# pynbody/topsy

Measured on AMD Instinct MI355X. Metric: particles/sec splatted to 1024^2 buffer, higher is better.
Workload: dtype f32

## Files before the change

### include/topsy_splat.h

```cpp
#ifndef TOPSY_SPLAT_H
#define TOPSY_SPLAT_H

#include <stdint.h>

#ifdef __cplusplus
extern "C" {
#endif

typedef struct tsp_context tsp_context;

enum {
    TSP_OK = 0,
    TSP_EINVAL = -1,
    TSP_EHIP = -2,
    TSP_ENODEV = -3,
    TSP_ESTATE = -4,
    TSP_ECOMM = -5,
    TSP_ENOMEM = -6
};

enum {
    TSP_MODE_WEIGHTED = 0,
    TSP_MODE_DEPTH = 1,
    TSP_MODE_RGB = 2,
    TSP_MODE_KINEMATIC = 3
};

enum {
    TSP_PIPE_DEFAULT = 0,
    TSP_PIPE_GENERIC = 1,
    TSP_SAMPLE_BILINEAR_MIP0 = 0x10,
    TSP_SAMPLE_BILINEAR_MIP = 0x20
};

const char *tsp_last_error(void);
int tsp_version(void);
int tsp_stats_size(void);

int tsp_device_count(void);

int tsp_create(int device_id, int resolution, int n_channels, tsp_context **out);
void tsp_destroy(tsp_context *ctx);

int tsp_set_kernel_mips(tsp_context *ctx, const float *lut, int n0, int n_levels);

int tsp_upload_particles(tsp_context *ctx, int64_t n, const float *x, const float *y, const float *z,
                         const float *h, const float *mass);
int tsp_upload_quantity(tsp_context *ctx, const float *q);
int tsp_upload_rgb(tsp_context *ctx, const float *r, const float *g, const float *b);
int tsp_upload_band_magnitudes(tsp_context *ctx, int n_bands, const double *mags, const double *weights);

int tsp_generate_synthetic(tsp_context *ctx, int64_t n_total, int64_t first, int64_t count,
                           uint64_t seed, float h_cap, int with_quantity, int with_rgb);

int tsp_reorder_spatial(tsp_context *ctx, int n_strata, uint64_t seed, int64_t *perm_out);
int tsp_get_strata_offsets(tsp_context *ctx, int64_t *offsets_out, int capacity);

int tsp_get_cell_layout(tsp_context *ctx, int *n_strata_out, int *cells_per_axis_out, float *box_lo_out ,
                        float *cell_width_out );
int64_t tsp_get_cell_offsets(tsp_context *ctx, int64_t *offsets_out, int64_t capacity);

int tsp_download_particles(tsp_context *ctx, float *x, float *y, float *z, float *h, float *mass,
                           float *q, float *r, float *g, float *b);
int64_t tsp_num_particles(tsp_context *ctx);

int tsp_render(tsp_context *ctx, const float *M, float scale_factor, const int64_t *starts,
               const int64_t *lens, int n_ranges, int clear, int mode, int flags, double *gpu_ms_out);

int tsp_render_undo(tsp_context *ctx);

int tsp_read_image(tsp_context *ctx, float *out);
int tsp_write_image(tsp_context *ctx, const float *in);

int tsp_colormap_scalar(tsp_context *ctx, const float *lut_rgba, int n_lut, float vmin, float vmax,
                        int log_scale, int weighted, uint8_t *out_rgba);
int tsp_colormap_rgb(tsp_context *ctx, float vmin, float vmax, float gamma, uint8_t *out_rgba8,
                     float *out_rgba_f32);

int tsp_colormap_set_lut2d(tsp_context *ctx, const float *lut_rgba, int n);
int tsp_colormap_bivariate(tsp_context *ctx, float vmin, float vmax, float density_vmin, float density_vmax,
                           int log_scale, int weighted, uint8_t *out_rgba);
int tsp_colormap_bivariate_host(tsp_context *ctx, const float *img, int H, int W, int C, float vmin, float vmax,
                                float density_vmin, float density_vmax, int log_scale, int weighted,
                                uint8_t *out_rgba);

int tsp_colormap_scalar_host(tsp_context *ctx, const float *img, int H, int W, int C,
                             const float *lut_rgba, int n_lut, float vmin, float vmax, int log_scale,
                             int weighted, uint8_t *out_rgba);
int tsp_colormap_rgb_host(tsp_context *ctx, const float *img, int H, int W, int C, float vmin,
                          float vmax, float gamma, uint8_t *out_rgba8, float *out_rgba_f32);

int tsp_tile_periodic(tsp_context *ctx, int n, const float *offsets_xy, const float *weights);

int tsp_smoothing_lengths(tsp_context *ctx, int64_t n, const float *x, const float *y, const float *z,
                          int n_neighbours, float period, float *h_out);

int tsp_sph_sum(tsp_context *ctx, int64_t n, const float *x, const float *y, const float *z, const float *h,
                const float *a, float period, float *out);

typedef struct {
    int64_t n_valid, n_inside;
    int32_t iterations, reserved;
    double radius, mass_inside;
} tsp_center_info;
int tsp_shrink_sphere_center(tsp_context *ctx, int64_t n, const float *x, const float *y, const float *z, const float *mass,
                             float mass_cut_factor, double r_start, double shrink_factor, int64_t min_particles,
                             int max_iterations, double center_out[3], tsp_center_info *info_out);

typedef struct {
    int64_t n_valid, n_groups, n_grouped, largest;
} tsp_fof_info;
int tsp_fof_groups(tsp_context *ctx, int64_t n, const float *x, const float *y, const float *z, float linking_length,
                   float period, int64_t min_members, int32_t *group_out, tsp_fof_info *info_out);

typedef struct {
    int64_t n_valid, n_inside, n_inside_vel;
    double  mass, mass_vel;
    double  com[3];
    double  v_cen[3];
    double  L[3];
    double  S[6];
    double  A;
} tsp_moments;
int tsp_sphere_moments(tsp_context *ctx, int64_t n, const float *x, const float *y, const float *z, const float *mass,
                       const float *vx, const float *vy, const float *vz,
                       const double center[3], double r, double r_vel, tsp_moments *out);

typedef struct {
    int32_t geometry;
    int32_t n_bins;
    const double *edges;
    double center[3];
    double v_cen[3];
    double frame[9];
    double half_height;
} tsp_profile_spec;
typedef struct {
    int64_t n_valid, n_inner, n_binned;
    double  mass_inner;
} tsp_profile_info;
int tsp_radial_profile(tsp_context *ctx, int64_t n, const float *x, const float *y, const float *z, const float *mass,
                       const float *vx, const float *vy, const float *vz,
                       const tsp_profile_spec *spec, int64_t *count_out , double *sums_out ,
                       tsp_profile_info *info_out);

int tsp_upload_velocities(tsp_context *ctx, const float *vx, const float *vy, const float *vz);
int tsp_set_line_of_sight(tsp_context *ctx, const float axis[3], const float v_ref[3]);
int tsp_velocity_moments(tsp_context *ctx, float *maps_out );
int tsp_colormap_moment(tsp_context *ctx, int which , const float *lut_rgba, int n_lut, float vmin, float vmax,
                        int log_scale, uint8_t *out_rgba8);
int tsp_moment_sort(tsp_context *ctx, int which , int absolute, int64_t *n_finite);

typedef struct tsp_surface_params {
    double smoothing_scale;
    float depth_scale;
    float light_direction[3];
    float light_color[3];
    float ambient_color[3];
    float vmin, vmax;
    int weighted_average;
    int log_scale;
    const float *lut_rgba;
    int n_lut;
} tsp_surface_params;

int tsp_set_sphere_mips(tsp_context *ctx, const float *lut, int n0, int n_levels);
int tsp_density_order_stats(tsp_context *ctx, const int64_t *ranks, int n_ranks, float *values_out);
int tsp_render_surface(tsp_context *ctx, const float *M, float scale_factor, float density_cut, const int64_t *starts,
                       const int64_t *lens, int n_ranges, int clear, double *gpu_ms_out);
int tsp_surface_present(tsp_context *ctx, const tsp_surface_params *params, float *content_out, uint8_t *rgba8_out,
                        double *ms_out);

enum { TSP_PRESENT_SCALAR = 0, TSP_PRESENT_BIVARIATE = 1, TSP_PRESENT_RGB = 2, TSP_PRESENT_RGB_HDR = 3, TSP_PRESENT_MOMENT_MEAN = 4,
       TSP_PRESENT_MOMENT_SIGMA = 5 };
enum { TSP_LAYER_QUAD = 0, TSP_LAYER_LINES = 1 };
typedef struct tsp_present_base {
    int map;
    float vmin, vmax;
    float density_vmin, density_vmax;
    float gamma;
    int log_scale, weighted;
    const float *lut_rgba;
    int n_lut;
} tsp_present_base;
typedef struct tsp_present_layer {
    int kind;
    const float *texture_rgba;
    int tex_width, tex_height;
    float clip_origin[2], clip_extent[2], tex_origin[2], tex_extent[2];
    int n_instances;
    const float *instance_offsets;
    const float *instance_weights;
    int n_segments;
    const float *starts, *ends;
    float transform[16];
    float color[4];
    float width_px;
} tsp_present_layer;
int tsp_present(tsp_context *ctx, int width, int height, const tsp_present_base *base, const tsp_present_layer *layers,
                int n_layers, void *out, double *gpu_ms_out);

int tsp_present_yuv420(tsp_context *ctx, int width, int height, const tsp_present_base *base, const tsp_present_layer *layers,
                       int n_layers, uint8_t *out, double *gpu_ms_out);

int tsp_present_surface(tsp_context *ctx, int width, int height, const tsp_surface_params *params, const tsp_present_layer *layers,
                        int n_layers, uint8_t *out_rgba8, double *ms_out);
int tsp_present_surface_yuv420(tsp_context *ctx, int width, int height, const tsp_surface_params *params,
                               const tsp_present_layer *layers, int n_layers, uint8_t *out, double *ms_out);

int tsp_content_sort(tsp_context *ctx, int kind, float scale, int64_t *n_finite, int64_t *n_nonpositive);
int tsp_content_values(tsp_context *ctx, const int64_t *ranks, int n_ranks, float *out);
int tsp_content_neg_inf(tsp_context *ctx, int64_t *n_neg_inf);

typedef struct {
    int64_t n_particles;
    int64_t n_small;
    int64_t n_mid;
    int64_t n_huge;
    int64_t n_culled;
    int64_t n_fragments;
    double ms_stream, ms_mid, ms_huge, ms_total;
    double ms_mega;
    int64_t n_mega;
    int64_t n_fragments_stream, n_fragments_mid, n_fragments_huge, n_fragments_mega;
    int64_t n_chunk_culled;
} tsp_stats;
int tsp_get_stats(tsp_context *ctx, tsp_stats *out);
int tsp_set_option(tsp_context *ctx, const char *name, int64_t value);

int tsp_measure_read_bandwidth(tsp_context *ctx, int64_t bytes, int iters, double *gbps_out);

#define TSP_UNIQUE_ID_BYTES 128
int tsp_comm_unique_id(char *id_out);
int tsp_comm_init(tsp_context *ctx, int n_ranks, int rank, const char *id);
int tsp_comm_reduce_image(tsp_context *ctx, int root, double *gpu_ms_out);
int tsp_comm_destroy(tsp_context *ctx);
int tsp_set_reduced_image(tsp_context *ctx, const float *sum);

typedef struct tsp_group tsp_group;
int tsp_group_create(int n_devices, const int *device_ids, int resolution, int n_channels, tsp_group **out);
void tsp_group_destroy(tsp_group *group);
int tsp_group_size(tsp_group *group);
tsp_context *tsp_group_context(tsp_group *group, int index);
int tsp_group_uses_rccl(tsp_group *group);
int tsp_group_set_kernel_mips(tsp_group *group, const float *lut, int n0, int n_levels);
int tsp_group_upload_particles(tsp_group *group, int64_t n, const float *x, const float *y, const float *z, const float *h,
                               const float *mass);
int tsp_group_upload_quantity(tsp_group *group, const float *q);
int tsp_group_upload_rgb(tsp_group *group, const float *r, const float *g, const float *b);
int tsp_group_generate_synthetic(tsp_group *group, int64_t n_total, int64_t first, int64_t count, uint64_t seed, float h_cap,
                                 int with_quantity, int with_rgb);
int tsp_group_reorder_spatial(tsp_group *group, int n_strata, uint64_t seed);
int64_t tsp_group_num_particles(tsp_group *group);
int tsp_group_set_option(tsp_group *group, const char *name, int64_t value);
int tsp_group_render(tsp_group *group, const float *M, float scale_factor, const int64_t *starts, const int64_t *lens,
                     int n_ranges, int clear, int mode, int flags, double *gpu_ms_out);
int tsp_group_end_frame(tsp_group *group, double *ms_out);
int tsp_group_get_stats(tsp_group *group, tsp_stats *out);
int tsp_group_shard_range(tsp_group *group, int index, int64_t *first_out, int64_t *count_out);
int tsp_group_upload_band_magnitudes(tsp_group *group, int n_bands, const double *mags, const double *weights);

#ifdef __cplusplus
}
#endif
#endif
```

### topsy_amd/_native.py

```python
import ctypes
import os

import numpy as np

_HERE = os.path.dirname(os.path.abspath(__file__))
LIB_PATH = os.environ.get("TOPSY_SPLAT_LIB") or os.path.join(_HERE, "libtopsy_splat.so")

MODE_WEIGHTED, MODE_DEPTH, MODE_RGB, MODE_KINEMATIC = 0, 1, 2, 3
PIPE_DEFAULT, PIPE_GENERIC = 0, 1
SAMPLE_BILINEAR_MIP0, SAMPLE_BILINEAR_MIP = 0x10, 0x20
UNIQUE_ID_BYTES = 128
ABI_VERSION = 112
PRESENT_SCALAR, PRESENT_BIVARIATE, PRESENT_RGB, PRESENT_RGB_HDR, PRESENT_MOMENT_MEAN, PRESENT_MOMENT_SIGMA = 0, 1, 2, 3, 4, 5
LAYER_QUAD, LAYER_LINES = 0, 1


class SurfaceParams(ctypes.Structure):
    _fields_ = [("smoothing_scale", ctypes.c_double), ("depth_scale", ctypes.c_float),
                ("light_direction", ctypes.c_float * 3), ("light_color", ctypes.c_float * 3), ("ambient_color", ctypes.c_float * 3),
                ("vmin", ctypes.c_float), ("vmax", ctypes.c_float), ("weighted_average", ctypes.c_int), ("log_scale", ctypes.c_int),
                ("lut_rgba", ctypes.POINTER(ctypes.c_float)), ("n_lut", ctypes.c_int)]


class PresentBase(ctypes.Structure):
    _fields_ = [("map", ctypes.c_int), ("vmin", ctypes.c_float), ("vmax", ctypes.c_float), ("density_vmin", ctypes.c_float),
                ("density_vmax", ctypes.c_float), ("gamma", ctypes.c_float), ("log_scale", ctypes.c_int), ("weighted", ctypes.c_int),
                ("lut_rgba", ctypes.POINTER(ctypes.c_float)), ("n_lut", ctypes.c_int)]


class PresentLayer(ctypes.Structure):
    _fields_ = [("kind", ctypes.c_int), ("texture_rgba", ctypes.POINTER(ctypes.c_float)), ("tex_width", ctypes.c_int),
                ("tex_height", ctypes.c_int), ("clip_origin", ctypes.c_float * 2), ("clip_extent", ctypes.c_float * 2),
                ("tex_origin", ctypes.c_float * 2), ("tex_extent", ctypes.c_float * 2), ("n_instances", ctypes.c_int),
                ("instance_offsets", ctypes.POINTER(ctypes.c_float)), ("instance_weights", ctypes.POINTER(ctypes.c_float)),
                ("n_segments", ctypes.c_int), ("starts", ctypes.POINTER(ctypes.c_float)), ("ends", ctypes.POINTER(ctypes.c_float)),
                ("transform", ctypes.c_float * 16), ("color", ctypes.c_float * 4), ("width_px", ctypes.c_float)]


class CenterInfo(ctypes.Structure):
    _fields_ = [("n_valid", ctypes.c_int64), ("n_inside", ctypes.c_int64), ("iterations", ctypes.c_int32),
                ("reserved", ctypes.c_int32), ("radius", ctypes.c_double), ("mass_inside", ctypes.c_double)]


class FofInfo(ctypes.Structure):
    _fields_ = [("n_valid", ctypes.c_int64), ("n_groups", ctypes.c_int64), ("n_grouped", ctypes.c_int64),
                ("largest", ctypes.c_int64)]


class Moments(ctypes.Structure):
    _fields_ = [("n_valid", ctypes.c_int64), ("n_inside", ctypes.c_int64), ("n_inside_vel", ctypes.c_int64),
                ("mass", ctypes.c_double), ("mass_vel", ctypes.c_double), ("com", ctypes.c_double * 3),
                ("v_cen", ctypes.c_double * 3), ("L", ctypes.c_double * 3), ("S", ctypes.c_double * 6), ("A", ctypes.c_double)]

    def as_dict(self):
        out = {}
        for name, kind in self._fields_:
            v = getattr(self, name)
            out[name] = int(v) if kind is ctypes.c_int64 else float(v) if kind is ctypes.c_double else np.array(v, dtype=np.float64)
        return out


class ProfileSpec(ctypes.Structure):
    _fields_ = [("geometry", ctypes.c_int32), ("n_bins", ctypes.c_int32), ("edges", ctypes.POINTER(ctypes.c_double)),
                ("center", ctypes.c_double * 3), ("v_cen", ctypes.c_double * 3), ("frame", ctypes.c_double * 9),
                ("half_height", ctypes.c_double)]


class ProfileInfo(ctypes.Structure):
    _fields_ = [("n_valid", ctypes.c_int64), ("n_inner", ctypes.c_int64), ("n_binned", ctypes.c_int64),
                ("mass_inner", ctypes.c_double)]


PROFILE_SUMS = 11


class BackendUnavailable(RuntimeError):
    """libtopsy_splat.so could not be loaded, or no MI355X-class GPU is visible."""


class BackendError(RuntimeError):
    """A C-ABI call returned a negative status."""


class Stats(ctypes.Structure):
    _fields_ = [("n_particles", ctypes.c_int64), ("n_small", ctypes.c_int64), ("n_mid", ctypes.c_int64),
                ("n_huge", ctypes.c_int64), ("n_culled", ctypes.c_int64), ("n_fragments", ctypes.c_int64),
                ("ms_stream", ctypes.c_double), ("ms_mid", ctypes.c_double), ("ms_huge", ctypes.c_double),
                ("ms_total", ctypes.c_double), ("ms_mega", ctypes.c_double), ("n_mega", ctypes.c_int64),
                ("n_fragments_stream", ctypes.c_int64), ("n_fragments_mid", ctypes.c_int64),
                ("n_fragments_huge", ctypes.c_int64), ("n_fragments_mega", ctypes.c_int64), ("n_chunk_culled", ctypes.c_int64)]

    def as_dict(self):
        return {k: getattr(self, k) for k, _ in self._fields_}


_fp = ctypes.POINTER(ctypes.c_float)
_i64p = ctypes.POINTER(ctypes.c_int64)
_u8p = ctypes.POINTER(ctypes.c_uint8)
_ctx = ctypes.c_void_p

SIGNATURES = {
    "tsp_last_error": (ctypes.c_char_p, []),
    "tsp_version": (ctypes.c_int, []),
    "tsp_stats_size": (ctypes.c_int, []),
    "tsp_device_count": (ctypes.c_int, []),
    "tsp_create": (ctypes.c_int, [ctypes.c_int, ctypes.c_int, ctypes.c_int, ctypes.POINTER(_ctx)]),
    "tsp_destroy": (None, [_ctx]),
    "tsp_set_kernel_mips": (ctypes.c_int, [_ctx, _fp, ctypes.c_int, ctypes.c_int]),
    "tsp_upload_particles": (ctypes.c_int, [_ctx, ctypes.c_int64, _fp, _fp, _fp, _fp, _fp]),
    "tsp_upload_quantity": (ctypes.c_int, [_ctx, _fp]),
    "tsp_upload_rgb": (ctypes.c_int, [_ctx, _fp, _fp, _fp]),
    "tsp_upload_velocities": (ctypes.c_int, [_ctx, _fp, _fp, _fp]),
    "tsp_set_line_of_sight": (ctypes.c_int, [_ctx, _fp, _fp]),
    "tsp_velocity_moments": (ctypes.c_int, [_ctx, _fp]),
    "tsp_colormap_moment": (ctypes.c_int, [_ctx, ctypes.c_int, _fp, ctypes.c_int, ctypes.c_float, ctypes.c_float, ctypes.c_int, _u8p]),
    "tsp_upload_band_magnitudes": (ctypes.c_int, [_ctx, ctypes.c_int, ctypes.POINTER(ctypes.c_double), ctypes.POINTER(ctypes.c_double)]),
    "tsp_generate_synthetic": (ctypes.c_int, [_ctx, ctypes.c_int64, ctypes.c_int64, ctypes.c_int64, ctypes.c_uint64,
                                              ctypes.c_float, ctypes.c_int, ctypes.c_int]),
    "tsp_reorder_spatial": (ctypes.c_int, [_ctx, ctypes.c_int, ctypes.c_uint64, _i64p]),
    "tsp_get_strata_offsets": (ctypes.c_int, [_ctx, _i64p, ctypes.c_int]),
    "tsp_get_cell_layout": (ctypes.c_int, [_ctx, ctypes.POINTER(ctypes.c_int), ctypes.POINTER(ctypes.c_int), _fp, _fp]),
    "tsp_get_cell_offsets": (ctypes.c_int64, [_ctx, _i64p, ctypes.c_int64]),
    "tsp_download_particles": (ctypes.c_int, [_ctx] + [_fp] * 9),
    "tsp_num_particles": (ctypes.c_int64, [_ctx]),
    "tsp_render": (ctypes.c_int, [_ctx, _fp, ctypes.c_float, _i64p, _i64p, ctypes.c_int, ctypes.c_int, ctypes.c_int,
                                  ctypes.c_int, ctypes.POINTER(ctypes.c_double)]),
    "tsp_render_undo": (ctypes.c_int, [_ctx]),
    "tsp_read_image": (ctypes.c_int, [_ctx, _fp]),
    "tsp_write_image": (ctypes.c_int, [_ctx, _fp]),
    "tsp_colormap_scalar": (ctypes.c_int, [_ctx, _fp, ctypes.c_int, ctypes.c_float, ctypes.c_float, ctypes.c_int,
                                           ctypes.c_int, _u8p]),
    "tsp_colormap_rgb": (ctypes.c_int, [_ctx, ctypes.c_float, ctypes.c_float, ctypes.c_float, _u8p, _fp]),
    "tsp_colormap_set_lut2d": (ctypes.c_int, [_ctx, _fp, ctypes.c_int]),
    "tsp_colormap_bivariate": (ctypes.c_int, [_ctx, ctypes.c_float, ctypes.c_float, ctypes.c_float, ctypes.c_float, ctypes.c_int,
                                              ctypes.c_int, _u8p]),
    "tsp_colormap_bivariate_host": (ctypes.c_int, [_ctx, _fp, ctypes.c_int, ctypes.c_int, ctypes.c_int, ctypes.c_float, ctypes.c_float,
                                                   ctypes.c_float, ctypes.c_float, ctypes.c_int, ctypes.c_int, _u8p]),
    "tsp_colormap_scalar_host": (ctypes.c_int, [_ctx, _fp, ctypes.c_int, ctypes.c_int, ctypes.c_int, _fp, ctypes.c_int,
                                                ctypes.c_float, ctypes.c_float, ctypes.c_int, ctypes.c_int, _u8p]),
    "tsp_colormap_rgb_host": (ctypes.c_int, [_ctx, _fp, ctypes.c_int, ctypes.c_int, ctypes.c_int, ctypes.c_float,
                                             ctypes.c_float, ctypes.c_float, _u8p, _fp]),
    "tsp_tile_periodic": (ctypes.c_int, [_ctx, ctypes.c_int, _fp, _fp]),
    "tsp_smoothing_lengths": (ctypes.c_int, [_ctx, ctypes.c_int64, _fp, _fp, _fp, ctypes.c_int, ctypes.c_float, _fp]),
    "tsp_sph_sum": (ctypes.c_int, [_ctx, ctypes.c_int64, _fp, _fp, _fp, _fp, _fp, ctypes.c_float, _fp]),
    "tsp_shrink_sphere_center": (ctypes.c_int, [_ctx, ctypes.c_int64, _fp, _fp, _fp, _fp, ctypes.c_float, ctypes.c_double,
                                                ctypes.c_double, ctypes.c_int64, ctypes.c_int, ctypes.POINTER(ctypes.c_double),
                                                ctypes.POINTER(CenterInfo)]),
    "tsp_fof_groups": (ctypes.c_int, [_ctx, ctypes.c_int64, _fp, _fp, _fp, ctypes.c_float, ctypes.c_float, ctypes.c_int64,
                                      ctypes.POINTER(ctypes.c_int32), ctypes.POINTER(FofInfo)]),
    "tsp_sphere_moments": (ctypes.c_int, [_ctx, ctypes.c_int64, _fp, _fp, _fp, _fp, _fp, _fp, _fp, ctypes.POINTER(ctypes.c_double),
                                          ctypes.c_double, ctypes.c_double, ctypes.POINTER(Moments)]),
    "tsp_radial_profile": (ctypes.c_int, [_ctx, ctypes.c_int64, _fp, _fp, _fp, _fp, _fp, _fp, _fp, ctypes.POINTER(ProfileSpec), _i64p,
                                          ctypes.POINTER(ctypes.c_double), ctypes.POINTER(ProfileInfo)]),
    "tsp_set_sphere_mips": (ctypes.c_int, [_ctx, _fp, ctypes.c_int, ctypes.c_int]),
    "tsp_density_order_stats": (ctypes.c_int, [_ctx, _i64p, ctypes.c_int, _fp]),
    "tsp_render_surface": (ctypes.c_int, [_ctx, _fp, ctypes.c_float, ctypes.c_float, _i64p, _i64p, ctypes.c_int, ctypes.c_int,
                                          ctypes.POINTER(ctypes.c_double)]),
    "tsp_surface_present": (ctypes.c_int, [_ctx, ctypes.c_void_p, _fp, _u8p, ctypes.POINTER(ctypes.c_double)]),
    "tsp_present": (ctypes.c_int, [_ctx, ctypes.c_int, ctypes.c_int, ctypes.c_void_p, ctypes.c_void_p, ctypes.c_int, ctypes.c_void_p,
                                   ctypes.POINTER(ctypes.c_double)]),
    "tsp_present_yuv420": (ctypes.c_int, [_ctx, ctypes.c_int, ctypes.c_int, ctypes.c_void_p, ctypes.c_void_p, ctypes.c_int, _u8p,
                                          ctypes.POINTER(ctypes.c_double)]),
    "tsp_present_surface": (ctypes.c_int, [_ctx, ctypes.c_int, ctypes.c_int, ctypes.c_void_p, ctypes.c_void_p, ctypes.c_int, _u8p,
                                           ctypes.POINTER(ctypes.c_double)]),
    "tsp_present_surface_yuv420": (ctypes.c_int, [_ctx, ctypes.c_int, ctypes.c_int, ctypes.c_void_p, ctypes.c_void_p, ctypes.c_int,
                                                  _u8p, ctypes.POINTER(ctypes.c_double)]),
    "tsp_content_sort": (ctypes.c_int, [_ctx, ctypes.c_int, ctypes.c_float, _i64p, _i64p]),
    "tsp_moment_sort": (ctypes.c_int, [_ctx, ctypes.c_int, ctypes.c_int, _i64p]),
    "tsp_content_values": (ctypes.c_int, [_ctx, _i64p, ctypes.c_int, _fp]),
    "tsp_content_neg_inf": (ctypes.c_int, [_ctx, _i64p]),
    "tsp_get_stats": (ctypes.c_int, [_ctx, ctypes.POINTER(Stats)]),
    "tsp_set_option": (ctypes.c_int, [_ctx, ctypes.c_char_p, ctypes.c_int64]),
    "tsp_measure_read_bandwidth": (ctypes.c_int, [_ctx, ctypes.c_int64, ctypes.c_int, ctypes.POINTER(ctypes.c_double)]),
    "tsp_comm_unique_id": (ctypes.c_int, [ctypes.c_char_p]),
    "tsp_comm_init": (ctypes.c_int, [_ctx, ctypes.c_int, ctypes.c_int, ctypes.c_char_p]),
    "tsp_comm_reduce_image": (ctypes.c_int, [_ctx, ctypes.c_int, ctypes.POINTER(ctypes.c_double)]),
    "tsp_comm_destroy": (ctypes.c_int, [_ctx]),
    "tsp_set_reduced_image": (ctypes.c_int, [_ctx, _fp]),
    "tsp_group_create": (ctypes.c_int, [ctypes.c_int, ctypes.POINTER(ctypes.c_int), ctypes.c_int, ctypes.c_int, ctypes.POINTER(_ctx)]),
    "tsp_group_destroy": (None, [_ctx]),
    "tsp_group_size": (ctypes.c_int, [_ctx]),
    "tsp_group_context": (_ctx, [_ctx, ctypes.c_int]),
    "tsp_group_uses_rccl": (ctypes.c_int, [_ctx]),
    "tsp_group_set_kernel_mips": (ctypes.c_int, [_ctx, _fp, ctypes.c_int, ctypes.c_int]),
    "tsp_group_upload_particles": (ctypes.c_int, [_ctx, ctypes.c_int64, _fp, _fp, _fp, _fp, _fp]),
    "tsp_group_upload_quantity": (ctypes.c_int, [_ctx, _fp]),
    "tsp_group_upload_rgb": (ctypes.c_int, [_ctx, _fp, _fp, _fp]),
    "tsp_group_generate_synthetic": (ctypes.c_int, [_ctx, ctypes.c_int64, ctypes.c_int64, ctypes.c_int64, ctypes.c_uint64,
                                                    ctypes.c_float, ctypes.c_int, ctypes.c_int]),
    "tsp_group_reorder_spatial": (ctypes.c_int, [_ctx, ctypes.c_int, ctypes.c_uint64]),
    "tsp_group_num_particles": (ctypes.c_int64, [_ctx]),
    "tsp_group_set_option": (ctypes.c_int, [_ctx, ctypes.c_char_p, ctypes.c_int64]),
    "tsp_group_render": (ctypes.c_int, [_ctx, _fp, ctypes.c_float, _i64p, _i64p, ctypes.c_int, ctypes.c_int, ctypes.c_int,
                                        ctypes.c_int, ctypes.POINTER(ctypes.c_double)]),
    "tsp_group_end_frame": (ctypes.c_int, [_ctx, ctypes.POINTER(ctypes.c_double)]),
    "tsp_group_get_stats": (ctypes.c_int, [_ctx, ctypes.POINTER(Stats)]),
    "tsp_group_shard_range": (ctypes.c_int, [_ctx, ctypes.c_int, _i64p, _i64p]),
    "tsp_group_upload_band_magnitudes": (ctypes.c_int, [_ctx, ctypes.c_int, ctypes.POINTER(ctypes.c_double), ctypes.POINTER(ctypes.c_double)]),
}

_lib = None


def load_library():
    global _lib
    if _lib is not None:
        return _lib
    if not os.path.exists(LIB_PATH):
        raise BackendUnavailable(
            f"{LIB_PATH} not found: build it with `python -c 'import __graft_entry__ as g; g.build()'` "
            f"or `make -C topsy_amd/csrc` (needs hipcc, --offload-arch=gfx950)")
    try:
        lib = ctypes.CDLL(LIB_PATH)
    except OSError as e:
        raise BackendUnavailable(f"cannot load {LIB_PATH}: {e}") from e
    for name, (restype, argtypes) in SIGNATURES.items():
        try:
            fn = getattr(lib, name)
        except AttributeError as e:
            raise BackendUnavailable(f"{LIB_PATH} does not export {name}") from e
        fn.restype = restype
        fn.argtypes = argtypes
    if lib.tsp_version() < ABI_VERSION or lib.tsp_stats_size() != ctypes.sizeof(Stats):
        raise BackendUnavailable(f"{LIB_PATH} has ABI version {lib.tsp_version()} / tsp_stats of {lib.tsp_stats_size()} bytes; "
                                 f"this binding needs version >= {ABI_VERSION} and {ctypes.sizeof(Stats)} bytes: rebuild the library")
    _lib = lib
    return lib


def _check(rc):
    if rc < 0:
        raise BackendError(f"libtopsy_splat error {rc}: {load_library().tsp_last_error().decode(errors='replace')}")
    return rc


def _f32(a, n=None, name="array"):
    a = np.ascontiguousarray(a, dtype=np.float32)
    if n is not None and a.size != n:
        raise ValueError(f"{name} has {a.size} elements, expected {n}")
    return a


def _ptr(a):
    return None if a is None else a.ctypes.data_as(_fp)


def device_count():
    return load_library().tsp_device_count()


def _ranges(starts, lens):
    if starts is None:
        return None, None, 0, None
    s = np.ascontiguousarray(starts, dtype=np.int64)
    l = np.ascontiguousarray(lens, dtype=np.int64)
    if s.shape != l.shape or s.ndim != 1:
        raise ValueError("starts and lens must be 1-D arrays of equal length")
    if len(s) == 0:
        s = np.zeros(1, dtype=np.int64)
        l = np.zeros(1, dtype=np.int64)
    return s.ctypes.data_as(_i64p), l.ctypes.data_as(_i64p), len(s), (s, l)


class Context:

    def __init__(self, resolution, n_channels, device_id=0):
        lib = load_library()
        ndev = lib.tsp_device_count()
        if ndev <= 0:
            raise BackendUnavailable("no HIP device visible: the topsy_amd render path needs an AMD GPU "
                                     "(there is no CPU fallback)")
        h = _ctx()
        _check(lib.tsp_create(int(device_id), int(resolution), int(n_channels), ctypes.byref(h)))
        self._h = h
        self._lib = lib
        self.resolution = int(resolution)
        self.n_channels = int(n_channels)
        self.active_channels = int(n_channels)
        self.device_id = int(device_id)

    def close(self):
        if getattr(self, "_h", None):
            self._lib.tsp_destroy(self._h)
            self._h = None

    def __del__(self):
        try:
            self.close()
        except Exception:
            pass

    def set_kernel_mips(self, mips, n0=64, n_levels=4):
        mips = _f32(mips, name="kernel mips")
        _check(self._lib.tsp_set_kernel_mips(self._h, _ptr(mips), n0, n_levels))

    def upload_particles(self, x, y, z, h, mass=None):
        n = len(x)
        arrs = [_f32(a, n, nm) for a, nm in ((x, "x"), (y, "y"), (z, "z"), (h, "h"))]
        m = None if mass is None else _f32(mass, n, "mass")
        _check(self._lib.tsp_upload_particles(self._h, n, *[_ptr(a) for a in arrs], _ptr(m)))

    def upload_quantity(self, q):
        q = None if q is None else _f32(q, self.num_particles, "quantity")
        _check(self._lib.tsp_upload_quantity(self._h, _ptr(q)))

    def upload_rgb(self, r, g, b):
        n = self.num_particles
        r, g, b = _f32(r, n, "r"), _f32(g, n, "g"), _f32(b, n, "b")
        _check(self._lib.tsp_upload_rgb(self._h, _ptr(r), _ptr(g), _ptr(b)))

    def upload_velocities(self, vx, vy=None, vz=None):
        if vx is None and vy is None and vz is None:
            _check(self._lib.tsp_upload_velocities(self._h, None, None, None))
            return
        n = self.num_particles
        v = [None if a is None else _f32(a, n, name) for a, name in ((vx, "vx"), (vy, "vy"), (vz, "vz"))]
        _check(self._lib.tsp_upload_velocities(self._h, *[_ptr(a) for a in v]))

    def set_line_of_sight(self, axis, v_ref=(0.0, 0.0, 0.0)):
        axis, v_ref = _f32(axis, 3, "axis"), _f32(v_ref, 3, "v_ref")
        _check(self._lib.tsp_set_line_of_sight(self._h, _ptr(axis), _ptr(v_ref)))

    def velocity_moments(self):
        out = np.empty((self.resolution, self.resolution, 4), dtype=np.float32)
        _check(self._lib.tsp_velocity_moments(self._h, _ptr(out)))
        return out

    def colormap_moment(self, which, lut_rgba, vmin, vmax, log=False):
        lut = _f32(lut_rgba, name="lut")
        out = np.empty((self.resolution, self.resolution, 4), dtype=np.uint8)
        _check(self._lib.tsp_colormap_moment(self._h, int(which), _ptr(lut), lut.size // 4, float(vmin), float(vmax), int(bool(log)),
                                             out.ctypes.data_as(_u8p)))
        return out

    def upload_band_magnitudes(self, mags, weights):
        mags = np.ascontiguousarray(mags, dtype=np.float64)
        weights = np.ascontiguousarray(weights, dtype=np.float64)
        if mags.ndim != 2 or mags.shape[1] != self.num_particles or weights.shape != (3, mags.shape[0]):
            raise ValueError("mags must be (n_bands, n_particles) and weights (3, n_bands)")
        dp = ctypes.POINTER(ctypes.c_double)
        _check(self._lib.tsp_upload_band_magnitudes(self._h, mags.shape[0], mags.ctypes.data_as(dp), weights.ctypes.data_as(dp)))

    def generate_synthetic(self, n_total, first=0, count=None, seed=1337, h_cap=0.0, with_quantity=False,
                           with_rgb=False):
        count = n_total - first if count is None else count
        _check(self._lib.tsp_generate_synthetic(self._h, n_total, first, count, seed, h_cap, int(with_quantity),
                                                int(with_rgb)))

    def reorder_spatial(self, n_strata=1, seed=1337, want_permutation=False):
        perm = np.empty(self.num_particles, dtype=np.int64) if want_permutation else None
        _check(self._lib.tsp_reorder_spatial(self._h, n_strata, seed,
                                             None if perm is None else perm.ctypes.data_as(_i64p)))
        return perm

    def strata_offsets(self):
        buf = np.empty(4098, dtype=np.int64)
        k = int(self._lib.tsp_get_strata_offsets(self._h, buf.ctypes.data_as(_i64p), len(buf)))
        return buf[:k].copy()

    def cell_layout(self):
        ns, ca = ctypes.c_int(0), ctypes.c_int(0)
        lo, width = np.zeros(3, dtype=np.float32), np.zeros(3, dtype=np.float32)
        if self._lib.tsp_get_cell_layout(self._h, ctypes.byref(ns), ctypes.byref(ca), _ptr(lo), _ptr(width)) < 0:
            return None
        buf = np.empty(ns.value * ca.value ** 3 + 1, dtype=np.int64)
        k = int(self._lib.tsp_get_cell_offsets(self._h, buf.ctypes.data_as(_i64p), len(buf)))
        if k != len(buf):
            raise BackendError("tsp_get_cell_offsets returned an unexpected number of values")
        return {"n_strata": ns.value, "cells_per_axis": ca.value, "box_lo": lo.astype(np.float64),
                "cell_width": width.astype(np.float64), "offsets": buf}

    def cell_layouts(self):
        lay = self.cell_layout()
        return [] if lay is None else [lay]

    def download_particles(self, names=("x", "y", "z", "h", "mass")):
        order = ("x", "y", "z", "h", "mass", "q", "r", "g", "b")
        n = self.num_particles
        out = {k: np.empty(n, dtype=np.float32) for k in names}
        _check(self._lib.tsp_download_particles(self._h, *[_ptr(out.get(k)) for k in order]))
        return out

    @property
    def num_particles(self):
        return int(self._lib.tsp_num_particles(self._h))

    def render(self, matrix, scale_factor, starts=None, lens=None, clear=True, mode=MODE_WEIGHTED, flags=PIPE_DEFAULT):
        M = _f32(np.asarray(matrix, dtype=np.float32).reshape(16), 16, "matrix")
        ms = ctypes.c_double(0.0)
        sp, lp, nr, _keep = _ranges(starts, lens)
        _check(self._lib.tsp_render(self._h, _ptr(M), float(scale_factor), sp, lp, nr, int(bool(clear)), int(mode),
                                    int(flags), ctypes.byref(ms)))
        self.active_channels = 4 if mode in (MODE_RGB, MODE_KINEMATIC) else 2
        return ms.value

    def render_undo(self):
        _check(self._lib.tsp_render_undo(self._h))

    def read_image(self):
        out = np.empty((self.resolution, self.resolution, self.active_channels), dtype=np.float32)
        _check(self._lib.tsp_read_image(self._h, _ptr(out)))
        return out

    def write_image(self, img):
        img = np.ascontiguousarray(img, dtype=np.float32)
        if img.shape[:2] != (self.resolution, self.resolution) or img.shape[2] not in (2, 4) or img.shape[2] > self.n_channels:
            raise ValueError(f"image shape {img.shape} does not fit the render target")
        self.set_option("active_channels", img.shape[2])
        self.active_channels = img.shape[2]
        _check(self._lib.tsp_write_image(self._h, _ptr(img)))

    def tile_periodic(self, offsets_xy, weights):
        off = _f32(offsets_xy, name="offsets")
        w = _f32(weights, name="weights")
        if off.size != 2 * w.size:
            raise ValueError("offsets must have shape (n, 2) for n weights")
        _check(self._lib.tsp_tile_periodic(self._h, w.size, _ptr(off), _ptr(w)))

    def smoothing_lengths(self, x, y, z, n_neighbours=32, period=None):
        n = len(x)
        x, y, z = _f32(x, n, "x"), _f32(y, n, "y"), _f32(z, n, "z")
        out = np.empty(n, dtype=np.float32)
        _check(self._lib.tsp_smoothing_lengths(self._h, n, _ptr(x), _ptr(y), _ptr(z), int(n_neighbours),
                                               float(np.float32(period or 0.0)), _ptr(out)))
        return out

    def sph_sum(self, x, y, z, h, a, period=None):
        n = len(x)
        x, y, z, h, a = _f32(x, n, "x"), _f32(y, n, "y"), _f32(z, n, "z"), _f32(h, n, "h"), _f32(a, n, "a")
        out = np.empty(n, dtype=np.float32)
        _check(self._lib.tsp_sph_sum(self._h, n, _ptr(x), _ptr(y), _ptr(z), _ptr(h), _ptr(a), float(np.float32(period or 0.0)),
                                     _ptr(out)))
        return out

    def shrink_sphere_center(self, x, y, z, mass, mass_cut_factor=0.0, r_start=0.0, shrink_factor=0.7, min_particles=100,
                             max_iterations=256):
        n = len(x)
        x, y, z, mass = _f32(x, n, "x"), _f32(y, n, "y"), _f32(z, n, "z"), _f32(mass, n, "mass")
        center = np.empty(3, dtype=np.float64)
        info = CenterInfo()
        _check(self._lib.tsp_shrink_sphere_center(self._h, n, _ptr(x), _ptr(y), _ptr(z), _ptr(mass), float(np.float32(mass_cut_factor)),
                                                  float(r_start), float(shrink_factor), int(min_particles), int(max_iterations),
                                                  center.ctypes.data_as(ctypes.POINTER(ctypes.c_double)), ctypes.byref(info)))
        return center, {"n_valid": int(info.n_valid), "n_inside": int(info.n_inside), "iterations": int(info.iterations),
                        "radius": float(info.radius), "mass_inside": float(info.mass_inside)}

    def fof_groups(self, x, y, z, linking_length, period=0.0, min_members=20):
        n = len(x)
        x, y, z = _f32(x, n, "x"), _f32(y, n, "y"), _f32(z, n, "z")
        out = np.empty(n, dtype=np.int32)
        info = FofInfo()
        _check(self._lib.tsp_fof_groups(self._h, n, _ptr(x), _ptr(y), _ptr(z), float(np.float32(linking_length)),
                                        float(np.float32(period or 0.0)), int(min_members),
                                        out.ctypes.data_as(ctypes.POINTER(ctypes.c_int32)), ctypes.byref(info)))
        return out, {"n_valid": int(info.n_valid), "n_groups": int(info.n_groups), "n_grouped": int(info.n_grouped),
                     "largest": int(info.largest)}

    def sphere_moments(self, x, y, z, mass, vel=None, center=(0.0, 0.0, 0.0), r=1.0, r_vel=0.0):
        n = len(x)
        x, y, z, mass = _f32(x, n, "x"), _f32(y, n, "y"), _f32(z, n, "z"), _f32(mass, n, "mass")
        if vel is not None:
            if len(vel) != 3:
                raise ValueError("vel must be the three arrays (vx, vy, vz)")
            vel = [_f32(v, n, name) for v, name in zip(vel, ("vx", "vy", "vz"))]
        vx, vy, vz = vel if vel is not None else (None, None, None)
        center = np.ascontiguousarray(center, dtype=np.float64)
        if center.shape != (3,):
            raise ValueError(f"center must be three coordinates, not shape {center.shape}")
        out = Moments()
        _check(self._lib.tsp_sphere_moments(self._h, n, _ptr(x), _ptr(y), _ptr(z), _ptr(mass), _ptr(vx), _ptr(vy), _ptr(vz),
                                            center.ctypes.data_as(ctypes.POINTER(ctypes.c_double)), float(r), float(r_vel),
                                            ctypes.byref(out)))
        return out.as_dict()

    def radial_profile(self, x, y, z, mass, vel=None, edges=(0.0, 1.0), geometry=0, center=(0.0, 0.0, 0.0), v_cen=(0.0, 0.0, 0.0),
                       frame=None, half_height=np.inf):
        n = len(x)
        x, y, z, mass = _f32(x, n, "x"), _f32(y, n, "y"), _f32(z, n, "z"), _f32(mass, n, "mass")
        if vel is not None:
            if len(vel) != 3:
                raise ValueError("vel must be the three arrays (vx, vy, vz)")
            vel = [_f32(v, n, name) for v, name in zip(vel, ("vx", "vy", "vz"))]
        vx, vy, vz = vel if vel is not None else (None, None, None)
        edges = np.ascontiguousarray(edges, dtype=np.float64)
        if edges.ndim != 1 or len(edges) < 2:
            raise ValueError(f"edges must be at least two radii, not shape {edges.shape}")
        spec = ProfileSpec()
        spec.geometry, spec.n_bins = int(geometry), len(edges) - 1
        spec.edges = edges.ctypes.data_as(ctypes.POINTER(ctypes.c_double))
        for name, value, shape in (("center", center, (3,)), ("v_cen", v_cen, (3,)),
                                   ("frame", np.eye(3) if frame is None else frame, (3, 3))):
            value = np.ascontiguousarray(value, dtype=np.float64)
            if value.shape != shape:
                raise ValueError(f"{name} must have shape {shape}, not {value.shape}")
            getattr(spec, name)[:] = value.ravel().tolist()
        spec.half_height = float(half_height)
        count = np.zeros(spec.n_bins, dtype=np.int64)
        sums = np.zeros((spec.n_bins, PROFILE_SUMS), dtype=np.float64)
        info = ProfileInfo()
        _check(self._lib.tsp_radial_profile(self._h, n, _ptr(x), _ptr(y), _ptr(z), _ptr(mass), _ptr(vx), _ptr(vy), _ptr(vz),
                                            ctypes.byref(spec), count.ctypes.data_as(_i64p),
                                            sums.ctypes.data_as(ctypes.POINTER(ctypes.c_double)), ctypes.byref(info)))
        return {"count": count, "sums": sums, "n_valid": int(info.n_valid), "n_inner": int(info.n_inner),
                "n_binned": int(info.n_binned), "mass_inner": float(info.mass_inner)}

    def set_sphere_mips(self, mips, n0=64, n_levels=4):
        mips = _f32(mips, name="sphere mips")
        _check(self._lib.tsp_set_sphere_mips(self._h, _ptr(mips), n0, n_levels))

    def density_order_stats(self, ranks):
        r = np.ascontiguousarray(ranks, dtype=np.int64)
        out = np.empty(len(r), dtype=np.float32)
        _check(self._lib.tsp_density_order_stats(self._h, r.ctypes.data_as(_i64p), len(r), _ptr(out)))
        return out

    def render_surface(self, matrix, scale_factor, density_cut, starts=None, lens=None, clear=True):
        M = _f32(np.asarray(matrix, dtype=np.float32).reshape(16), 16, "matrix")
        ms = ctypes.c_double(0.0)
        sp, lp, nr, _keep = _ranges(starts, lens)
        _check(self._lib.tsp_render_surface(self._h, _ptr(M), float(scale_factor), float(np.float32(density_cut)), sp, lp, nr,
                                            int(bool(clear)), ctypes.byref(ms)))
        self.active_channels = 2
        return ms.value

    @staticmethod
    def _surface_params(smoothing_scale=0.01, depth_scale=1.0, light_direction=(0.0, 0.0, 1.0), light_color=(1.0, 1.0, 1.0),
                        ambient_color=(0.2, 0.2, 0.2), vmin=0.0, vmax=1.0, weighted_average=False, log=False, lut_rgba=None):
        p = SurfaceParams()
        p.smoothing_scale = float(smoothing_scale)
        p.depth_scale = float(depth_scale)
        p.light_direction[:] = [float(np.float32(v)) for v in light_direction]
        p.light_color[:] = [float(np.float32(v)) for v in light_color]
        p.ambient_color[:] = [float(np.float32(v)) for v in ambient_color]
        p.vmin, p.vmax = float(np.float32(vmin)), float(np.float32(vmax))
        p.weighted_average, p.log_scale = int(bool(weighted_average)), int(bool(log))
        lut = None
        if weighted_average:
            lut = _f32(lut_rgba, name="lut")
            p.lut_rgba, p.n_lut = _ptr(lut), lut.size // 4
        return p, lut

    def surface_present(self, smoothing_scale=0.01, depth_scale=1.0, light_direction=(0.0, 0.0, 1.0), light_color=(1.0, 1.0, 1.0),
                        ambient_color=(0.2, 0.2, 0.2), vmin=0.0, vmax=1.0, weighted_average=False, log=False, lut_rgba=None,
                        content=True, rgba=True, timings=None):
        p, _lut = self._surface_params(smoothing_scale, depth_scale, light_direction, light_color, ambient_color, vmin, vmax,
                                       weighted_average, log, lut_rgba)
        R = self.resolution
        c = np.empty((R, R, 2), dtype=np.float32) if content else None
        o = np.empty((R, R, 4), dtype=np.uint8) if rgba else None
        ms = (ctypes.c_double * 2)()
        _check(self._lib.tsp_surface_present(self._h, ctypes.byref(p), _ptr(c), None if o is None else o.ctypes.data_as(_u8p), ms))
        if timings is not None:
            timings[:] = [ms[0], ms[1]]
        return c, o

    def present_surface(self, width, height, params=None, layers=(), timings=None):
# ... 322 lines not shown
```

### topsy_amd/csrc/tsp_api.hip

```cpp
#include <stdarg.h>
#include <string.h>

#include <algorithm>
#include <cmath>
#include <vector>

#include "tsp_internal.h"

namespace tsp {

static thread_local char g_err[1024] = "";

void set_error(const char *fmt, ...) {
    va_list ap;
    va_start(ap, fmt);
    vsnprintf(g_err, sizeof(g_err), fmt, ap);
    va_end(ap);
}

int ensure_array(float **p, int64_t n) {
    if (*p) {
        TSP_HIP(hipFree(*p));
        *p = nullptr;
    }
// ... 36 lines not shown
            }
            return rc;
        }
    }
    for (const Capacity &c : caps) c.set(c.value);
    return TSP_OK;
}

int scratch_alloc(tsp_context *ctx, const char *site, DeviceScratch &buf, size_t bytes) {
    TSP_REQUIRE(!buf.p, TSP_ESTATE, "scratch buffer of site %s is allocated twice", site);
    if (ctx->debug_fail_alloc > 0 && --ctx->debug_fail_alloc == 0) {
        set_error("injected allocation failure at %s (debug_fail_alloc)", site);
        return TSP_ENOMEM;
    }
    const hipError_t e = hipMalloc(&buf.p, bytes ? bytes : 16);
    if (e != hipSuccess) {
        (void)hipGetLastError();
        buf.p = nullptr;
        set_error("hipMalloc of %zu bytes failed at %s: %s", bytes, site, hipGetErrorString(e));
        return e == hipErrorOutOfMemory ? TSP_ENOMEM : TSP_EHIP;
    }
    return TSP_OK;
}

int check_workspace(const tsp_context *ctx) {
    const Workspace &ws = ctx->ws;
    struct Pair { int64_t cap; const void *p; const char *name; } pairs[] = {
        {ws.mid_capacity, ws.mid_geom, "mid_geom"}, {ws.mid_capacity, ws.mid_w, "mid_w"},
        {ws.huge_capacity, ws.huge_geom, "huge_geom"}, {ws.huge_capacity, ws.huge_w, "huge_w"},
        {ws.hband_stride, ws.hband_geom, "hband_geom"}, {ws.hband_stride, ws.hband_w, "hband_w"}, {ws.hband_stride, ws.hband_count, "hband_count"},
        {ws.hband_bands, ws.hband_geom, "hband_geom"},
        {ws.mband_capacity, ws.mband_geom, "mband_geom"}, {ws.mband_capacity, ws.mband_w, "mband_w"},
        {ws.mitem_capacity, ws.mitem_tile, "mitem_tile"},
        {ws.mtile_capacity, ws.mband_count, "mband_count"}, {ws.mtile_capacity, ws.mband_base, "mband_base"},
        {ws.mtile_capacity, ws.mitem_base, "mitem_base"},
        {ws.chunk_capacity, ws.alive_list, "alive_list"},
        {ws.bounds_capacity, ws.block_bounds, "block_bounds"},
        {ws.range_capacity, ws.range_prefix, "range_prefix"},
        {ws.count_R, ws.count_diff, "count_diff"}, {ws.count_R, ws.count_band, "count_band"},
    };
    for (const Pair &q : pairs)
        TSP_REQUIRE(q.cap <= 0 || q.p, TSP_ESTATE, "workspace invariant broken: %s is null with capacity %lld", q.name, (long long)q.cap);
    return TSP_OK;
}

static int upload_array(tsp_context *ctx, float **dst, const float *src, int64_t n) {
    if (!*dst) TSP_HIP(hipMalloc((void **)dst, (size_t)n * sizeof(float)));
    TSP_HIP(hipMemcpyAsync(*dst, src, (size_t)n * sizeof(float), hipMemcpyHostToDevice, ctx->stream));
    return TSP_OK;
}

__global__ void image_to_float_kernel(const double *__restrict__ src, float *__restrict__ dst, int64_t n) {
    for (int64_t i = (int64_t)blockIdx.x * blockDim.x + threadIdx.x; i < n; i += (int64_t)gridDim.x * blockDim.x)
        dst[i] = (float)src[i];
}
__global__ void image_to_double_kernel(const float *__restrict__ src, double *__restrict__ dst, int64_t n) {
    for (int64_t i = (int64_t)blockIdx.x * blockDim.x + threadIdx.x; i < n; i += (int64_t)gridDim.x * blockDim.x)
        dst[i] = (double)src[i];
}

int launch_image_convert(tsp_context *ctx, bool to_float) {
    const int64_t n = (int64_t)ctx->R * ctx->R * ctx->C;
    const unsigned grid = (unsigned)std::min<int64_t>((n + 255) / 256, (int64_t)ctx->cu_count * 8);
    if (to_float) hipLaunchKernelGGL(image_to_float_kernel, dim3(grid), dim3(256), 0, ctx->stream, ctx->image64, ctx->image, n);
    else hipLaunchKernelGGL(image_to_double_kernel, dim3(grid), dim3(256), 0, ctx->stream, ctx->image, ctx->image64, n);
    TSP_HIP(hipGetLastError());
    return TSP_OK;
}

__global__ void gather_kernel(const float *__restrict__ src, const uint32_t *__restrict__ perm, float *__restrict__ dst,
                              int64_t n) {
    for (int64_t i = (int64_t)blockIdx.x * blockDim.x + threadIdx.x; i < n; i += (int64_t)gridDim.x * blockDim.x)
        dst[i] = src[perm[i]];
}

static int upload_permuted(tsp_context *ctx, float **dst, const float *src, int64_t n) {
    if (!ctx->p.perm) return upload_array(ctx, dst, src, n);
    float *tmp = nullptr;
    TSP_HIP(hipMalloc((void **)&tmp, (size_t)n * sizeof(float)));
    TSP_HIP(hipMemcpyAsync(tmp, src, (size_t)n * sizeof(float), hipMemcpyHostToDevice, ctx->stream));
    if (!*dst) TSP_HIP(hipMalloc((void **)dst, (size_t)n * sizeof(float)));
    hipLaunchKernelGGL(gather_kernel, dim3(2048), dim3(256), 0, ctx->stream, tmp, ctx->p.perm, *dst, n);
    TSP_HIP(hipGetLastError());
    TSP_HIP(hipStreamSynchronize(ctx->stream));
    TSP_HIP(hipFree(tmp));
    return TSP_OK;
}

static void free_particles(tsp_context *ctx) {
    Particles &p = ctx->p;
    float **arrs[] = {&p.x, &p.y, &p.z, &p.h, &p.m, &p.q, &p.r, &p.g, &p.b, &p.vx, &p.vy, &p.vz};
    for (float **a : arrs) {
        if (*a) (void)hipFree(*a);
        *a = nullptr;
    }
    float **derived[] = {&p.wm, &p.wr, &p.wg, &p.wb};
    for (float **a : derived) {
        if (*a) (void)hipFree(*a);
        *a = nullptr;
    }
    p.wm_valid = false;
    p.wrgb_source = W_NONE;
    if (p.perm) (void)hipFree(p.perm);
    p.perm = nullptr;
    p.n = 0;
    ctx->ws.bounds_valid = false;
    ctx->surface_keys = false;
    ctx->forget_render_undo();
    ctx->strata_offsets.clear();
    ctx->cell_offsets.clear();
    ctx->cell_bits = 0;
}

static int clip_ranges(const tsp_context *ctx, const int64_t *starts, const int64_t *lens, int n_ranges, std::vector<int64_t> &s,
                       std::vector<int64_t> &l, int64_t *total) {
    if (!starts) {
        if (ctx->p.n > 0) { s.push_back(0); l.push_back(ctx->p.n); }
    } else {
        for (int i = 0; i < n_ranges; ++i) {
            TSP_REQUIRE(lens[i] >= 0, TSP_EINVAL, "range %d has negative length %lld", i, (long long)lens[i]);
            int64_t b = starts[i], len = lens[i];
            if (b < 0) {
                len = (len > -b) ? len + b : 0;
                b = 0;
            }
            if (b >= ctx->p.n || len == 0) continue;
            if (len > ctx->p.n - b) len = ctx->p.n - b;
            s.push_back(b);
            l.push_back(len);
        }
    }
    *total = 0;
    for (int64_t v : l) *total += v;
    return TSP_OK;
}

static Camera make_camera(const tsp_context *ctx, const float *M, float scale_factor) {
    Camera cam;
    for (int i = 0; i < 12; ++i) cam.m[i] = M[i];
    cam.sf = scale_factor;
    cam.R = ctx->R;
    cam.Rf = (float)ctx->R;
    cam.halfR = 0.5f * cam.Rf;
    return cam;
}

}

using namespace tsp;

extern "C" {

const char *tsp_last_error(void) { return g_err; }
int tsp_version(void) { return 119; }
int tsp_stats_size(void) { return (int)sizeof(tsp_stats); }

int tsp_device_count(void) {
    int n = 0;
    if (hipGetDeviceCount(&n) != hipSuccess) {
        set_error("hipGetDeviceCount failed");
        return TSP_ENODEV;
    }
    return n;
}

static int create_resources(tsp_context *ctx, int device_id, int resolution, int n_channels) {
    hipDeviceProp_t prop;
    TSP_HIP(hipGetDeviceProperties(&prop, device_id));
    ctx->cu_count = prop.multiProcessorCount > 0 ? prop.multiProcessorCount : 256;
    TSP_HIP(hipStreamCreateWithFlags(&ctx->stream, hipStreamNonBlocking));
    TSP_HIP(hipStreamCreateWithFlags(&ctx->stream2, hipStreamNonBlocking));
    for (auto &e : ctx->ev) TSP_HIP(hipEventCreate(&e));
    const size_t npx = (size_t)resolution * resolution;
    TSP_HIP(hipMalloc((void **)&ctx->image, npx * n_channels * sizeof(float)));
    TSP_HIP(hipMemsetAsync(ctx->image, 0, npx * n_channels * sizeof(float), ctx->stream));
    TSP_HIP(hipMalloc((void **)&ctx->image64, npx * n_channels * sizeof(double)));
    TSP_HIP(hipMemsetAsync(ctx->image64, 0, npx * n_channels * sizeof(double), ctx->stream));
    TSP_HIP(hipMalloc((void **)&ctx->mips, 2 * MIP_TOTAL * sizeof(float)));
    TSP_HIP(hipMalloc((void **)&ctx->counters, sizeof(Counters)));
    TSP_HIP(hipMemsetAsync(ctx->counters, 0, sizeof(Counters), ctx->stream));
    TSP_HIP(hipMalloc((void **)&ctx->out8, npx * 4));
    TSP_HIP(hipStreamSynchronize(ctx->stream));
    return TSP_OK;
}

int tsp_create(int device_id, int resolution, int n_channels, tsp_context **out) {
    TSP_REQUIRE(out != nullptr, TSP_EINVAL, "out is NULL");
    *out = nullptr;
    TSP_REQUIRE(resolution > 0 && resolution <= 16384, TSP_EINVAL, "resolution %d out of range", resolution);
    TSP_REQUIRE(n_channels == 2 || n_channels == 4, TSP_EINVAL, "n_channels must be 2 (SPH) or 4 (RGBSPH), got %d",
                n_channels);
    int ndev = 0;
    if (hipGetDeviceCount(&ndev) != hipSuccess || ndev <= 0) {
        set_error("no HIP device available");
        return TSP_ENODEV;
    }
    TSP_REQUIRE(device_id >= 0 && device_id < ndev, TSP_ENODEV, "device %d not present (%d devices)", device_id, ndev);
    TSP_HIP(hipSetDevice(device_id));
    tsp_context *ctx = new tsp_context();
    ctx->device = device_id;
    ctx->R = resolution;
    ctx->C = n_channels;
    ctx->Ccap = n_channels;
    const int rc = create_resources(ctx, device_id, resolution, n_channels);
    if (rc != TSP_OK) {
        tsp_destroy(ctx);
        return rc;
    }
    *out = ctx;
    return TSP_OK;
}

void tsp_destroy(tsp_context *ctx) {
    if (!ctx) return;
    (void)hipSetDevice(ctx->device);
    tsp_comm_destroy(ctx);
    free_particles(ctx);
    void *ptrs[] = {ctx->image, ctx->image64, ctx->image64_entry, ctx->mips, ctx->counters, ctx->out8, ctx->outf, ctx->lut, ctx->lut2d, ctx->scratch,
                    ctx->ws.mid_geom, ctx->ws.mid_w, ctx->ws.huge_geom, ctx->ws.huge_w, ctx->ws.hband_geom, ctx->ws.hband_w, ctx->ws.hband_count, ctx->ws.mband_geom, ctx->ws.mband_w, ctx->ws.mband_count, ctx->ws.mband_base, ctx->ws.mitem_tile, ctx->ws.mitem_base, 
                    ctx->ws.block_bounds, ctx->ws.alive_list, ctx->ws.cull_info, ctx->ws.range_prefix, ctx->ws.count_diff, ctx->ws.count_band, ctx->sort_keys, ctx->sort_keys_alt, ctx->sort_tmp};
    for (void *p : ptrs)
        if (p) (void)hipFree(p);
    for (auto &e : ctx->ev)
        if (e) (void)hipEventDestroy(e);
    if (ctx->stream2) (void)hipStreamDestroy(ctx->stream2);
    if (ctx->stream) (void)hipStreamDestroy(ctx->stream);
    delete ctx;
}

int tsp_set_kernel_mips(tsp_context *ctx, const float *lut, int n0, int n_levels) {
    TSP_REQUIRE(ctx && lut, TSP_EINVAL, "NULL argument");
    TSP_REQUIRE(n0 == 64 && n_levels == 4, TSP_EINVAL,
                "kernel texture must be 64^2 with 4 mip levels (reference sph.py:396), got n0=%d levels=%d", n0, n_levels);
    TSP_HIP(hipSetDevice(ctx->device));
    TSP_HIP(hipMemcpy(ctx->mips, lut, MIP_TOTAL * sizeof(float), hipMemcpyHostToDevice));
    ctx->have_mips = true;
    bool zero = true;
    for (int l = 0, off = 0; l < 4 && zero; off += (64 >> l) * (64 >> l), ++l) {
        const int n = 64 >> l;
        for (int j = 0; j < n && zero; ++j)
            for (int i = 0; i < n; ++i) {
                const double x = -2.0 + (i + 0.5) * 4.0 / n, y = -2.0 + (j + 0.5) * 4.0 / n;
                if (x * x + y * y >= 4.0 && lut[off + j * n + i] != 0.0f) { zero = false; break; }
            }
    }
    ctx->lut_zero_outside_disc = zero;
    bool sym = true;
    for (int l = 0, off = 0; l < 4 && sym; off += (64 >> l) * (64 >> l), ++l) {
        const int n = 64 >> l;
        for (int j = 0; j < n && sym; ++j)
            for (int i = 0; i < n; ++i)
                if (memcmp(&lut[off + j * n + i], &lut[off + j * n + (n - 1 - i)], 4) || memcmp(&lut[off + j * n + i], &lut[off + (n - 1 - j) * n + i], 4)) { sym = false; break; }
    }
    ctx->lut_mirror_symmetric = sym;
    return TSP_OK;
}

int tsp_upload_particles(tsp_context *ctx, int64_t n, const float *x, const float *y, const float *z, const float *h,
                         const float *mass) {
    TSP_REQUIRE(ctx, TSP_EINVAL, "NULL context");
    TSP_REQUIRE(n >= 0 && n < ((int64_t)1 << 32), TSP_EINVAL, "particle count %lld out of range", (long long)n);
    TSP_REQUIRE(n == 0 || (x && y && z && h), TSP_EINVAL, "NULL position/smoothing array");
    TSP_HIP(hipSetDevice(ctx->device));
    free_particles(ctx);
    ctx->p.n = n;
    if (n == 0) return TSP_OK;
    int rc;
    if ((rc = upload_array(ctx, &ctx->p.x, x, n))) return rc;
    if ((rc = upload_array(ctx, &ctx->p.y, y, n))) return rc;
    if ((rc = upload_array(ctx, &ctx->p.z, z, n))) return rc;
    if ((rc = upload_array(ctx, &ctx->p.h, h, n))) return rc;
    if (mass && (rc = upload_array(ctx, &ctx->p.m, mass, n))) return rc;
    TSP_HIP(hipStreamSynchronize(ctx->stream));
    return TSP_OK;
}

int tsp_upload_quantity(tsp_context *ctx, const float *q) {
    TSP_REQUIRE(ctx, TSP_EINVAL, "NULL context");
    TSP_REQUIRE(!q || ctx->p.n > 0, TSP_ESTATE, "upload particles before the quantity");
    TSP_HIP(hipSetDevice(ctx->device));
    ctx->forget_render_undo();
    if (!q) {
        if (ctx->p.q) TSP_HIP(hipFree(ctx->p.q));
        ctx->p.q = nullptr;
        return TSP_OK;
    }
    int rc = upload_permuted(ctx, &ctx->p.q, q, ctx->p.n);
    if (rc) return rc;
    TSP_HIP(hipStreamSynchronize(ctx->stream));
    return TSP_OK;
}

int tsp_upload_rgb(tsp_context *ctx, const float *r, const float *g, const float *b) {
    TSP_REQUIRE(ctx && r && g && b, TSP_EINVAL, "NULL argument");
    TSP_REQUIRE(ctx->p.n > 0, TSP_ESTATE, "upload particles before rgb");
    TSP_HIP(hipSetDevice(ctx->device));
    ctx->forget_render_undo();
    int rc;
    if ((rc = upload_permuted(ctx, &ctx->p.r, r, ctx->p.n))) return rc;
    if ((rc = upload_permuted(ctx, &ctx->p.g, g, ctx->p.n))) return rc;
    if ((rc = upload_permuted(ctx, &ctx->p.b, b, ctx->p.n))) return rc;
    ctx->p.wrgb_source = W_NONE;
    TSP_HIP(hipStreamSynchronize(ctx->stream));
    return TSP_OK;
}

int tsp_upload_velocities(tsp_context *ctx, const float *vx, const float *vy, const float *vz) {
    TSP_REQUIRE(ctx, TSP_EINVAL, "NULL context");
    TSP_REQUIRE((vx && vy && vz) || (!vx && !vy && !vz), TSP_EINVAL, "vx, vy and vz must be given together or not at all");
    Particles &p = ctx->p;
    TSP_REQUIRE(!vx || p.n > 0, TSP_ESTATE, "upload particles before the velocities");
    TSP_HIP(hipSetDevice(ctx->device));
    ctx->forget_render_undo();
    if (p.wrgb_source == W_KINEMATIC) p.wrgb_source = W_NONE;
    if (!vx) {
        float **arrs[] = {&p.vx, &p.vy, &p.vz};
        for (float **a : arrs) {
            if (*a) TSP_HIP(hipFree(*a));
            *a = nullptr;
        }
        return TSP_OK;
    }
    int rc;
    if ((rc = upload_permuted(ctx, &p.vx, vx, p.n))) return rc;
    if ((rc = upload_permuted(ctx, &p.vy, vy, p.n))) return rc;
    if ((rc = upload_permuted(ctx, &p.vz, vz, p.n))) return rc;
    TSP_HIP(hipStreamSynchronize(ctx->stream));
    return TSP_OK;
}

int tsp_set_line_of_sight(tsp_context *ctx, const float axis[3], const float v_ref[3]) {
    TSP_REQUIRE(ctx && axis && v_ref, TSP_EINVAL, "NULL argument");
    double norm2 = 0.0;
    for (int k = 0; k < 3; ++k) {
        TSP_REQUIRE(std::isfinite(axis[k]) && std::isfinite(v_ref[k]), TSP_EINVAL, "axis and v_ref must be finite");
        norm2 += (double)axis[k] * (double)axis[k];
    }
    TSP_REQUIRE(std::fabs(std::sqrt(norm2) - 1.0) <= 1e-5, TSP_EINVAL, "axis must have unit length to 1e-5, not %.9g", std::sqrt(norm2));
    for (int k = 0; k < 3; ++k) {
        ctx->los[k] = axis[k] == 0.0f ? 0.0f : axis[k];
        ctx->los[3 + k] = v_ref[k] == 0.0f ? 0.0f : v_ref[k];
    }
    ctx->have_los = true;
    return TSP_OK;
}

__global__ __launch_bounds__(256) void band_contraction_kernel(const double *__restrict__ mags, const double *__restrict__ weights,
                                                               int n_bands, int64_t n, const uint32_t *__restrict__ perm,
                                                               float *__restrict__ r, float *__restrict__ g, float *__restrict__ b) {
    for (int64_t i = (int64_t)blockIdx.x * blockDim.x + threadIdx.x; i < n; i += (int64_t)gridDim.x * blockDim.x) {
        const int64_t src = perm ? (int64_t)perm[i] : i;
        double acc[3] = {0.0, 0.0, 0.0};
        for (int k = 0; k < n_bands; ++k) {
            const double lum = pow(10.0, -0.4 * mags[(int64_t)k * n + src]);
            for (int c = 0; c < 3; ++c) {
                const double w = weights[c * n_bands + k];
                if (w != 0.0) acc[c] += w * lum;
            }
        }
        const float fr = (float)acc[0], fg = (float)acc[1], fb = (float)acc[2];
        r[i] = (fr != fr) ? 0.0f : fr;
        g[i] = (fg != fg) ? 0.0f : fg;
        b[i] = (fb != fb) ? 0.0f : fb;
    }
}

int tsp_upload_band_magnitudes(tsp_context *ctx, int n_bands, const double *mags, const double *weights) {
    TSP_REQUIRE(ctx && mags && weights, TSP_EINVAL, "NULL argument");
    TSP_REQUIRE(n_bands >= 1 && n_bands <= 64, TSP_EINVAL, "n_bands %d out of range", n_bands);
    TSP_REQUIRE(ctx->p.n > 0, TSP_ESTATE, "upload particles before the band magnitudes");
    TSP_HIP(hipSetDevice(ctx->device));
    ctx->forget_render_undo();
    const int64_t n = ctx->p.n;
    DeviceScratch d_mags, d_w;
    TSP_SCRATCH_ALLOC(ctx, SITE("band_magnitudes"), d_mags, (size_t)n_bands * n * sizeof(double));
    TSP_SCRATCH_ALLOC(ctx, SITE("band_weights"), d_w, (size_t)3 * n_bands * sizeof(double));
    TSP_HIP(hipMemcpyAsync(d_mags.p, mags, (size_t)n_bands * n * sizeof(double), hipMemcpyHostToDevice, ctx->stream));
// ... 99 lines not shown
    const int rc = render_block(ctx, M, scale_factor, starts, lens, n_ranges, clear, mode, flags, gpu_ms_out);
    if (rc != TSP_OK) {
        const std::string why = tsp_last_error();
        ctx->C = C_entry; ctx->stats = stats_entry; ctx->chunk_culled_particles = culled_entry;
        const hipError_t e0 = ctx->stream2 ? hipStreamSynchronize(ctx->stream2) : hipSuccess;
        const hipError_t e1 = hipMemcpyAsync(ctx->image64, ctx->image64_entry, bytes, hipMemcpyDeviceToDevice, ctx->stream);
        const hipError_t e2 = hipStreamSynchronize(ctx->stream);
        const hipError_t e = e0 != hipSuccess ? e0 : (e1 != hipSuccess ? e1 : e2);
        if (e != hipSuccess) set_error("%s; and the accumulator could not be restored (%s)", why.c_str(), hipGetErrorString(e));
        else set_error("%s", why.c_str());
        if (e == hipSuccess && !ctx->surface_keys) ctx->undo.kind = 2;
    } else {
        if (!ctx->surface_keys) {
            ctx->undo.kind = 1;
            ctx->undo.C = C_entry; ctx->undo.stats = stats_entry; ctx->undo.chunk_culled_particles = culled_entry;
            ctx->undo.image_source = source_entry;
            memcpy(ctx->undo.image_los, los_entry, sizeof(los_entry));
        }
        ctx->surface_keys = false;
    }
    return rc;
}

int tsp_render_undo(tsp_context *ctx) {
    TSP_REQUIRE(ctx, TSP_EINVAL, "NULL context");
    TSP_REQUIRE(ctx->undo.kind != 0, TSP_ESTATE, "nothing to undo: the last call that changed the image was not tsp_render");
    TSP_HIP(hipSetDevice(ctx->device));
    if (ctx->undo.kind == 1) {
        const size_t bytes = (size_t)ctx->R * ctx->R * ctx->Ccap * sizeof(double);
        if (ctx->stream2) TSP_HIP(hipStreamSynchronize(ctx->stream2));
        TSP_HIP(hipMemcpyAsync(ctx->image64, ctx->image64_entry, bytes, hipMemcpyDeviceToDevice, ctx->stream));
        ctx->C = ctx->undo.C; ctx->stats = ctx->undo.stats; ctx->chunk_culled_particles = ctx->undo.chunk_culled_particles;
        ctx->image_source = ctx->undo.image_source;
        memcpy(ctx->image_los, ctx->undo.image_los, sizeof(ctx->image_los));
    }
    ctx->forget_render_undo();
    const int rc = launch_image_convert(ctx, true);
    if (rc) return rc;
    ctx->image_is_reduced = false;
    TSP_HIP(hipStreamSynchronize(ctx->stream));
    return TSP_OK;
}

static int render_block(tsp_context *ctx, const float *M, float scale_factor, const int64_t *starts, const int64_t *lens,
                        int n_ranges, int clear, int mode, int flags, double *gpu_ms_out) {
    TSP_REQUIRE(ctx && M, TSP_EINVAL, "NULL argument");
    TSP_REQUIRE(ctx->have_mips, TSP_ESTATE, "tsp_set_kernel_mips must be called before tsp_render");
    TSP_REQUIRE(mode == TSP_MODE_WEIGHTED || mode == TSP_MODE_DEPTH || mode == TSP_MODE_RGB || mode == TSP_MODE_KINEMATIC, TSP_EINVAL,
                "bad mode %d", mode);
    const bool kinematic = mode == TSP_MODE_KINEMATIC;
    if (kinematic) {
        TSP_REQUIRE(ctx->Ccap == 4, TSP_EINVAL, "TSP_MODE_KINEMATIC needs a 4-channel context");
        TSP_REQUIRE(!(flags & (TSP_PIPE_GENERIC | TSP_SAMPLE_BILINEAR_MIP0 | TSP_SAMPLE_BILINEAR_MIP)), TSP_EINVAL,
                    "TSP_MODE_KINEMATIC draws with the three-class pipeline only (flags must be TSP_PIPE_DEFAULT)");
        TSP_REQUIRE(ctx->p.n == 0 || ctx->p.m, TSP_ESTATE, "mass array not uploaded");
        TSP_REQUIRE(ctx->p.n == 0 || (ctx->p.vx && ctx->p.vy && ctx->p.vz), TSP_ESTATE, "velocities not uploaded (tsp_upload_velocities)");
        TSP_REQUIRE(ctx->have_los, TSP_ESTATE, "no line of sight set (tsp_set_line_of_sight)");
    } else if (mode == TSP_MODE_RGB) {
        TSP_REQUIRE(ctx->Ccap == 4, TSP_EINVAL, "TSP_MODE_RGB needs a 4-channel context");
        TSP_REQUIRE(ctx->p.n == 0 || (ctx->p.r && ctx->p.g && ctx->p.b), TSP_ESTATE, "rgb arrays not uploaded");
    } else {
        TSP_REQUIRE(ctx->p.n == 0 || ctx->p.m, TSP_ESTATE, "mass array not uploaded");
    }
    const int newC = (mode == TSP_MODE_RGB || kinematic) ? 4 : 2;
    TSP_REQUIRE(clear || newC == ctx->C, TSP_ESTATE, "cannot accumulate a %d-channel block onto a %d-channel image",
                newC, ctx->C);
    const int source = newC == 4 ? (kinematic ? W_KINEMATIC : W_RGB) : W_NONE;
    if (!clear && newC == 4 && ctx->image_source != W_NONE) {
        TSP_REQUIRE(ctx->image_source == source, TSP_ESTATE, "cannot accumulate %s block onto %s image: start with clear = 1",
                    kinematic ? "a kinematic" : "an rgb", kinematic ? "an rgb" : "a kinematic");
        TSP_REQUIRE(!kinematic || !memcmp(ctx->image_los, ctx->los, sizeof(ctx->los)), TSP_ESTATE,
                    "the kinematic image was started along another line of sight (axis or v_ref): start with clear = 1");
    }
    ctx->C = newC;
    TSP_REQUIRE(n_ranges >= 0 && (n_ranges == 0 || (starts && lens) || (!starts && !lens)), TSP_EINVAL, "bad ranges");
    TSP_HIP(hipSetDevice(ctx->device));

    std::vector<int64_t> s, l;
    int64_t total = 0;
    if (int rc = clip_ranges(ctx, starts, lens, n_ranges, s, l, &total)) return rc;
    const int nr = (int)s.size();
    const Camera cam = make_camera(ctx, M, scale_factor);

    TSP_HIP(hipEventRecord(ctx->ev[EV_RENDER_BEGIN], ctx->stream));
    if (clear)
        TSP_HIP(hipMemsetAsync(ctx->image64, 0, (size_t)ctx->R * ctx->R * ctx->C * sizeof(double), ctx->stream));
    TSP_HIP(hipMemsetAsync(ctx->counters, 0, sizeof(Counters), ctx->stream));
    ctx->stats = tsp_stats{};
    ctx->stats.n_particles = total;
    ctx->chunk_culled_particles = 0;
    int rc = TSP_OK;
    if (total > 0) {
        const int rule = (flags & TSP_SAMPLE_BILINEAR_MIP0) ? 1 : ((flags & TSP_SAMPLE_BILINEAR_MIP) ? 2 : 0);
        if ((flags & TSP_PIPE_GENERIC) || rule != 0) {
            std::vector<int64_t> pack(3 * (size_t)nr + 1);
            int64_t acc = 0;
            for (int i = 0; i < nr; ++i) {
                pack[i] = s[i];
                pack[nr + i] = l[i];
                pack[2 * nr + i] = acc;
                acc += l[i];
            }
            pack[3 * nr] = acc;
            if (ctx->ws.range_capacity < (int64_t)pack.size()) {
                const int64_t cap = (int64_t)pack.size() * 2 + 64;
                if ((rc = alloc_group(ctx, {{"range_prefix_generic", (void **)&ctx->ws.range_prefix, (size_t)cap * sizeof(int64_t)}},
                                      {{&ctx->ws.range_capacity, cap}})))
                    return rc;
            }
            TSP_HIP(hipMemcpyAsync(ctx->ws.range_prefix, pack.data(), pack.size() * sizeof(int64_t),
                                   hipMemcpyHostToDevice, ctx->stream));
            rc = launch_generic(ctx, cam, ctx->ws.range_prefix, nr, total, mode, rule);
            TSP_HIP(hipStreamSynchronize(ctx->stream));
        } else {
            ctx->kinematic_block = kinematic;
            rc = launch_pipeline(ctx, cam, s.data(), l.data(), nr, total, kinematic ? (int)TSP_MODE_RGB : mode);
            ctx->kinematic_block = false;
        }
    }
    if (rc) return rc;
    if ((rc = launch_image_convert(ctx, true))) return rc;
    ctx->image_is_reduced = false;
    ctx->image_source = source;
    if (kinematic) memcpy(ctx->image_los, ctx->los, sizeof(ctx->los));
    TSP_HIP(hipEventRecord(ctx->ev[EV_RENDER_END], ctx->stream));
    TSP_HIP(hipStreamSynchronize(ctx->stream));
    float ms = 0.f;
    TSP_HIP(hipEventElapsedTime(&ms, ctx->ev[EV_RENDER_BEGIN], ctx->ev[EV_RENDER_END]));
    ctx->stats.ms_total = ms;
    Counters hc;
    TSP_HIP(hipMemcpy(&hc, ctx->counters, sizeof(hc), hipMemcpyDeviceToHost));
    ctx->stats.n_small = (int64_t)hc.n_small;
    ctx->stats.n_mid = (int64_t)hc.n_mid;
    ctx->stats.n_huge = (int64_t)hc.n_huge;
    ctx->stats.n_mega = 0;
    ctx->stats.n_culled = (int64_t)hc.n_culled + ctx->chunk_culled_particles;
    ctx->stats.n_chunk_culled = ctx->chunk_culled_particles;
    ctx->stats.n_fragments = (int64_t)hc.n_fragments;
    ctx->stats.n_fragments_stream = (int64_t)hc.n_frag_class[0];
    ctx->stats.n_fragments_mid = (int64_t)hc.n_frag_class[1];
    ctx->stats.n_fragments_huge = (int64_t)hc.n_frag_class[2];
    ctx->stats.n_fragments_mega = (int64_t)hc.n_frag_class[3];
    if (gpu_ms_out) *gpu_ms_out = ms;
    return TSP_OK;
}

int tsp_read_image(tsp_context *ctx, float *out) {
    TSP_REQUIRE(ctx && out, TSP_EINVAL, "NULL argument");
    TSP_HIP(hipSetDevice(ctx->device));
    TSP_HIP(hipMemcpy(out, ctx->image, (size_t)ctx->R * ctx->R * ctx->C * sizeof(float), hipMemcpyDeviceToHost));
    return TSP_OK;
}

int tsp_write_image(tsp_context *ctx, const float *in) {
    TSP_REQUIRE(ctx && in, TSP_EINVAL, "NULL argument");
    TSP_HIP(hipSetDevice(ctx->device));
    TSP_HIP(hipMemcpy(ctx->image, in, (size_t)ctx->R * ctx->R * ctx->C * sizeof(float), hipMemcpyHostToDevice));
    int rc = launch_image_convert(ctx, false);
    if (rc) return rc;
    ctx->forget_render_undo();
    ctx->image_is_reduced = false;
    ctx->surface_keys = false;
    TSP_HIP(hipStreamSynchronize(ctx->stream));
    return TSP_OK;
}

int tsp_set_reduced_image(tsp_context *ctx, const float *sum) {
    TSP_REQUIRE(ctx && sum, TSP_EINVAL, "NULL argument");
    TSP_REQUIRE(!ctx->image_is_reduced, TSP_ESTATE, "the render target was already reduced for this frame (call tsp_render before reducing again)");
    TSP_HIP(hipSetDevice(ctx->device));
    TSP_HIP(hipMemcpy(ctx->image, sum, (size_t)ctx->R * ctx->R * ctx->C * sizeof(float), hipMemcpyHostToDevice));
    ctx->forget_render_undo();
    ctx->image_is_reduced = true;
    return TSP_OK;
}

static int ensure_lut(tsp_context *ctx, const float *lut_rgba, int n_lut) {
    TSP_REQUIRE(lut_rgba && n_lut >= 2 && n_lut <= 65536, TSP_EINVAL, "bad colormap LUT (n=%d)", n_lut);
    if (ctx->lut_capacity < n_lut) {
        const int rc = alloc_group(ctx, {{"lut", (void **)&ctx->lut, (size_t)n_lut * 4 * sizeof(float)}}, {{&ctx->lut_capacity, n_lut}});
        if (rc) return rc;
    }
    TSP_HIP(hipMemcpyAsync(ctx->lut, lut_rgba, (size_t)n_lut * 4 * sizeof(float), hipMemcpyHostToDevice, ctx->stream));
    return TSP_OK;
}

int tsp_colormap_scalar(tsp_context *ctx, const float *lut_rgba, int n_lut, float vmin, float vmax, int log_scale,
                        int weighted, uint8_t *out_rgba) {
    TSP_REQUIRE(ctx && out_rgba, TSP_EINVAL, "NULL argument");
    TSP_HIP(hipSetDevice(ctx->device));
    int rc = ensure_lut(ctx, lut_rgba, n_lut);
    if (rc) return rc;
    const int64_t npix = (int64_t)ctx->R * ctx->R;
    rc = launch_colormap_scalar(ctx, ctx->image, npix, ctx->C, ctx->lut, n_lut, vmin, vmax, log_scale, weighted, ctx->out8);
    if (rc) return rc;
    TSP_HIP(hipMemcpyAsync(out_rgba, ctx->out8, (size_t)npix * 4, hipMemcpyDeviceToHost, ctx->stream));
    TSP_HIP(hipStreamSynchronize(ctx->stream));
    return TSP_OK;
}

static int ensure_outf(tsp_context *ctx) {
    if (ctx->outf) return TSP_OK;
    return alloc_group(ctx, {{"outf", (void **)&ctx->outf, (size_t)ctx->R * ctx->R * 4 * sizeof(float)}}, {});
}

static int moment_maps(tsp_context *ctx) {
    TSP_REQUIRE(ctx->image_source == W_KINEMATIC && ctx->C == 4, TSP_ESTATE,
                "the image is not a kinematic one (render with TSP_MODE_KINEMATIC first)");
    TSP_HIP(hipSetDevice(ctx->device));
    if (int rc = ensure_outf(ctx)) return rc;
    return launch_velocity_moments(ctx, ctx->image, (int64_t)ctx->R * ctx->R, ctx->outf);
}

int tsp_velocity_moments(tsp_context *ctx, float *maps_out) {
    TSP_REQUIRE(ctx && maps_out, TSP_EINVAL, "NULL argument");
    if (int rc = moment_maps(ctx)) return rc;
    TSP_HIP(hipMemcpyAsync(maps_out, ctx->outf, (size_t)ctx->R * ctx->R * 4 * sizeof(float), hipMemcpyDeviceToHost, ctx->stream));
    TSP_HIP(hipStreamSynchronize(ctx->stream));
    return TSP_OK;
}

int tsp_colormap_moment(tsp_context *ctx, int which, const float *lut_rgba, int n_lut, float vmin, float vmax, int log_scale,
                        uint8_t *out_rgba8) {
    TSP_REQUIRE(ctx && out_rgba8, TSP_EINVAL, "NULL argument");
    TSP_REQUIRE(which == 1 || which == 2, TSP_EINVAL, "which must be 1 (mean) or 2 (sigma), not %d", which);
    TSP_REQUIRE(lut_rgba && n_lut >= 2 && n_lut <= 65536, TSP_EINVAL, "bad colormap LUT (n=%d)", n_lut);
    int rc = moment_maps(ctx);
    if (rc) return rc;
    if ((rc = ensure_lut(ctx, lut_rgba, n_lut))) return rc;
    const int64_t npix = (int64_t)ctx->R * ctx->R;
    if ((rc = launch_colormap_scalar(ctx, ctx->outf + which, npix, 4, ctx->lut, n_lut, vmin, vmax, log_scale, 0, ctx->out8))) return rc;
    TSP_HIP(hipMemcpyAsync(out_rgba8, ctx->out8, (size_t)npix * 4, hipMemcpyDeviceToHost, ctx->stream));
    TSP_HIP(hipStreamSynchronize(ctx->stream));
    return TSP_OK;
}

int tsp_colormap_rgb(tsp_context *ctx, float vmin, float vmax, float gamma, uint8_t *out_rgba8, float *out_rgba_f32) {
    TSP_REQUIRE(ctx && (out_rgba8 || out_rgba_f32), TSP_EINVAL, "NULL argument");
    TSP_REQUIRE(ctx->C == 4, TSP_EINVAL, "rgb colormap needs a 4-channel image");
    TSP_HIP(hipSetDevice(ctx->device));
    const int64_t npix = (int64_t)ctx->R * ctx->R;
    int rc;
    if (out_rgba_f32 && (rc = ensure_outf(ctx))) return rc;
    rc = launch_colormap_rgb(ctx, ctx->image, npix, ctx->C, vmin, vmax, gamma, out_rgba8 ? ctx->out8 : nullptr,
                                 out_rgba_f32 ? ctx->outf : nullptr);
    if (rc) return rc;
    if (out_rgba8) TSP_HIP(hipMemcpyAsync(out_rgba8, ctx->out8, (size_t)npix * 4, hipMemcpyDeviceToHost, ctx->stream));
    if (out_rgba_f32)
        TSP_HIP(hipMemcpyAsync(out_rgba_f32, ctx->outf, (size_t)npix * 16, hipMemcpyDeviceToHost, ctx->stream));
    TSP_HIP(hipStreamSynchronize(ctx->stream));
    return TSP_OK;
}

int tsp_colormap_set_lut2d(tsp_context *ctx, const float *lut_rgba, int n) {
    TSP_REQUIRE(ctx && lut_rgba && n >= 2 && n <= 4096, TSP_EINVAL, "bad 2-D colormap LUT (n=%d)", n);
    TSP_HIP(hipSetDevice(ctx->device));
    if (ctx->lut2d_n != n || !ctx->lut2d) {
        const int rc = alloc_group(ctx, {{"lut2d", (void **)&ctx->lut2d, (size_t)n * n * 4 * sizeof(float)}}, {{&ctx->lut2d_n, n}});
        if (rc) return rc;
    }
    TSP_HIP(hipMemcpy(ctx->lut2d, lut_rgba, (size_t)n * n * 4 * sizeof(float), hipMemcpyHostToDevice));
    return TSP_OK;
}

int tsp_colormap_bivariate(tsp_context *ctx, float vmin, float vmax, float density_vmin, float density_vmax, int log_scale,
                           int weighted, uint8_t *out_rgba) {
    TSP_REQUIRE(ctx && out_rgba, TSP_EINVAL, "NULL argument");
    TSP_REQUIRE(ctx->lut2d, TSP_ESTATE, "tsp_colormap_set_lut2d must be called first");
    TSP_HIP(hipSetDevice(ctx->device));
    const int64_t npix = (int64_t)ctx->R * ctx->R;
    int rc = launch_colormap_bivariate(ctx, ctx->image, npix, ctx->C, vmin, vmax, density_vmin, density_vmax, log_scale, weighted,
                                       ctx->out8);
    if (rc) return rc;
    TSP_HIP(hipMemcpyAsync(out_rgba, ctx->out8, (size_t)npix * 4, hipMemcpyDeviceToHost, ctx->stream));
    TSP_HIP(hipStreamSynchronize(ctx->stream));
    return TSP_OK;
}

struct HostStage { float *in; uint8_t *out8; float *outf; };
static int stage_host_image(tsp_context *ctx, size_t in_bytes, size_t out8_bytes, size_t outf_bytes, HostStage &hs) {
    const size_t a_in = (in_bytes + 255) & ~(size_t)255, a_o8 = (out8_bytes + 255) & ~(size_t)255, bytes = a_in + a_o8 + outf_bytes;
    if (ctx->scratch_bytes < bytes)
        if (int rc = alloc_group(ctx, {{"colormap_scratch", &ctx->scratch, bytes}}, {{&ctx->scratch_bytes, (int64_t)bytes}})) return rc;
    hs.in = (float *)ctx->scratch;
    hs.out8 = (uint8_t *)ctx->scratch + a_in;
    hs.outf = (float *)(hs.out8 + a_o8);
    return TSP_OK;
}
static int unstage_host_image(tsp_context *ctx, const HostStage &hs, uint8_t *out8, size_t out8_bytes, float *outf, size_t outf_bytes) {
    if (out8) TSP_HIP(hipMemcpyAsync(out8, hs.out8, out8_bytes, hipMemcpyDeviceToHost, ctx->stream));
    if (outf) TSP_HIP(hipMemcpyAsync(outf, hs.outf, outf_bytes, hipMemcpyDeviceToHost, ctx->stream));
    TSP_HIP(hipStreamSynchronize(ctx->stream));
    return TSP_OK;
}

int tsp_colormap_scalar_host(tsp_context *ctx, const float *img, int H, int W, int C, const float *lut_rgba, int n_lut,
                             float vmin, float vmax, int log_scale, int weighted, uint8_t *out_rgba) {
    TSP_REQUIRE(ctx && img && out_rgba, TSP_EINVAL, "NULL argument");
    TSP_REQUIRE(H > 0 && W > 0 && C >= 2, TSP_EINVAL, "bad image shape %dx%dx%d", H, W, C);
    TSP_HIP(hipSetDevice(ctx->device));
    const int64_t npix = (int64_t)H * W;
    const size_t in_bytes = (size_t)npix * C * sizeof(float), out_bytes = (size_t)npix * 4;
    HostStage hs;
    int rc = stage_host_image(ctx, in_bytes, out_bytes, 0, hs);
    if (rc) return rc;
    if ((rc = ensure_lut(ctx, lut_rgba, n_lut))) return rc;
// ... 172 lines not shown
    TSP_REQUIRE(ctx && n_finite, TSP_EINVAL, "NULL argument");
    TSP_REQUIRE(which == 1 || which == 2, TSP_EINVAL, "which must be 1 (mean) or 2 (sigma), not %d", which);
    TSP_REQUIRE(ctx->image_source == W_KINEMATIC && ctx->C == 4, TSP_ESTATE,
                "the image is not a kinematic one (render with TSP_MODE_KINEMATIC first)");
    TSP_HIP(hipSetDevice(ctx->device));
    return moment_sort(ctx, which, absolute, n_finite);
}

int tsp_content_values(tsp_context *ctx, const int64_t *ranks, int n_ranks, float *out) {
    TSP_REQUIRE(ctx && ranks && out && n_ranks >= 0, TSP_EINVAL, "bad argument");
    TSP_REQUIRE(ctx->sort_keys_alt, TSP_ESTATE, "tsp_content_sort / tsp_moment_sort has not been called");
    TSP_HIP(hipSetDevice(ctx->device));
    for (int i = 0; i < n_ranks; ++i) {
        TSP_REQUIRE(ranks[i] >= 0 && ranks[i] < ctx->sorted_count, TSP_EINVAL, "rank %lld outside [0, %lld)",
                    (long long)ranks[i], (long long)ctx->sorted_count);
        uint32_t key;
        TSP_HIP(hipMemcpy(&key, ctx->sort_keys_alt + ranks[i], 4, hipMemcpyDeviceToHost));
        const uint32_t bits = (key & 0x80000000u) ? (key & 0x7fffffffu) : ~key;
        memcpy(&out[i], &bits, 4);
    }
    return TSP_OK;
}

int tsp_content_neg_inf(tsp_context *ctx, int64_t *n_neg_inf) {
    TSP_REQUIRE(ctx && n_neg_inf, TSP_EINVAL, "NULL argument");
    TSP_REQUIRE(ctx->sort_keys_alt, TSP_ESTATE, "tsp_content_sort / tsp_moment_sort has not been called");
    *n_neg_inf = ctx->sorted_neg_inf;
    return TSP_OK;
}

int tsp_set_sphere_mips(tsp_context *ctx, const float *lut, int n0, int n_levels) {
    TSP_REQUIRE(ctx && lut, TSP_EINVAL, "NULL argument");
    TSP_REQUIRE(n0 == 64 && n_levels == 4, TSP_EINVAL, "sphere texture must be 64^2 with 4 mip levels, got n0=%d levels=%d", n0,
                n_levels);
    TSP_HIP(hipSetDevice(ctx->device));
    TSP_HIP(hipMemcpy(ctx->mips + MIP_TOTAL, lut, MIP_TOTAL * sizeof(float), hipMemcpyHostToDevice));
    ctx->have_sphere_mips = true;
    return TSP_OK;
}

int tsp_density_order_stats(tsp_context *ctx, const int64_t *ranks, int n_ranks, float *values_out) {
    TSP_REQUIRE(ctx && n_ranks >= 0 && (n_ranks == 0 || (ranks && values_out)), TSP_EINVAL, "bad argument");
    TSP_REQUIRE(ctx->p.n > 0 && ctx->p.m, TSP_EINVAL, "the density cut needs resident particles with mass");
    for (int i = 0; i < n_ranks; ++i)
        TSP_REQUIRE(ranks[i] >= 0 && ranks[i] < ctx->p.n, TSP_EINVAL, "rank %lld outside [0, %lld)", (long long)ranks[i],
                    (long long)ctx->p.n);
    TSP_HIP(hipSetDevice(ctx->device));
    return density_order_stats(ctx, ranks, n_ranks, values_out);
}

int tsp_render_surface(tsp_context *ctx, const float *M, float scale_factor, float density_cut, const int64_t *starts,
                       const int64_t *lens, int n_ranges, int clear, double *gpu_ms_out) {
    TSP_REQUIRE(ctx && M, TSP_EINVAL, "NULL argument");
    TSP_REQUIRE(ctx->p.n == 0 || ctx->p.m, TSP_EINVAL, "the surface pass needs the mass array (density cut)");
    TSP_REQUIRE(ctx->p.n < ((int64_t)1 << 32), TSP_EINVAL, "the surface keys hold indices below 2^32");
    TSP_REQUIRE(n_ranges >= 0 && (n_ranges == 0 || (starts && lens) || (!starts && !lens)), TSP_EINVAL, "bad ranges");
    TSP_REQUIRE(ctx->have_sphere_mips, TSP_ESTATE, "tsp_set_sphere_mips must be called before tsp_render_surface");
    TSP_REQUIRE(clear || ctx->surface_keys, TSP_ESTATE, "clear = 0 continues a surface image; the accumulator holds none");
    ctx->forget_render_undo();
    TSP_HIP(hipSetDevice(ctx->device));
    std::vector<int64_t> s, l;
    int64_t total = 0;
    if (int rc = clip_ranges(ctx, starts, lens, n_ranges, s, l, &total)) return rc;
    const Camera cam = make_camera(ctx, M, scale_factor);
    double ms_draw = 0.0, ms_resolve = 0.0;
    const int rc = render_surface(ctx, cam, density_cut, s.data(), l.data(), (int)s.size(), total, clear, &ms_draw, &ms_resolve);
    if (rc) return rc;
    ctx->C = 2;
    ctx->image_source = W_NONE;
    ctx->surface_keys = true;
    ctx->image_is_reduced = false;
    ctx->stats.ms_stream = ms_draw;
    ctx->stats.ms_mid = ms_resolve;
    ctx->stats.ms_total = ms_draw + ms_resolve;
    if (gpu_ms_out) *gpu_ms_out = ms_draw + ms_resolve;
    return TSP_OK;
}

static int check_surface_params(const tsp_context *ctx, const tsp_surface_params *params, bool shading) {
    TSP_REQUIRE(ctx->C == 2, TSP_EINVAL, "surface presentation needs a 2-channel (q, depth) image, the active one has %d", ctx->C);
    TSP_REQUIRE(std::isfinite(params->smoothing_scale), TSP_EINVAL, "smoothing_scale must be finite");
    TSP_REQUIRE(!shading || !params->weighted_average || (params->lut_rgba && params->n_lut >= 2 && params->n_lut <= 65536),
                TSP_EINVAL, "weighted_average needs a colormap LUT of 2 to 65536 entries");
    return TSP_OK;
}

int tsp_surface_present(tsp_context *ctx, const tsp_surface_params *params, float *content_out, uint8_t *rgba8_out,
                        double *ms_out) {
    TSP_REQUIRE(ctx && params, TSP_EINVAL, "NULL argument");
    if (int rc = check_surface_params(ctx, params, rgba8_out != nullptr)) return rc;
    TSP_HIP(hipSetDevice(ctx->device));
    return surface_present(ctx, *params, content_out, rgba8_out, ms_out);
}

static int check_surface_frame(const tsp_context *ctx, const tsp_surface_params *params) {
    if (int rc = check_surface_params(ctx, params, true)) return rc;
    bool ok = std::isfinite(params->depth_scale);
    for (int k = 0; k < 3; ++k)
        ok = ok && std::isfinite(params->light_direction[k]) && std::isfinite(params->light_color[k]) &&
             std::isfinite(params->ambient_color[k]);
    TSP_REQUIRE(ok, TSP_EINVAL, "depth_scale, light_direction, light_color and ambient_color must be finite");
    TSP_REQUIRE(!params->weighted_average || (std::isfinite(params->vmin) && std::isfinite(params->vmax)), TSP_EINVAL,
                "the material range [vmin, vmax] must be finite");
    return TSP_OK;
}

int tsp_present_surface(tsp_context *ctx, int width, int height, const tsp_surface_params *params, const tsp_present_layer *layers,
                        int n_layers, uint8_t *out_rgba8, double *ms_out) {
    TSP_REQUIRE(ctx && params && out_rgba8, TSP_EINVAL, "NULL argument");
    if (int rc = check_surface_frame(ctx, params)) return rc;
    return present_surface(ctx, width, height, *params, layers, n_layers, out_rgba8, ms_out, false);
}

int tsp_present_surface_yuv420(tsp_context *ctx, int width, int height, const tsp_surface_params *params,
                               const tsp_present_layer *layers, int n_layers, uint8_t *out, double *ms_out) {
    TSP_REQUIRE(ctx && params && out, TSP_EINVAL, "NULL argument");
    if (int rc = check_surface_frame(ctx, params)) return rc;
    return present_surface(ctx, width, height, *params, layers, n_layers, out, ms_out, true);
}

int tsp_get_stats(tsp_context *ctx, tsp_stats *out) {
    TSP_REQUIRE(ctx && out, TSP_EINVAL, "NULL argument");
    *out = ctx->stats;
    return TSP_OK;
}

int tsp_set_option(tsp_context *ctx, const char *name, int64_t value) {
    TSP_REQUIRE(ctx && name, TSP_EINVAL, "NULL argument");
    if (!strcmp(name, "count_fragments")) {
        ctx->count_fragments = value != 0;
        return TSP_OK;
    }
    if (!strcmp(name, "p_small_milli")) {
        TSP_REQUIRE(value >= 0 && value <= 16000, TSP_EINVAL, "p_small out of range (kernel S packs <= 16 texel columns per footprint)");
        ctx->p_small = (float)value * 1e-3f;
        return TSP_OK;
    }
    if (!strcmp(name, "debug_no_raster")) {
        ctx->debug_no_raster = value != 0;
        return TSP_OK;
    }
    if (!strcmp(name, "huge_split") || !strcmp(name, "stream_blocks_per_cu")) {
        TSP_REQUIRE(value >= 0 && value <= 4096, TSP_EINVAL, "%s out of range", name);
        if (name[0] == 'h') ctx->huge_split = (int)value;
        else ctx->stream_blocks_per_cu = (int)value;
        return TSP_OK;
    }
    if (!strcmp(name, "slice_records")) {
        TSP_REQUIRE(value == 0 || (value >= 64 && value <= (1ll << 27)), TSP_EINVAL, "%s: 0 or 64 .. 2^27", name);
        ctx->slice_records = value;
        return TSP_OK;
    }
    if (!strcmp(name, "debug_fail_stage")) {
        TSP_REQUIRE(value >= 0 && value <= 2, TSP_EINVAL, "%s out of range", name);
        ctx->debug_fail_stage = (int)value;
        return TSP_OK;
    }
    if (!strcmp(name, "debug_fail_alloc")) {
        TSP_REQUIRE(value >= 0, TSP_EINVAL, "%s out of range", name);
        ctx->debug_fail_alloc = value;
        return TSP_OK;
    }
    if (!strcmp(name, "debug_gather_full_lut")) { ctx->debug_gather_full_lut = value ? 1 : 0; return TSP_OK; }
    if (!strcmp(name, "mid_item_scale_milli")) {
        TSP_REQUIRE(value >= 1 && value <= 100000, TSP_EINVAL, "%s out of range", name);
        ctx->mid_item_scale = (double)value * 1e-3;
        return TSP_OK;
    }
    if (!strcmp(name, "mid_narrow_px_milli")) {
        TSP_REQUIRE(value >= 0 && value <= 64000, TSP_EINVAL, "%s out of range", name);
        ctx->mid_narrow_px = (float)value * 1e-3f;
        return TSP_OK;
    }
    if (!strcmp(name, "mid_item_records")) {
        TSP_REQUIRE(value == 0 || (value >= 64 && value <= 8192 && (value & (value - 1)) == 0), TSP_EINVAL, "%s: 0 or a power of two from 64 to 8192", name);
        ctx->mid_item_records = (int)value;
        return TSP_OK;
    }
    if (!strcmp(name, "stream_batch_chunks")) {
        TSP_REQUIRE(value >= 4 && value <= 4096, TSP_EINVAL, "%s out of range", name);
        ctx->stream_batch_chunks = (int)value;
        return TSP_OK;
    }
    if (!strcmp(name, "huge_band_mib")) {
        TSP_REQUIRE(value >= 0 && value <= (1 << 20), TSP_EINVAL, "%s out of range", name);
        ctx->huge_band_budget = value << 20;
        return TSP_OK;
    }
    if (!strcmp(name, "huge_variant")) {
        TSP_REQUIRE(value >= 1 && value <= 7 && value != 3, TSP_EINVAL, "huge_variant out of range");
        ctx->huge_variant = (int)value;
        return TSP_OK;
    }
    if (!strcmp(name, "h2_walk")) {
        TSP_REQUIRE(value == 0 || value == 1, TSP_EINVAL, "%s out of range", name);
        ctx->h2_walk = (int)value;
        return TSP_OK;
    }
    if (!strcmp(name, "reorder_interleave")) {
        TSP_REQUIRE(value >= 0 && value <= 2, TSP_EINVAL, "%s out of range", name);
        ctx->reorder_interleave = (int)value;
        return TSP_OK;
    }
    if (!strcmp(name, "chunk_cull")) {
        ctx->chunk_cull = value != 0;
        return TSP_OK;
    }
    if (!strcmp(name, "overlap_mid_huge")) {
        ctx->overlap_mid_huge = value != 0;
        return TSP_OK;
    }
    if (!strcmp(name, "use_quantity")) {
        ctx->use_quantity = value != 0;
        return TSP_OK;
    }
    if (!strcmp(name, "active_channels")) {
        TSP_REQUIRE((value == 2 || value == 4) && value <= ctx->Ccap, TSP_EINVAL, "bad channel count %lld", (long long)value);
        ctx->C = (int)value;
        ctx->forget_render_undo();
        return TSP_OK;
    }
    set_error("unknown option '%s'", name);
    return TSP_EINVAL;
}

int tsp_measure_read_bandwidth(tsp_context *ctx, int64_t bytes, int iters, double *gbps_out) {
    TSP_REQUIRE(ctx && gbps_out && bytes > 0 && iters > 0, TSP_EINVAL, "bad argument");
    TSP_HIP(hipSetDevice(ctx->device));
    return measure_read_bandwidth(ctx, bytes, iters, gbps_out);
}

}
```

### topsy_amd/csrc/tsp_group.hip

```cpp
#include <algorithm>
#include <string>
#include <thread>
#include <vector>

#include "tsp_internal.h"

struct tsp_group {
    std::vector<tsp_context *> ctx;
    std::vector<int64_t> bounds;
    bool rccl = false;
    bool needs_reduce = false;
    int R = 0, Ccap = 0;
};

namespace {

using tsp::set_error;

template <typename F> int for_each_context(tsp_group *grp, F fn) {
    const int G = (int)grp->ctx.size();
    std::vector<int> rc(G, TSP_OK);
    std::vector<std::string> msg(G);
    std::vector<std::thread> th;
    th.reserve(G);
// ... 92 lines not shown
    return for_each_context(grp, [&](int g) {
        const int64_t a = grp->bounds[g], len = grp->bounds[g + 1] - a;
        return tsp_upload_particles(grp->ctx[g], len, x + a, y + a, z + a, h + a, mass ? mass + a : nullptr);
    });
}

int tsp_group_upload_quantity(tsp_group *grp, const float *q) {
    TSP_REQUIRE(grp, TSP_EINVAL, "NULL group");
    return for_each_context(grp, [&](int g) {
        if (q && grp->bounds[g + 1] == grp->bounds[g]) return (int)TSP_OK;
        return tsp_upload_quantity(grp->ctx[g], q ? q + grp->bounds[g] : nullptr);
    });
}

int tsp_group_upload_rgb(tsp_group *grp, const float *r, const float *g_, const float *b) {
    TSP_REQUIRE(grp && r && g_ && b, TSP_EINVAL, "NULL argument");
    return for_each_context(grp, [&](int g) {
        const int64_t a = grp->bounds[g];
        if (grp->bounds[g + 1] == a) return (int)TSP_OK;
        return tsp_upload_rgb(grp->ctx[g], r + a, g_ + a, b + a);
    });
}

int tsp_group_generate_synthetic(tsp_group *grp, int64_t n_total, int64_t first, int64_t count, uint64_t seed, float h_cap,
                                 int with_quantity, int with_rgb) {
    TSP_REQUIRE(grp, TSP_EINVAL, "NULL group");
    TSP_REQUIRE(count >= 0, TSP_EINVAL, "negative particle count");
    set_bounds(grp, count);
    return for_each_context(grp, [&](int g) {
        const int64_t a = grp->bounds[g], len = grp->bounds[g + 1] - a;
        return tsp_generate_synthetic(grp->ctx[g], n_total, first + a, len, seed, h_cap, with_quantity, with_rgb);
    });
}

int tsp_group_reorder_spatial(tsp_group *grp, int n_strata, uint64_t seed) {
    TSP_REQUIRE(grp, TSP_EINVAL, "NULL group");
    const int G = (int)grp->ctx.size();
    const int per = std::max(1, (n_strata + G - 1) / G);
    return for_each_context(grp, [&](int g) {
        if (grp->bounds[g + 1] == grp->bounds[g]) return (int)TSP_OK;
        return tsp_reorder_spatial(grp->ctx[g], per, seed, nullptr);
    });
}

int64_t tsp_group_num_particles(tsp_group *grp) { return grp ? grp->bounds.back() : 0; }

int tsp_group_set_option(tsp_group *grp, const char *name, int64_t value) {
    TSP_REQUIRE(grp && name, TSP_EINVAL, "NULL argument");
    return for_each_context(grp, [&](int g) { return tsp_set_option(grp->ctx[g], name, value); });
}

int tsp_group_render(tsp_group *grp, const float *M, float scale_factor, const int64_t *starts, const int64_t *lens, int n_ranges,
                     int clear, int mode, int flags, double *gpu_ms_out) {
    TSP_REQUIRE(grp && M, TSP_EINVAL, "NULL argument");
    TSP_REQUIRE(n_ranges >= 0 && (n_ranges == 0 || (starts && lens) || (!starts && !lens)), TSP_EINVAL, "bad ranges");
    const int G = (int)grp->ctx.size();
    const int64_t all_start = 0, all_len = grp->bounds.back();
    if (!starts) { starts = &all_start; lens = &all_len; n_ranges = 1; }
    for (int i = 0; i < n_ranges; ++i) TSP_REQUIRE(lens[i] >= 0, TSP_EINVAL, "range %d has negative length %lld", i, (long long)lens[i]);
    std::vector<double> ms(G, 0.0);
    const int rc = for_each_context(grp, [&](int g) {
        const int64_t a = grp->bounds[g], b = grp->bounds[g + 1];
        std::vector<int64_t> s, l;
        const int64_t n = grp->bounds.back();
        for (int i = 0; i < n_ranges; ++i) {
            int64_t r0 = starts[i], len = lens[i];
            if (r0 < 0) { len = (len > -r0) ? len + r0 : 0; r0 = 0; }
            if (r0 >= n || len == 0) continue;
            if (len > n - r0) len = n - r0;
            const int64_t lo = std::max(r0, a), hi = std::min(r0 + len, b);
            if (hi > lo) { s.push_back(lo - a); l.push_back(hi - lo); }
        }
        if (s.empty()) { s.push_back(0); l.push_back(0); }
        return tsp_render(grp->ctx[g], M, scale_factor, s.data(), l.data(), (int)s.size(), clear, mode, flags, &ms[g]);
    });
    if (rc) {
        const std::string why = tsp_last_error();
        std::string undo_error;
        for (int g = 0; g < G; ++g)
            if (grp->ctx[g]->undo.kind != 0 && tsp_render_undo(grp->ctx[g]) != TSP_OK)
                undo_error += std::string("; and context ") + std::to_string(g) + " could not be put back (" + tsp_last_error() + ")";
        if (!grp->ctx[0]->image_is_reduced) grp->needs_reduce = true;
        set_error("%s%s", why.c_str(), undo_error.c_str());
        return rc;
    }
    grp->needs_reduce = true;
    if (gpu_ms_out) *gpu_ms_out = *std::max_element(ms.begin(), ms.end());
    return TSP_OK;
}

int tsp_group_end_frame(tsp_group *grp, double *ms_out) {
    TSP_REQUIRE(grp, TSP_EINVAL, "NULL group");
    if (ms_out) *ms_out = 0.0;
    if (!grp->needs_reduce || grp->ctx.size() == 1) { grp->needs_reduce = false; return TSP_OK; }
    const int G = (int)grp->ctx.size();
    for (int g = 0; g < G; ++g) {
        const tsp_context *c = grp->ctx[g];
        TSP_REQUIRE(c->C == grp->ctx[0]->C, TSP_ESTATE, "context %d holds a %d-channel image, context 0 a %d-channel one", g, c->C, grp->ctx[0]->C);
        TSP_REQUIRE(!c->image_is_reduced, TSP_ESTATE, "context %d was already reduced for this frame", g);
        TSP_REQUIRE(!grp->rccl || c->comm, TSP_ESTATE, "context %d has lost its communicator", g);
    }
    grp->needs_reduce = false;
    if (grp->rccl) {
        std::vector<double> ms(G, 0.0);
        const int rc = for_each_context(grp, [&](int g) { return tsp_comm_reduce_image(grp->ctx[g], 0, &ms[g]); });
        if (rc) return rc;
        if (ms_out) *ms_out = *std::max_element(ms.begin(), ms.end());
        return TSP_OK;
    }
    const size_t count = (size_t)grp->R * grp->R * grp->ctx[0]->C;
    std::vector<std::vector<float>> part(G, std::vector<float>(count));
    int rc = for_each_context(grp, [&](int g) { return tsp_read_image(grp->ctx[g], part[g].data()); });
    if (rc) return rc;
    std::vector<float> sum(part[0]);
    for (int g = 1; g < G; ++g)
        for (size_t i = 0; i < count; ++i) sum[i] += part[g][i];
    return tsp_set_reduced_image(grp->ctx[0], sum.data());
}

int tsp_group_shard_range(tsp_group *grp, int index, int64_t *first_out, int64_t *count_out) {
    TSP_REQUIRE(grp && first_out && count_out, TSP_EINVAL, "NULL argument");
    TSP_REQUIRE(index >= 0 && index < (int)grp->ctx.size(), TSP_EINVAL, "shard %d of %d", index, (int)grp->ctx.size());
    *first_out = grp->bounds[index];
    *count_out = grp->bounds[index + 1] - grp->bounds[index];
    return TSP_OK;
}

int tsp_group_upload_band_magnitudes(tsp_group *grp, int n_bands, const double *mags, const double *weights) {
    TSP_REQUIRE(grp && mags && weights, TSP_EINVAL, "NULL argument");
    TSP_REQUIRE(n_bands >= 1 && n_bands <= 64, TSP_EINVAL, "n_bands %d out of range", n_bands);
    const int64_t n = grp->bounds.back();
    return for_each_context(grp, [&](int g) {
        const int64_t a = grp->bounds[g], len = grp->bounds[g + 1] - a;
        if (len == 0) return (int)TSP_OK;
        std::vector<double> cut((size_t)n_bands * len);
        for (int k = 0; k < n_bands; ++k) std::copy(mags + (size_t)k * n + a, mags + (size_t)k * n + a + len, cut.begin() + (size_t)k * len);
        return tsp_upload_band_magnitudes(grp->ctx[g], n_bands, cut.data(), weights);
    });
}

int tsp_group_get_stats(tsp_group *grp, tsp_stats *out) {
    TSP_REQUIRE(grp && out, TSP_EINVAL, "NULL argument");
    tsp_stats t = {};
    for (tsp_context *c : grp->ctx) {
        tsp_stats s;
        const int rc = tsp_get_stats(c, &s);
        if (rc) return rc;
        t.n_particles += s.n_particles; t.n_small += s.n_small; t.n_mid += s.n_mid; t.n_huge += s.n_huge; t.n_culled += s.n_culled;
        t.n_fragments += s.n_fragments; t.n_mega += s.n_mega;
        t.n_fragments_stream += s.n_fragments_stream; t.n_fragments_mid += s.n_fragments_mid;
        t.n_fragments_huge += s.n_fragments_huge; t.n_fragments_mega += s.n_fragments_mega; t.n_chunk_culled += s.n_chunk_culled;
        t.ms_stream = std::max(t.ms_stream, s.ms_stream); t.ms_mid = std::max(t.ms_mid, s.ms_mid);
        t.ms_huge = std::max(t.ms_huge, s.ms_huge); t.ms_mega = std::max(t.ms_mega, s.ms_mega);
        t.ms_total = std::max(t.ms_total, s.ms_total);
    }
    *out = t;
    return TSP_OK;
}

}
```

### topsy_amd/csrc/tsp_internal.h

```cpp
#pragma once
#include <hip/hip_runtime.h>
#include <stdint.h>

#include <initializer_list>
#include <vector>
#include <stdio.h>
#include <string>

#include "../../include/topsy_splat.h"
#include "tsp_math.h"

namespace tsp {

void set_error(const char *fmt, ...);

#define TSP_HIP(call)                                                                          \
    do {                                                                                       \
        hipError_t e_ = (call);                                                                \
        if (e_ != hipSuccess) {                                                                \
            tsp::set_error("%s failed: %s (%s:%d)", #call, hipGetErrorString(e_), __FILE__, __LINE__); \
            return TSP_EHIP;                                                                   \
        }                                                                                      \
    } while (0)

#define TSP_REQUIRE(cond, code, ...)       \
    do {                                   \
        if (!(cond)) {                     \
            tsp::set_error(__VA_ARGS__);   \
            return (code);                 \
        }                                  \
    } while (0)

struct Particles {
    int64_t n = 0;
    float *x = nullptr, *y = nullptr, *z = nullptr, *h = nullptr, *m = nullptr;
    float *q = nullptr;
    float *r = nullptr, *g = nullptr, *b = nullptr;
    float *vx = nullptr, *vy = nullptr, *vz = nullptr;
    uint32_t *perm = nullptr;
    float *wm = nullptr;
    float *wr = nullptr, *wg = nullptr, *wb = nullptr;
    bool wm_valid = false;
    int wrgb_source = 0;
};
enum { W_NONE = 0, W_RGB = 1, W_KINEMATIC = 2 };

constexpr int BOUNDS_BLOCK = 512;

struct Record {
    float pcx, pcy, P, w0, w1;
};
struct Record4 {
    float pcx, pcy, P, w0, w1, w2;
};

struct Counters {
    unsigned long long n_small, n_mid, n_huge, n_culled, n_fragments, huge_count, next_chunk, mid_odd_weights;
    unsigned long long n_frag_class[4];
};

struct Workspace {
    void *mid_geom = nullptr, *mid_w = nullptr;
    int64_t mid_capacity = 0;
    void *huge_geom = nullptr, *huge_w = nullptr;
    int64_t huge_capacity = 0;
    void *hband_geom = nullptr, *hband_w = nullptr;
    int *hband_count = nullptr;
    int64_t hband_stride = 0; int hband_bands = 0;
    void *mband_geom = nullptr, *mband_w = nullptr;
    int *mband_count = nullptr;
    long long *mband_base = nullptr;
    int64_t mband_capacity = 0;
    int mtile_capacity = 0;
    int64_t mitem_capacity = 0;
    int *mitem_tile = nullptr, *mitem_base = nullptr;
    int64_t chunk_capacity = 0;
    float4 *block_bounds = nullptr;
    int64_t bounds_capacity = 0;
    bool bounds_valid = false;
    int *alive_list = nullptr;
    unsigned long long *cull_info = nullptr;
    int64_t *range_prefix = nullptr;
    int64_t range_capacity = 0;
    int *count_diff = nullptr;
    int *count_band = nullptr;
    int count_R = 0;
};

enum {
    EV_RENDER_BEGIN, EV_RENDER_END,
    EV_S_BEGIN, EV_S_END,
    EV_MID_BEGIN, EV_MID_END,
    EV_BLOCK_END,
    EV_CULL_BEGIN,
    EV_S_DONE,
    EV_HUGE_BEGIN, EV_HUGE_END,
    EV_COUNT,
    EV_T0 = 0, EV_T1, EV_T2, EV_T3, EV_T4, EV_T5
};
constexpr uint32_t attr_bit_stream(int mode) { return 1u << mode; }
constexpr uint32_t attr_bit_bins(int nw) { return 1u << (8 + nw); }

}

struct tsp_context {
    int device = 0;
    int R = 0, C = 0, Ccap = 0;
    bool use_quantity = true;
    hipStream_t stream = nullptr;
    hipStream_t stream2 = nullptr;
    hipEvent_t ev[tsp::EV_COUNT] = {};
    float *image = nullptr;
    double *image64 = nullptr;
    double *image64_entry = nullptr;
    float *mips = nullptr;
    bool have_mips = false;
    bool have_sphere_mips = false;
    bool surface_keys = false;
    bool lut_mirror_symmetric = false;
    bool lut_zero_outside_disc = false;
    tsp::Particles p;
    tsp::Counters *counters = nullptr;
    tsp::Workspace ws;
    uint8_t *out8 = nullptr;
    float *outf = nullptr;
    float *lut = nullptr;
    int lut_capacity = 0;
    float *lut2d = nullptr;
    int lut2d_n = 0;
    void *scratch = nullptr;
    size_t scratch_bytes = 0;
    uint32_t *sort_keys = nullptr, *sort_keys_alt = nullptr;
    void *sort_tmp = nullptr;
    size_t sort_tmp_bytes = 0;
    int64_t sort_capacity = 0, sorted_count = 0;
    int64_t sorted_neg_inf = 0;
    tsp_stats stats = {};
    std::vector<int64_t> cell_offsets;
    int cell_bits = 0;
    float cell_lo[3] = {0, 0, 0}, cell_width[3] = {0, 0, 0};
    std::vector<int64_t> strata_offsets;
    uint32_t kernel_attr_done = 0;
    bool count_fragments = false;
    float p_small = 16.0f;
    int64_t huge_band_budget = 6ll << 30;
    int huge_variant = 1;
    int h2_walk = 1;
    int huge_split = 0;
    int reorder_interleave = 2;
    int stream_blocks_per_cu = 0;
    int debug_gather_full_lut = 0;
    double mid_item_scale = 0.35;
    float mid_narrow_px = 64.0f;
    int mid_item_records = 0;
    int stream_batch_chunks = 8;
    bool chunk_cull = true;
    int64_t chunk_culled_particles = 0;
    bool overlap_mid_huge = false;
    int64_t slice_records = 0;
    int debug_fail_stage = 0;
    int64_t debug_fail_alloc = 0;
    int stream_occ[3][2] = {};
    bool debug_no_raster = false;
    int cu_count = 256;
    void *comm = nullptr;
    int n_ranks = 1, rank = 0;
    bool image_is_reduced = false;
    bool have_los = false;
    float los[6] = {};
    float w_los[6] = {};
    int image_source = tsp::W_NONE;
    float image_los[6] = {};
    bool kinematic_block = false;
    struct RenderUndo {
        int kind = 0;
        int C = 0;
        tsp_stats stats = {};
        int64_t chunk_culled_particles = 0;
        int image_source = tsp::W_NONE;
        float image_los[6] = {};
    } undo;
    void forget_render_undo() { undo.kind = 0; }
};

namespace tsp {
struct DeviceScratch {
    void *p = nullptr;
    DeviceScratch() = default;
    DeviceScratch(const DeviceScratch &) = delete;
    DeviceScratch &operator=(const DeviceScratch &) = delete;
    ~DeviceScratch() { if (p) (void)hipFree(p); }
    template <typename T> T *as() const { return static_cast<T *>(p); }
    void *release() { void *q = p; p = nullptr; return q; }
    void reset(void *q) { if (p) (void)hipFree(p); p = q; }
};
int scratch_alloc(tsp_context *ctx, const char *site, DeviceScratch &buf, size_t bytes);
#define TSP_SCRATCH_ALLOC(ctx, site, buf, bytes)                                     \
    do {                                                                             \
        const int rc_ = tsp::scratch_alloc((ctx), (site), (buf), (size_t)(bytes));   \
        if (rc_ != TSP_OK) return rc_;                                               \
    } while (0)

#define SITE(name) name
struct DeviceBuffer {
    const char *site;
    void **p;
    size_t bytes;
};
struct Capacity {
    int64_t *c64 = nullptr; int *c32 = nullptr; size_t *csz = nullptr;
    int64_t value = 0;
    Capacity(int64_t *c, int64_t v) : c64(c), value(v) {}
    Capacity(int *c, int64_t v) : c32(c), value(v) {}
    Capacity(size_t *c, int64_t v) : csz(c), value(v) {}
    void set(int64_t v) const {
        if (c64) *c64 = v;
        else if (c32) *c32 = (int)v;
        else *csz = (size_t)v;
    }
};
int alloc_group(tsp_context *ctx, std::initializer_list<DeviceBuffer> bufs, std::initializer_list<Capacity> caps);

int check_workspace(const tsp_context *ctx);

int launch_generic(tsp_context *ctx, const Camera &cam, const int64_t *d_ranges, int n_ranges,
                   int64_t total, int mode, int rule);
int launch_pipeline(tsp_context *ctx, const Camera &cam, const int64_t *h_starts, const int64_t *h_lens,
                    int n_ranges, int64_t total, int mode);
int launch_colormap_scalar(tsp_context *ctx, const float *d_img, int64_t npix, int C, const float *d_lut,
                           int n_lut, float vmin, float vmax, int log_scale, int weighted, uint8_t *d_out);
int launch_colormap_rgb(tsp_context *ctx, const float *d_img, int64_t npix, int C, float vmin, float vmax,
                        float gamma, uint8_t *d_out8, float *d_outf);
int launch_colormap_bivariate(tsp_context *ctx, const float *d_img, int64_t npix, int C, float vmin, float vmax,
                             float dvmin, float dvmax, int log_scale, int weighted, uint8_t *d_out);
int generate_synthetic(tsp_context *ctx, int64_t n_total, int64_t first, int64_t count, uint64_t seed,
                       float h_cap, int with_quantity, int with_rgb);
int reorder_spatial(tsp_context *ctx, int n_strata, uint64_t seed, int64_t *perm_out);
int ensure_weights(tsp_context *ctx, bool rgb);
int launch_kinematic_weights(tsp_context *ctx);
int launch_velocity_moments(tsp_context *ctx, const float *d_img, int64_t npix, float *d_maps);
int ensure_block_bounds(tsp_context *ctx);
int measure_read_bandwidth(tsp_context *ctx, int64_t bytes, int iters, double *gbps_out);
int launch_image_convert(tsp_context *ctx, bool to_float);
int tile_periodic(tsp_context *ctx, int n, const float *h_offsets, const float *h_weights);
int moment_sort(tsp_context *ctx, int which, int absolute, int64_t *n_finite);
int content_sort(tsp_context *ctx, int kind, float scale, int64_t *n_finite, int64_t *n_nonpositive);
int ensure_array(float **p, int64_t n);
int smoothing_lengths(tsp_context *ctx, int64_t n, const float *x, const float *y, const float *z, int k, float period,
                      float *h_out);
int sph_sum(tsp_context *ctx, int64_t n, const float *x, const float *y, const float *z, const float *h, const float *a,
            float period, float *out);
int fof_groups(tsp_context *ctx, int64_t n, const float *x, const float *y, const float *z, float linking_length, float period,
               int64_t min_members, int32_t *group_out, tsp_fof_info *info_out);
int shrink_sphere_center(tsp_context *ctx, int64_t n, const float *x, const float *y, const float *z, const float *mass,
                         float mass_cut_factor, double r_start, double shrink_factor, int64_t min_particles, int max_iterations,
                         double center_out[3], tsp_center_info *info_out);
int sphere_moments(tsp_context *ctx, int64_t n, const float *x, const float *y, const float *z, const float *mass, const float *vx,
                   const float *vy, const float *vz, const double center[3], double r, double r_vel, tsp_moments *out);
int radial_profile(tsp_context *ctx, int64_t n, const float *x, const float *y, const float *z, const float *mass, const float *vx,
                   const float *vy, const float *vz, const tsp_profile_spec *spec, int64_t *count_out, double *sums_out,
                   tsp_profile_info *info_out);
int render_surface(tsp_context *ctx, const Camera &cam, float cut, const int64_t *h_starts, const int64_t *h_lens,
                   int n_ranges, int64_t total, int clear, double *ms_draw, double *ms_resolve);
int density_order_stats(tsp_context *ctx, const int64_t *ranks, int n_ranks, float *values_out);
int surface_present(tsp_context *ctx, const tsp_surface_params &prm, float *content_out, uint8_t *rgba8_out, double *ms_out);
int launch_bilateral(tsp_context *ctx, double smoothing_scale, float2 *filtered);
ShadeParams shade_params(const tsp_surface_params &prm, int width);
int present(tsp_context *ctx, int W, int H, const tsp_present_base &base, const tsp_present_layer *layers, int n_layers, void *out,
            double *gpu_ms_out, bool yuv420);
int present_surface(tsp_context *ctx, int W, int H, const tsp_surface_params &prm, const tsp_present_layer *layers, int n_layers,
                    void *out, double *ms_out, bool yuv420);
}
```

### topsy_amd/csrc/tsp_mid.hip

```cpp
#include <algorithm>
#include <cmath>

#include "tsp_pipeline.h"

namespace tsp {

#ifndef TSP_G_OCC1
#define TSP_G_OCC1 8
#define TSP_G_HR1 32
#define TSP_G_OCC2 8
#define TSP_G_OCC3 5
#endif
constexpr int GCHUNK_MAX = 1024;
#ifndef TSP_BIN_PER
#define TSP_BIN_PER 4
#endif
constexpr int G_WIN_TILES = 4096;
constexpr int G_LDS_TILES = 16384;

template <int MODE, int NACC, int HR, int OCC, bool QUAD, bool CNT>
__global__ __launch_bounds__(H2T, OCC) void splat_mid_gather_kernel(TileArgs a) {
    constexpr int C = (MODE == TSP_MODE_RGB) ? 4 : 2;
    constexpr int NW = (MODE == TSP_MODE_RGB) ? 2 : 1;
    constexpr int NG = HR / 4;
// ... 343 lines not shown
struct TileSpan { int x0, x1, y0, y1; };
struct BinArgs {
    int R, tw, th, tiles_x, tiles_y;
    float pmin, pmax;
    float disc_k2;
    int exact;
    int narrow;
    int win_rows;
};
__device__ __forceinline__ TileSpan tile_span(const float4 g, const BinArgs &b) {
    TileSpan s; s.x0 = s.y0 = 1; s.x1 = s.y1 = 0;
    if (!(g.z >= b.pmin && g.z < b.pmax)) return s;
    const float half = 0.5f * g.z, mx = bin_margin(g.x, half), my = bin_margin(g.y, half);
    const float xl = g.x - half - mx, xh = g.x + half + mx, yl = g.y - half - my, yh = g.y + half + my;
    if (xh >= 0.0f && xl < (float)b.R && yh >= 0.0f && yl < (float)b.R && xl == xl && xh == xh && yl == yl && yh == yh) {
        s.x0 = max(0, (int)__builtin_floorf(fmaxf(xl, 0.0f) / (float)b.tw));
        s.x1 = min(b.tiles_x - 1, (int)__builtin_floorf(fminf(xh, (float)b.R) / (float)b.tw));
        s.y0 = max(0, (int)__builtin_floorf(fmaxf(yl, 0.0f) / (float)b.th));
        s.y1 = min(b.tiles_y - 1, (int)__builtin_floorf(fminf(yh, (float)b.R) / (float)b.th));
    }
    return s;
}
__device__ __forceinline__ bool strip_hit(const float4 g, int tx, int ty, const BinArgs &b) {
    if (!b.exact) return true;
    return reaches_strip(g, (float)(tx * b.tw), (float)(tx * b.tw + b.tw), (float)(ty * b.th), (float)(ty * b.th + b.th), b.disc_k2);
}
__global__ __launch_bounds__(256) void tile_count_kernel(const float4 *__restrict__ geom, long long n, BinArgs b, int *__restrict__ tile_count) {
    constexpr int PER = TSP_BIN_PER;
    extern __shared__ int s_tile[];
    const int tiles_x = b.tiles_x;
    const int row0 = (int)blockIdx.y * b.win_rows, row1 = min(b.tiles_y, row0 + b.win_rows) - 1, t0 = row0 * tiles_x, n_win = (row1 - row0 + 1) * tiles_x;
    const bool lds = n_win <= G_LDS_TILES;
    if (lds) {
        for (int t = threadIdx.x; t < n_win; t += 256) s_tile[t] = 0;
        __syncthreads();
    }
    int *cnt = lds ? s_tile : tile_count + t0;
    const long long first = ((long long)blockIdx.x * 256 + threadIdx.x) * PER;
#pragma unroll
    for (int k = 0; k < PER; ++k) {
        if (first + k >= n) continue;
        const float4 g = geom[first + k];
        const TileSpan sp = tile_span(g, b);
        for (int ty = max(sp.y0, row0); ty <= min(sp.y1, row1); ++ty)
            for (int tx = sp.x0; tx <= sp.x1; ++tx)
                if (strip_hit(g, tx, ty, b)) atomicAdd(&cnt[ty * tiles_x + tx - t0], 1);
    }
    if (lds) {
        __syncthreads();
        for (int t = threadIdx.x; t < n_win; t += 256)
            if (s_tile[t]) atomicAdd(&tile_count[t0 + t], s_tile[t]);
    }
}
__global__ __launch_bounds__(1024) void tile_prefix_kernel(const int *__restrict__ tile_count, int n_tiles, long long *__restrict__ tile_base,
                                                           int *__restrict__ item_base, int *__restrict__ item_tile, int item_capacity, int item_records) {
    __shared__ long long s_rec[1024];
    __shared__ int s_item[1024];
    __shared__ long long s_carry_rec;
    __shared__ int s_carry_item;
    const int tid = threadIdx.x;
    if (tid == 0) { s_carry_rec = 0; s_carry_item = 0; }
    __syncthreads();
    for (int base = 0; base < n_tiles; base += 1024) {
        const int t = base + tid;
        const int c = t < n_tiles ? tile_count[t] : 0;
        const int it = (c + item_records - 1) / item_records;
        s_rec[tid] = c; s_item[tid] = it;
        __syncthreads();
        for (int o = 1; o < 1024; o <<= 1) {
            const long long vr = tid >= o ? s_rec[tid - o] : 0;
            const int vi = tid >= o ? s_item[tid - o] : 0;
            __syncthreads();
            s_rec[tid] += vr; s_item[tid] += vi;
            __syncthreads();
        }
        const long long rec0 = s_carry_rec + s_rec[tid] - c;
        const int item0 = s_carry_item + s_item[tid] - it;
        if (t < n_tiles) {
            tile_base[t] = rec0; item_base[t] = item0;
            for (int i = 0; item_tile && i < it; ++i)
                if ( item0 + i < item_capacity) item_tile[item0 + i] = t;
        }
        __syncthreads();
        if (tid == 1023) { s_carry_rec += s_rec[1023]; s_carry_item += s_item[1023]; }
        __syncthreads();
    }
    if (tid == 0) { tile_base[n_tiles] = s_carry_rec; item_base[n_tiles] = s_carry_item; }
}
template <int NW>
__global__ __launch_bounds__(256) void tile_fill_kernel(const float4 *__restrict__ geom, const float *__restrict__ w, long long n, BinArgs b,
                                                        float4 *__restrict__ out_geom, float *__restrict__ out_w,
                                                        const long long *__restrict__ tile_base, int *__restrict__ tile_cursor,
                                                        unsigned long long *__restrict__ odd_flag) {
    constexpr int PER = TSP_BIN_PER;
    extern __shared__ int s_tile[];
    const int tiles_x = b.tiles_x;
    const int row0 = (int)blockIdx.y * b.win_rows, row1 = min(b.tiles_y, row0 + b.win_rows) - 1, t0 = row0 * tiles_x, n_win = (row1 - row0 + 1) * tiles_x;
    const bool lds = n_win <= G_LDS_TILES;
    int *s_cnt = s_tile, *s_base = s_tile + n_win;
    if (lds) {
        for (int t = threadIdx.x; t < n_win; t += 256) s_cnt[t] = 0;
        __syncthreads();
    }
    const long long first = ((long long)blockIdx.x * 256 + threadIdx.x) * PER;
    float4 g[PER];
    TileSpan sp[PER];
#pragma unroll
    for (int k = 0; k < PER; ++k) {
        sp[k].x0 = sp[k].y0 = 1; sp[k].x1 = sp[k].y1 = 0;
        if (first + k < n) {
            g[k] = geom[first + k];
            sp[k] = tile_span(g[k], b);
            sp[k].y0 = max(sp[k].y0, row0); sp[k].y1 = min(sp[k].y1, row1);
            if (lds)
                for (int ty = sp[k].y0; ty <= sp[k].y1; ++ty)
                    for (int tx = sp[k].x0; tx <= sp[k].x1; ++tx)
                        if (strip_hit(g[k], tx, ty, b)) atomicAdd(&s_cnt[ty * tiles_x + tx - t0], 1);
        }
    }
    if (lds) {
        __syncthreads();
        for (int t = threadIdx.x; t < n_win; t += 256) {
            const int c = s_cnt[t];
            s_base[t] = c ? atomicAdd(&tile_cursor[t0 + t], c) : 0;
            s_cnt[t] = 0;
        }
        __syncthreads();
    }
#pragma unroll
    for (int k = 0; k < PER; ++k) {
        if (first + k >= n || sp[k].y0 > sp[k].y1 || sp[k].x0 > sp[k].x1) continue;
        const float w0 = w[(first + k) * NW], w1 = (NW == 2) ? w[(first + k) * NW + 1] : 0.0f;
        const float4 gn = make_float4(g[k].x, g[k].y, g[k].z, 1.0f / g[k].z);
        if (b.narrow && odd_flag && !(__builtin_fabsf(g[k].w) < __builtin_inff() && __builtin_fabsf(w0) < __builtin_inff() && __builtin_fabsf(w1) < __builtin_inff()))
            *odd_flag = 1ull;
        for (int ty = sp[k].y0; ty <= sp[k].y1; ++ty)
            for (int tx = sp[k].x0; tx <= sp[k].x1; ++tx) {
                if (!strip_hit(g[k], tx, ty, b)) continue;
                const int t = ty * tiles_x + tx;
                const long long slot = tile_base[t] + (lds ? s_base[t - t0] + atomicAdd(&s_cnt[t - t0], 1) : atomicAdd(&tile_cursor[t], 1));
                if (b.narrow) {
                    out_geom[slot] = gn;
                    if (NW == 2) reinterpret_cast<float4 *>(out_w)[slot] = make_float4(g[k].w, w0, w1, 0.0f);
                    else reinterpret_cast<float2 *>(out_w)[slot] = make_float2(g[k].w, w0);
                } else {
                    out_geom[slot] = g[k];
                    out_w[slot * NW] = w0;
                    if (NW == 2) out_w[slot * NW + 1] = w1;
                }
            }
    }
}

template <int NW>
static int bin_mid_records(tsp_context *ctx, TileArgs &ta, const float4 *mid_geom, const float *mid_w, long long n_mid, int tw, int th, float pmin,
                           float pmax, bool exact, int *n_items_out, hipStream_t st) {
    Workspace &ws = ctx->ws;
    const int tiles_x = (ctx->R + tw - 1) / tw, tiles_y = (ctx->R + th - 1) / th, n_tiles = tiles_x * tiles_y;
    BinArgs ba;
    ba.R = ctx->R; ba.tw = tw; ba.th = th; ba.tiles_x = tiles_x; ba.tiles_y = tiles_y; ba.pmin = pmin; ba.pmax = pmax;
    ba.disc_k2 = ta.disc_k2; ba.exact = exact ? 1 : 0; ba.narrow = exact ? 1 : 0;
    ba.win_rows = std::max(1, G_WIN_TILES / tiles_x);
    const int n_win = (tiles_y + ba.win_rows - 1) / ba.win_rows, win_tiles = std::min(tiles_y, ba.win_rows) * tiles_x;
    int rc;
    if (ws.mtile_capacity < n_tiles) {
        if ((rc = alloc_group(ctx, {{"mband_count", (void **)&ws.mband_count, 2 * (size_t)n_tiles * sizeof(int)},
                                    {"mband_base", (void **)&ws.mband_base, ((size_t)n_tiles + 1) * sizeof(long long)},
                                    {"mitem_base", (void **)&ws.mitem_base, ((size_t)n_tiles + 1) * sizeof(int)}},
                              {{&ws.mtile_capacity, n_tiles}})))
            return rc;
    }
    if ((rc = check_workspace(ctx))) return rc;
    int item_records = ctx->mid_item_records;
    if (item_records <= 0) {
        const double want = ctx->mid_item_scale * std::sqrt((double)n_mid);
        item_records = 64;
        while (item_records < GCHUNK_MAX && (double)item_records * 1.41 < want) item_records *= 2;
    }
    TSP_HIP(hipMemsetAsync(ws.mband_count, 0, 2 * (size_t)ws.mtile_capacity * sizeof(int), st));
    const bool lds = win_tiles <= G_LDS_TILES;
    if (!(ctx->kernel_attr_done & attr_bit_bins(NW))) {
        TSP_HIP(hipFuncSetAttribute((const void *)tile_count_kernel, hipFuncAttributeMaxDynamicSharedMemorySize, G_LDS_TILES * (int)sizeof(int)));
        TSP_HIP(hipFuncSetAttribute((const void *)tile_fill_kernel<NW>, hipFuncAttributeMaxDynamicSharedMemorySize, 2 * G_LDS_TILES * (int)sizeof(int)));
        ctx->kernel_attr_done |= attr_bit_bins(NW);
    }
    const unsigned grid = (unsigned)((n_mid + 256 * TSP_BIN_PER - 1) / (256 * TSP_BIN_PER));
    hipLaunchKernelGGL(tile_count_kernel, dim3(grid, n_win), dim3(256), lds ? win_tiles * sizeof(int) : 0, st, mid_geom, n_mid, ba, ws.mband_count);
    hipLaunchKernelGGL(tile_prefix_kernel, dim3(1), dim3(1024), 0, st, (const int *)ws.mband_count, n_tiles, ws.mband_base, ws.mitem_base, (int *)nullptr, 0, item_records);
    long long total_records = 0; int total_items = 0;
    TSP_HIP(hipMemcpyAsync(&total_records, ws.mband_base + n_tiles, sizeof(long long), hipMemcpyDeviceToHost, st));
    TSP_HIP(hipMemcpyAsync(&total_items, ws.mitem_base + n_tiles, sizeof(int), hipMemcpyDeviceToHost, st));
    TSP_HIP(hipStreamSynchronize(st));
    if (ws.mband_capacity < total_records || ws.mitem_capacity < total_items) {
        const int64_t rec_cap = std::max<int64_t>(ws.mband_capacity, total_records + total_records / 4 + 1024);
        const int64_t item_cap = std::max<int64_t>(ws.mitem_capacity, (int64_t)total_items + total_items / 4 + 1024);
        if ((rc = alloc_group(ctx, {{"mband_geom", &ws.mband_geom, (size_t)rec_cap * sizeof(float4)},
                                    {"mband_w", &ws.mband_w, (size_t)rec_cap * 4 * sizeof(float)},
                                    {"mitem_tile", (void **)&ws.mitem_tile, (size_t)item_cap * sizeof(int)}},
                              {{&ws.mband_capacity, rec_cap}, {&ws.mitem_capacity, item_cap}})))
            return rc;
    }
    if ((rc = check_workspace(ctx))) return rc;
    hipLaunchKernelGGL(tile_prefix_kernel, dim3(1), dim3(1024), 0, st, (const int *)ws.mband_count, n_tiles, ws.mband_base, ws.mitem_base, ws.mitem_tile, total_items, item_records);
    hipLaunchKernelGGL((tile_fill_kernel<NW>), dim3(grid, n_win), dim3(256), lds ? 2 * win_tiles * sizeof(int) : 0, st, mid_geom, mid_w, n_mid, ba,
                       (float4 *)ws.mband_geom, (float *)ws.mband_w, (const long long *)ws.mband_base, ws.mband_count + ws.mtile_capacity,
                       &ctx->counters->mid_odd_weights);
    TSP_HIP(hipGetLastError());
    ta.geom = (const float4 *)ws.mband_geom; ta.w = (const float *)ws.mband_w;
    ta.bin_count = ws.mband_count; ta.band_stride = 0; ta.bin_base = ws.mband_base;
    ta.item_tile = ws.mitem_tile; ta.item_base = ws.mitem_base; ta.n_tiles = n_tiles; ta.item_records = item_records;
    ta.tiles_x = tiles_x;
    *n_items_out = total_items;
    return TSP_OK;
}

struct KernelG {
    static constexpr int STRIP_W = 64;
    static constexpr bool EXACT_BINS = false;
    static size_t lds_bytes(bool quad, int ) { return (size_t)(quad ? MIPQ_TOTAL : MIP_TOTAL) * sizeof(float) + (H2T / 64) * 64 * sizeof(int); }
    template <int MODE, int NACC, int HR, int OCC, bool QUAD, bool CNT> static constexpr auto kernel() { return splat_mid_gather_kernel<MODE, NACC, HR, OCC, QUAD, CNT>; }
};
struct KernelN {
    static constexpr int STRIP_W = NSW;
    static constexpr bool EXACT_BINS = true;
    static size_t lds_bytes(bool quad, int HR) { return (size_t)(quad ? NQ_LINES * 32 : MIP_TOTAL + 64) * sizeof(float) + (H2T / 64) * 4 * HR * sizeof(int); }
    template <int MODE, int NACC, int HR, int OCC, bool QUAD, bool CNT> static constexpr auto kernel() { return splat_narrow_gather_kernel<MODE, NACC, HR, OCC, QUAD, CNT>; }
};

template <class K, int MODE, int NACC, int HR, int OCC>
static int launch_strip_kernel(tsp_context *ctx, TileArgs ta, const float4 *mid_geom, const float *mid_w, long long n_mid, float pmin, float pmax, hipStream_t st) {
    const bool quad = ctx->lut_mirror_symmetric && !ctx->debug_gather_full_lut;
    int rc, n_items = 0;
    ta.n_records = n_mid;
    if ((rc = bin_mid_records<(MODE == TSP_MODE_RGB) ? 2 : 1>(ctx, ta, mid_geom, mid_w, n_mid, K::STRIP_W, HR, pmin, pmax, K::EXACT_BINS, &n_items, st))) return rc;
    if (n_items == 0) return TSP_OK;
    const dim3 grid((n_items + H2T / 64 - 1) / (H2T / 64));
    with_bool(quad, [&](auto Q) { with_bool(ta.count_frag != 0, [&](auto CNT) {
        hipLaunchKernelGGL((K::template kernel<MODE, NACC, HR, OCC, decltype(Q)::value, decltype(CNT)::value>()), grid, dim3(H2T), K::lds_bytes(quad, HR), st, ta);
    }); });
    TSP_HIP(hipGetLastError());
    return TSP_OK;
}
template <class K, int MODE>
static int launch_strip_kernel_mode(tsp_context *ctx, TileArgs ta, bool second_channel, const float4 *mid_geom, const float *mid_w, long long n_mid, float pmin, float pmax, hipStream_t st) {
    if (MODE == TSP_MODE_RGB) return launch_strip_kernel<K, MODE, 3, 16, TSP_G_OCC3>(ctx, ta, mid_geom, mid_w, n_mid, pmin, pmax, st);
    if (second_channel) return launch_strip_kernel<K, MODE, 2, 16, TSP_G_OCC2>(ctx, ta, mid_geom, mid_w, n_mid, pmin, pmax, st);
    return launch_strip_kernel<K, MODE, 1, TSP_G_HR1, TSP_G_OCC1>(ctx, ta, mid_geom, mid_w, n_mid, pmin, pmax, st);
}

template <int MODE>
static int launch_mid_gather_mode(tsp_context *ctx, TileArgs ta, bool second_channel, const float4 *mid_geom, const float *mid_w, long long n_mid, hipStream_t st) {
    TSP_REQUIRE(n_mid < (1ll << 28), TSP_EINVAL, "%lld mid footprints in one launch (kernel G indexes its work items with 32 bits; run_pipeline slices the list)", n_mid);
    const float split = ctx->mid_narrow_px;
    if (split > 0.0f) {
        if (int rc = launch_strip_kernel_mode<KernelN, MODE>(ctx, ta, second_channel, mid_geom, mid_w, n_mid, 0.0f, split, st)) return rc;
        if (split >= P_BILINEAR) return TSP_OK;
    }
    return launch_strip_kernel_mode<KernelG, MODE>(ctx, ta, second_channel, mid_geom, mid_w, n_mid, split, __builtin_inff(), st);
}

int launch_mid_gather(tsp_context *ctx, TileArgs ta, int mode, bool second_channel, const float4 *mid_geom, const float *mid_w,
                      long long n_mid, hipStream_t st) {
    return with_mode(mode, [&](auto M) {
        constexpr int MODE = decltype(M)::value;
        return launch_mid_gather_mode<MODE>(ctx, ta, MODE != TSP_MODE_WEIGHTED || second_channel, mid_geom, mid_w, n_mid, st);
    });
}

}
```

### topsy_amd/csrc/tsp_pipeline.h

```cpp
#pragma once
#include <type_traits>

#include "tsp_internal.h"

namespace tsp {


#ifndef TSP_S_BLOCK
#define TSP_S_BLOCK 256
#endif
#ifndef TSP_S_KPT
#define TSP_S_KPT 2
#endif
constexpr int SBLOCK = TSP_S_BLOCK;
constexpr int SWAVES = SBLOCK / 64;
constexpr int KPT = TSP_S_KPT;
constexpr int CHUNK = SBLOCK * KPT;
#ifndef TSP_WIN1
#define TSP_WIN1 60
#define TSP_WIN2 44
#define TSP_WIN4 40
#endif
#ifndef TSP_S_OCC
#define TSP_S_OCC 5
#endif
template <int WC> struct WinSize { static constexpr int value = (WC == 1) ? TSP_WIN1 : (WC == 2 ? TSP_WIN2 : TSP_WIN4); };

constexpr int HBAND_H = 64;

enum { CLS_NONE = 0, CLS_SMALL = 1, CLS_MID = 2, CLS_HUGE = 3 };

__device__ __forceinline__ void gatomic_add(double *addr, double v) {
#ifdef TSP_DEBUG_NO_FLUSH
    if (v == 123.456) *addr = v;
#else
    __hip_atomic_fetch_add(addr, v, __ATOMIC_RELAXED, __HIP_MEMORY_SCOPE_AGENT);
#endif
}
constexpr int MIPQ_TOTAL = 1024 + 256 + 64 + 16;
__device__ __forceinline__ int mipq_offset(int lvl) { return lvl == 0 ? 0 : (lvl == 1 ? 1024 : (lvl == 2 ? 1280 : 1344)); }

#define TSP_DPP_QUAD(t) "quad_perm:[" #t "," #t "," #t "," #t "] row_mask:0xf bank_mask:0xf"
template <int T> __device__ __forceinline__ void fmac_quad(float &acc, float rowval, float v) {
    static_assert(T >= 0 && T < 4, "quad lane");
    if (T == 0) asm volatile("v_fmac_f32_dpp %0, %1, %2 " TSP_DPP_QUAD(0) : "+v"(acc) : "v"(rowval), "v"(v));
    if (T == 1) asm volatile("v_fmac_f32_dpp %0, %1, %2 " TSP_DPP_QUAD(1) : "+v"(acc) : "v"(rowval), "v"(v));
    if (T == 2) asm volatile("v_fmac_f32_dpp %0, %1, %2 " TSP_DPP_QUAD(2) : "+v"(acc) : "v"(rowval), "v"(v));
    if (T == 3) asm volatile("v_fmac_f32_dpp %0, %1, %2 " TSP_DPP_QUAD(3) : "+v"(acc) : "v"(rowval), "v"(v));
}
template <int T> __device__ __forceinline__ float mul_quad(float rowval, float v) {
    float r;
    if (T == 0) asm volatile("v_mul_f32_dpp %0, %1, %2 " TSP_DPP_QUAD(0) : "=v"(r) : "v"(rowval), "v"(v));
    if (T == 1) asm volatile("v_mul_f32_dpp %0, %1, %2 " TSP_DPP_QUAD(1) : "=v"(r) : "v"(rowval), "v"(v));
    if (T == 2) asm volatile("v_mul_f32_dpp %0, %1, %2 " TSP_DPP_QUAD(2) : "=v"(r) : "v"(rowval), "v"(v));
    if (T == 3) asm volatile("v_mul_f32_dpp %0, %1, %2 " TSP_DPP_QUAD(3) : "=v"(r) : "v"(rowval), "v"(v));
    return r;
}
__device__ __forceinline__ void fmac_plain(float &acc, float x, float y) {
    asm volatile("v_fmac_f32_e32 %0, %1, %2" : "+v"(acc) : "v"(x), "v"(y));
}

__device__ __forceinline__ bool reaches_strip(const float4 g, float sx0, float sx1, float sy0, float sy1, float disc_k2) {
    const float half = 0.5f * g.z;
    const float sdx = fmaxf(fmaxf(sx0 - g.x, g.x - sx1), 0.0f), sdy = fmaxf(fmaxf(sy0 - g.y, g.y - sy1), 0.0f);
    return g.z > 0.0f && sdx < half && sdy < half && !(disc_k2 > 0.0f && sdx * sdx + sdy * sdy >= disc_k2 * g.z * g.z);
}
__device__ __forceinline__ float bin_margin(float c, float half) { return 1.0f + 2.4e-7f * (__builtin_fabsf(c) + half); }

constexpr int H2T = 256;

__device__ __forceinline__ void latomic_add(double *addr, float v) {
    __hip_atomic_fetch_add(addr, (double)v, __ATOMIC_RELAXED, __HIP_MEMORY_SCOPE_WORKGROUP);
}

#ifndef TSP_FOLD_EVERY
#define TSP_FOLD_EVERY 2048
#endif
#ifndef TSP_HDEAL
#define TSP_HDEAL 16
#endif
constexpr int HDEAL = TSP_HDEAL;

struct TileArgs {
    const float4 *geom; const float *w;
    long long n_records;
    Camera cam;
    const float *mips;
    double *img;
    Counters *cnt;
    int tiles_x, split;
    int count_frag;
    float disc_k2;
    const int *bin_count; long long band_stride; const long long *bin_base;
    int n_tiles; const int *item_tile; const int *item_base; int item_records;
};

template <bool BUILT = true, class F> auto with_bool(bool b, F &&f) {
    if constexpr (BUILT) { if (b) return f(std::true_type{}); }
    return f(std::false_type{});
}
template <class F> int with_mode(int mode, F &&f) {
    switch (mode) {
        case TSP_MODE_WEIGHTED: return f(std::integral_constant<int, TSP_MODE_WEIGHTED>{});
        case TSP_MODE_DEPTH: return f(std::integral_constant<int, TSP_MODE_DEPTH>{});
        case TSP_MODE_RGB: return f(std::integral_constant<int, TSP_MODE_RGB>{});
    }
    set_error("bad mode %d", mode);
    return TSP_EINVAL;
}

int launch_gather_kernels(tsp_context *ctx, TileArgs ta, int mode, bool second_channel, const float4 *huge_geom, const float *huge_w,
                          long long n_huge);

int launch_mid_gather(tsp_context *ctx, TileArgs ta, int mode, bool second_channel, const float4 *mid_geom, const float *mid_w,
                      long long n_mid, hipStream_t st);

}
```

### topsy_amd/csrc/tsp_pipeline.hip

```cpp
#include <string.h>

#include <algorithm>
#include <type_traits>
#include <vector>

#include "tsp_pipeline.h"

namespace tsp {

template <int CTRL, int ROW_MASK> __device__ __forceinline__ int dpp_or(int identity, int v) {
    return __builtin_amdgcn_update_dpp(identity, v, CTRL, ROW_MASK, 0xf, false);
}
template <typename Op> __device__ __forceinline__ int wave_scan_bits(int v, int identity, Op op) {
    v = op(v, dpp_or<0x111, 0xf>(identity, v));
    v = op(v, dpp_or<0x112, 0xf>(identity, v));
    v = op(v, dpp_or<0x114, 0xf>(identity, v));
    v = op(v, dpp_or<0x118, 0xf>(identity, v));
    v = op(v, dpp_or<0x142, 0xa>(identity, v));
    v = op(v, dpp_or<0x143, 0xc>(identity, v));
    return v;
}
__device__ __forceinline__ float wave_min(float v) {
    const int r = wave_scan_bits(__float_as_int(v), __float_as_int(__builtin_inff()),
                                 [](int a, int b) { return __float_as_int(fminf(__int_as_float(a), __int_as_float(b))); });
// ... 484 lines not shown
                    if (g == 2 || nc <= 4) {
                        if (nc <= 2) group(g, std::integral_constant<int, 2>());
                        else group(g, std::integral_constant<int, 4>());
                    } else group(g, std::integral_constant<int, 6>());
                }
            }
            if (act) {
                ++n_small;
                if (count_frag) n_frag += (unsigned long long)(nx * ny);
            }
        }

        if (tid == 0) {
            s_base[0] = r_mid; s_base[1] = r_huge;
            if (grab) s_batch = (int)r_batch;
        }
        __syncthreads();
        if (grab) {
            CArgs *ap = KA();
            const int n_todo = list_size(), start = (int)gridDim.x * ap->chunks_per_block + s_batch;
            if (start < n_todo) { n0 = start; n1 = min(start + grab, n_todo); }
        }
        const long long mid_base = s_base[0], huge_base = s_base[1];
        {
            CArgs *ap = KA();
            float4 *const mid_geom = ap->mid_geom, *const huge_geom = ap->huge_geom;
            float *const mid_w = ap->mid_w, *const huge_w = ap->huge_w;
            const long long mid_capacity = ap->mid_capacity, huge_capacity = ap->huge_capacity;
            long long mpos = mid_base + mid_before + (mid_incl - my_mid);
            long long hpos = huge_base + huge_before + (huge_incl - my_huge);
#pragma unroll
            for (int k = 0; k < KPT; ++k) {
                if (cls[k] == CLS_MID) {
                    if (mpos < mid_capacity) {
                        mid_geom[mpos] = make_float4(pcx[k], pcy[k], PP[k], w0[k]);
                        mid_w[mpos * NW] = w1[k];
                        if (NW == 2) mid_w[mpos * NW + 1] = w2[k];
                    }
                    ++mpos;
                } else if (cls[k] == CLS_HUGE) {
                    if (hpos < huge_capacity) {
                        huge_geom[hpos] = make_float4(pcx[k], pcy[k], PP[k], w0[k]);
                        huge_w[hpos * NW] = w1[k];
                        if (NW == 2) huge_w[hpos * NW + 1] = w2[k];
                    }
                    ++hpos;
                }
            }
        }
        if (c_next == NO_CHUNK) break;
        first = first_next; cnt = cnt_next;
        batch_head = false;
        if (c + 1 == b1) { b0 = n0; b1 = n1; n0 = n1 = NO_CHUNK; batch_head = true; }
        c = c_next;
    }
    __syncthreads();
    flush();
    for (int o = 32; o; o >>= 1) {
        n_small += __shfl_xor((long long)n_small, o);
        n_cull += __shfl_xor((long long)n_cull, o);
        n_frag += __shfl_xor((long long)n_frag, o);
    }
    if (lane == 0) {
        Counters *cntp = KA()->cnt;
        if (n_small) atomicAdd(&cntp->n_small, n_small);
        if (n_cull) atomicAdd(&cntp->n_culled, n_cull);
        if (n_frag) { atomicAdd(&cntp->n_fragments, n_frag); atomicAdd(&cntp->n_frag_class[0], n_frag); }
#ifdef TSP_S_DEBUG
        if (dbg_slots) atomicAdd(&cntp->n_frag_class[1], dbg_slots);
#endif
    }
}

__global__ __launch_bounds__(256) void rect_count_corners_kernel(const float4 *__restrict__ geom, long long n, int R, int *__restrict__ D) {
    const long long i = (long long)blockIdx.x * 256 + threadIdx.x;
    if (i >= n) return;
    const float4 g = geom[i];
    const float half = 0.5f * __builtin_fabsf(g.z);
    int ilo, ihi, jlo, jhi;
    cover_range(g.x, half, R, ilo, ihi);
    cover_range(g.y, half, R, jlo, jhi);
    if (ilo > ihi || jlo > jhi) return;
    const int S = R + 1;
    atomicAdd(&D[jlo * S + ilo], 1);
    atomicAdd(&D[jlo * S + ihi + 1], -1);
    atomicAdd(&D[(jhi + 1) * S + ilo], -1);
    atomicAdd(&D[(jhi + 1) * S + ihi + 1], 1);
}

__global__ __launch_bounds__(256) void count_row_scan_kernel(int *__restrict__ D, int R) {
    __shared__ int part[256];
    const int S = R + 1, tid = threadIdx.x;
    int *row = D + (size_t)blockIdx.x * S;
    const int per = (S + 255) / 256, b = tid * per, e = min(b + per, S);
    int sum = 0;
    for (int i = b; i < e; ++i) sum += row[i];
    part[tid] = sum;
    __syncthreads();
    for (int o = 1; o < 256; o <<= 1) {
        const int v = tid >= o ? part[tid - o] : 0;
        __syncthreads();
        part[tid] += v;
        __syncthreads();
    }
    int run = part[tid] - sum;
    for (int i = b; i < e; ++i) { run += row[i]; row[i] = run; }
}

constexpr int CBAND = 64;
__global__ __launch_bounds__(256) void count_band_sum_kernel(const int *__restrict__ D, int R, int *__restrict__ band) {
    const int i = blockIdx.x * 256 + threadIdx.x, bnd = blockIdx.y;
    if (i >= R) return;
    const int S = R + 1, j0 = bnd * CBAND, j1 = min(j0 + CBAND, R);
    int sum = 0;
    for (int j = j0; j < j1; ++j) sum += D[(size_t)j * S + i];
    band[(size_t)bnd * R + i] = sum;
}
__global__ __launch_bounds__(256) void count_apply_kernel(const int *__restrict__ D, const int *__restrict__ band, int R, double *__restrict__ img) {
    const int i = blockIdx.x * 256 + threadIdx.x, bnd = blockIdx.y;
    if (i >= R) return;
    const int S = R + 1, j0 = bnd * CBAND, j1 = min(j0 + CBAND, R);
    long long run = 0;
    for (int b = 0; b < bnd; ++b) run += band[(size_t)b * R + i];
    for (int j = j0; j < j1; ++j) {
        run += D[(size_t)j * S + i];
        if (run != 0) img[((size_t)j * R + i) * 4 + 3] += (double)run;
    }
}

static int add_rect_counts(tsp_context *ctx, const float4 *mid_geom, long long n_mid, const float4 *huge_geom, long long n_huge) {
    Workspace &ws = ctx->ws;
    const int R = ctx->R, S = R + 1, nb = (R + CBAND - 1) / CBAND;
    if (ws.count_R != R) {
        const int rc = alloc_group(ctx, {{"count_diff", (void **)&ws.count_diff, (size_t)S * S * sizeof(int)},
                                         {"count_band", (void **)&ws.count_band, (size_t)nb * R * sizeof(int)}}, {{&ws.count_R, R}});
        if (rc) return rc;
    }
    hipStream_t st = ctx->stream;
    TSP_HIP(hipMemsetAsync(ws.count_diff, 0, (size_t)S * S * sizeof(int), st));
    if (n_mid > 0) hipLaunchKernelGGL(rect_count_corners_kernel, dim3((unsigned)((n_mid + 255) / 256)), dim3(256), 0, st, mid_geom, n_mid, R, ws.count_diff);
    if (n_huge > 0) hipLaunchKernelGGL(rect_count_corners_kernel, dim3((unsigned)((n_huge + 255) / 256)), dim3(256), 0, st, huge_geom, n_huge, R, ws.count_diff);
    hipLaunchKernelGGL(count_row_scan_kernel, dim3(R), dim3(256), 0, st, ws.count_diff, R);
    hipLaunchKernelGGL(count_band_sum_kernel, dim3((R + 255) / 256, nb), dim3(256), 0, st, ws.count_diff, R, ws.count_band);
    hipLaunchKernelGGL(count_apply_kernel, dim3((R + 255) / 256, nb), dim3(256), 0, st, ws.count_diff, ws.count_band, R, ctx->image64);
    TSP_HIP(hipGetLastError());
    return TSP_OK;
}

static int alloc_list(tsp_context *ctx, void **geom, void **w, int64_t *cap, int64_t need, const char *geom_site, const char *w_site) {
    return alloc_group(ctx, {{geom_site, geom, (size_t)need * sizeof(float4)}, {w_site, w, (size_t)need * 2 * sizeof(float)}}, {{cap, need}});
}

template <int MODE>
static int run_pipeline(tsp_context *ctx, const Camera &cam, const int64_t *h_starts, const int64_t *h_lens, int n_ranges,
                        int64_t total) {
    constexpr int C = (MODE == TSP_MODE_RGB) ? 4 : 2;
    Workspace &ws = ctx->ws;
    hipStream_t st = ctx->stream;

    std::vector<int64_t> pack(3 * (size_t)n_ranges + 1);
    int64_t n_chunks64 = 0;
    for (int i = 0; i < n_ranges; ++i) {
        pack[i] = h_starts[i];
        pack[n_ranges + i] = h_lens[i];
        pack[2 * n_ranges + i] = n_chunks64;
        n_chunks64 += (h_lens[i] + CHUNK - 1) / CHUNK;
    }
    pack[3 * n_ranges] = n_chunks64;
    TSP_REQUIRE(n_chunks64 < (1ll << 30), TSP_EINVAL, "too many chunks");
    const int n_chunks = (int)n_chunks64;
    int rc;
    if ((rc = check_workspace(ctx))) return rc;
    if (ws.range_capacity < (int64_t)pack.size()) {
        const int64_t cap = (int64_t)pack.size() * 2 + 64;
        if ((rc = alloc_group(ctx, {{"range_prefix", (void **)&ws.range_prefix, (size_t)cap * sizeof(int64_t)}}, {{&ws.range_capacity, cap}}))) return rc;
    }
    TSP_HIP(hipMemcpyAsync(ws.range_prefix, pack.data(), pack.size() * sizeof(int64_t), hipMemcpyHostToDevice, st));
    if (ws.chunk_capacity < n_chunks) {
        const int64_t cap = (int64_t)n_chunks + n_chunks / 4 + 64;
        if ((rc = alloc_group(ctx, {{"alive_list", (void **)&ws.alive_list, (size_t)(cap + cap / 256 + 2) * sizeof(int)}}, {{&ws.chunk_capacity, cap}})))
            return rc;
    }
    if ((rc = ensure_weights(ctx, MODE == TSP_MODE_RGB))) return rc;
    if (ws.mid_capacity == 0 && (rc = alloc_list(ctx, &ws.mid_geom, &ws.mid_w, &ws.mid_capacity, std::max<int64_t>(total / 4, 1 << 16),
                                                 SITE("mid_geom"), SITE("mid_w"))))
        return rc;
    if (ws.huge_capacity == 0 && (rc = alloc_list(ctx, &ws.huge_geom, &ws.huge_w, &ws.huge_capacity, std::max<int64_t>(total / 16, 1 << 16),
                                                  SITE("huge_geom"), SITE("huge_w"))))
        return rc;

    Particles parts = ctx->p;
    if (!ctx->use_quantity) parts.q = nullptr;
    const bool second_channel = (MODE == TSP_MODE_DEPTH) || (MODE == TSP_MODE_RGB) || (ctx->p.q != nullptr && ctx->use_quantity);
    const int WCr = (MODE == TSP_MODE_RGB) ? 4 : (second_channel ? 2 : 1);
    const int WIN = (WCr == 1) ? WinSize<1>::value : WinSize<C>::value;
    const size_t smem_s = (size_t)WCr * WIN * WIN * sizeof(double) + T23_FLOATS * sizeof(float);
    if (!(ctx->kernel_attr_done & attr_bit_stream(MODE))) {
        TSP_HIP(hipFuncSetAttribute((const void *)splat_stream_kernel<MODE, C>, hipFuncAttributeMaxDynamicSharedMemorySize, (int)((size_t)C * WinSize<C>::value * WinSize<C>::value * sizeof(double) + T23_FLOATS * sizeof(float))));
        TSP_HIP(hipFuncSetAttribute((const void *)splat_stream_kernel<MODE, 1>, hipFuncAttributeMaxDynamicSharedMemorySize, (int)((size_t)WinSize<1>::value * WinSize<1>::value * sizeof(double) + T23_FLOATS * sizeof(float))));
        ctx->kernel_attr_done |= attr_bit_stream(MODE);
    }

    const bool cull = ctx->chunk_cull && n_chunks >= 4096;
    unsigned long long cull_info_h[2] = {0, 0};
    ctx->chunk_culled_particles = 0;
    TSP_HIP(hipEventRecord(ctx->ev[EV_CULL_BEGIN], st));
    if (cull) {
        if ((rc = ensure_block_bounds(ctx))) return rc;
        if (!ws.cull_info && (rc = alloc_group(ctx, {{"cull_info", (void **)&ws.cull_info, 2 * sizeof(unsigned long long)}}, {}))) return rc;
        TSP_HIP(hipMemsetAsync(ws.cull_info, 0, 2 * sizeof(unsigned long long), st));
        CullArgs ca;
        ca.ranges = ws.range_prefix; ca.n_ranges = n_ranges; ca.n_chunks = n_chunks; ca.cam = cam;
        ca.bounds = ws.block_bounds; ca.n_particles = ctx->p.n; ca.alive = ws.alive_list; ca.info = ws.cull_info;
        ca.wg_count = ws.alive_list + ws.chunk_capacity;
        const int n_wg = (n_chunks + 255) / 256;
        hipLaunchKernelGGL(chunk_cull_kernel<0>, dim3(n_wg), dim3(256), 0, st, ca);
        hipLaunchKernelGGL(chunk_cull_scan_kernel, dim3(1), dim3(1024), 0, st, ca.wg_count, n_wg, ws.cull_info);
        hipLaunchKernelGGL(chunk_cull_kernel<1>, dim3(n_wg), dim3(256), 0, st, ca);
        TSP_HIP(hipGetLastError());
    }

    Counters hc, carry;
    memset(&carry, 0, sizeof(carry));
    for (int attempt = 0; attempt < 2; ++attempt) {
        StreamArgs sa;
        sa.p = parts;
        sa.alive = cull ? ws.alive_list : nullptr; sa.cull_info = ws.cull_info;
        sa.ranges = ws.range_prefix; sa.n_ranges = n_ranges; sa.n_chunks = n_chunks;
        const int min_cpb = std::max(1, std::min(8, n_chunks / (ctx->cu_count * 2)));
        int per_cu = ctx->stream_blocks_per_cu;
        if (per_cu <= 0) {
            int &occ = ctx->stream_occ[MODE][WCr == 1 ? 0 : 1];
            if (occ <= 0) {
                const void *fn = (WCr == 1) ? (const void *)splat_stream_kernel<MODE, 1> : (const void *)splat_stream_kernel<MODE, C>;
                if (hipOccupancyMaxActiveBlocksPerMultiprocessor(&occ, fn, SBLOCK, smem_s) != hipSuccess || occ <= 0) { (void)hipGetLastError(); occ = 4; }
            }
            per_cu = occ;
        }
        const int resident = ctx->cu_count * per_cu;
        sa.dynamic = (min_cpb >= 8 && n_chunks > resident * 8) ? 1 : 0;
        sa.chunks_per_block = sa.dynamic ? std::max(4, ctx->stream_batch_chunks) : min_cpb;
        const int grid_s = sa.dynamic ? resident : (n_chunks + sa.chunks_per_block - 1) / sa.chunks_per_block;
        sa.cam = cam; sa.mips = ctx->mips; sa.img = ctx->image64;
        sa.mid_geom = (float4 *)ws.mid_geom; sa.mid_w = (float *)ws.mid_w; sa.mid_capacity = ws.mid_capacity;
        sa.huge_geom = (float4 *)ws.huge_geom; sa.huge_w = (float *)ws.huge_w; sa.huge_capacity = ws.huge_capacity;
        sa.cnt = ctx->counters; sa.p_small = ctx->p_small;
        sa.count_frag = ctx->count_fragments ? 1 : 0;
        sa.emit_small = (attempt == 0 && !ctx->debug_no_raster) ? 1 : 0;
        TSP_HIP(hipEventRecord(ctx->ev[EV_S_BEGIN], st));
        if (WCr == 1) hipLaunchKernelGGL((splat_stream_kernel<MODE, 1>), dim3(grid_s), dim3(SBLOCK), smem_s, st, sa);
        else hipLaunchKernelGGL((splat_stream_kernel<MODE, C>), dim3(grid_s), dim3(SBLOCK), smem_s, st, sa);
        TSP_HIP(hipGetLastError());
        TSP_HIP(hipEventRecord(ctx->ev[EV_S_END], st));
        TSP_HIP(hipMemcpyAsync(&hc, ctx->counters, sizeof(hc), hipMemcpyDeviceToHost, st));
        if (cull && attempt == 0) TSP_HIP(hipMemcpyAsync(cull_info_h, ws.cull_info, sizeof(cull_info_h), hipMemcpyDeviceToHost, st));
        TSP_HIP(hipStreamSynchronize(st));
        ctx->chunk_culled_particles = (int64_t)cull_info_h[1];
        const bool mid_over = (int64_t)hc.n_mid > ws.mid_capacity, huge_over = (int64_t)hc.n_huge > ws.huge_capacity;
        if (!mid_over && !huge_over) break;
        TSP_REQUIRE(attempt == 0, TSP_ENOMEM, "record lists overflowed twice");
        if (mid_over && (rc = alloc_list(ctx, &ws.mid_geom, &ws.mid_w, &ws.mid_capacity, (int64_t)hc.n_mid + (int64_t)hc.n_mid / 8 + 1024,
                                         SITE("mid_geom_replay"), SITE("mid_w_replay"))))
            return rc;
        if (huge_over && (rc = alloc_list(ctx, &ws.huge_geom, &ws.huge_w, &ws.huge_capacity, (int64_t)hc.n_huge + (int64_t)hc.n_huge / 8 + 1024,
                                          SITE("huge_geom_replay"), SITE("huge_w_replay"))))
            return rc;
        TSP_HIP(hipMemsetAsync(ctx->counters, 0, sizeof(Counters), st));
        carry = hc;
    }

    if (carry.n_small || carry.n_fragments) {
        hc.n_small += carry.n_small;
        hc.n_fragments += carry.n_fragments;
        hc.n_frag_class[0] += carry.n_frag_class[0];
        TSP_HIP(hipMemcpyAsync(ctx->counters, &hc, sizeof(hc), hipMemcpyHostToDevice, st));
        TSP_HIP(hipStreamSynchronize(st));
    }
    TileArgs ta;
    ta.cam = cam; ta.mips = ctx->mips; ta.img = ctx->image64; ta.cnt = ctx->counters; ta.tiles_x = 0; ta.split = 1;
    ta.count_frag = ctx->count_fragments ? 1 : 0;
    ta.bin_count = nullptr; ta.band_stride = 0; ta.bin_base = nullptr; ta.n_tiles = 0; ta.item_tile = nullptr; ta.item_base = nullptr;
    ta.disc_k2 = (ctx->lut_zero_outside_disc && !ctx->count_fragments) ? 0.5235f * 0.5235f : 0.0f;
    hipStream_t st_mid = ctx->overlap_mid_huge ? ctx->stream2 : st;
    if (ctx->overlap_mid_huge) {
        TSP_HIP(hipEventRecord(ctx->ev[EV_S_DONE], st));
        TSP_HIP(hipStreamWaitEvent(st_mid, ctx->ev[EV_S_DONE], 0));
    }
    if ((rc = check_workspace(ctx))) return rc;
    if (ctx->debug_fail_stage == 1) { ctx->debug_fail_stage = 0; TSP_REQUIRE(false, TSP_ENOMEM, "injected failure after kernel S (debug_fail_stage)"); }
    constexpr int NWr = (MODE == TSP_MODE_RGB) ? 2 : 1;
    const long long n_mid = (long long)hc.n_mid, n_huge = (long long)hc.n_huge;
    const long long mid_slice = ctx->slice_records > 0 ? ctx->slice_records : (1ll << 27);
    const long long huge_slice = ctx->slice_records > 0 ? ctx->slice_records : (1ll << 30);
    const float4 *mid_geom = (const float4 *)ws.mid_geom, *huge_geom = (const float4 *)ws.huge_geom;
    const float *mid_w = (const float *)ws.mid_w, *huge_w = (const float *)ws.huge_w;
    TSP_HIP(hipEventRecord(ctx->ev[EV_MID_BEGIN], st_mid));
    for (long long o = 0; o < n_mid; o += mid_slice)
        if ((rc = launch_mid_gather(ctx, ta, MODE, second_channel, mid_geom + o, mid_w + o * NWr, std::min(mid_slice, n_mid - o), st_mid))) return rc;
    TSP_HIP(hipEventRecord(ctx->ev[EV_MID_END], st_mid));
    if (ctx->debug_fail_stage == 2) { ctx->debug_fail_stage = 0; TSP_REQUIRE(false, TSP_ENOMEM, "injected failure after kernel G (debug_fail_stage)"); }
    TSP_HIP(hipEventRecord(ctx->ev[EV_HUGE_BEGIN], st));
    TSP_HIP(hipEventRecord(ctx->ev[EV_HUGE_END], st));
    for (long long o = 0; o < n_huge; o += huge_slice)
        if ((rc = launch_gather_kernels(ctx, ta, MODE, second_channel, huge_geom + o, huge_w + o * NWr, std::min(huge_slice, n_huge - o)))) return rc;
    if (MODE == TSP_MODE_RGB && (n_mid > 0 || n_huge > 0)) {
        if (ctx->overlap_mid_huge) TSP_HIP(hipStreamWaitEvent(st, ctx->ev[EV_MID_END], 0));
        if (n_mid <= mid_slice && n_huge <= huge_slice) {
            if ((rc = add_rect_counts(ctx, mid_geom, n_mid, huge_geom, n_huge))) return rc;
        } else {
            for (long long o = 0; o < n_mid; o += mid_slice)
                if ((rc = add_rect_counts(ctx, mid_geom + o, std::min(mid_slice, n_mid - o), nullptr, 0))) return rc;
            for (long long o = 0; o < n_huge; o += huge_slice)
                if ((rc = add_rect_counts(ctx, nullptr, 0, huge_geom + o, std::min(huge_slice, n_huge - o)))) return rc;
        }
    }
    TSP_HIP(hipEventRecord(ctx->ev[EV_BLOCK_END], st));
    if (ctx->overlap_mid_huge) TSP_HIP(hipStreamWaitEvent(st, ctx->ev[EV_MID_END], 0));
    TSP_HIP(hipStreamSynchronize(st));
    float ms = 0.f;
    TSP_HIP(hipEventElapsedTime(&ms, ctx->ev[cull ? EV_CULL_BEGIN : EV_S_BEGIN], ctx->ev[EV_S_END])); ctx->stats.ms_stream = ms;
    TSP_HIP(hipEventElapsedTime(&ms, ctx->ev[EV_MID_BEGIN], ctx->ev[EV_MID_END])); ctx->stats.ms_mid = ms;
    TSP_HIP(hipEventElapsedTime(&ms, ctx->ev[EV_HUGE_BEGIN], ctx->ev[EV_HUGE_END])); ctx->stats.ms_huge = ms;
    ctx->stats.ms_mega = 0.0;
    return TSP_OK;
}

int launch_pipeline(tsp_context *ctx, const Camera &cam, const int64_t *h_starts, const int64_t *h_lens, int n_ranges,
                    int64_t total, int mode) {
    return with_mode(mode, [&](auto M) { return run_pipeline<decltype(M)::value>(ctx, cam, h_starts, h_lens, n_ranges, total); });
}

}
```

Baseline: 20.76 billion.

## Overlap mid-footprint binning with huge gather kernels on a second stream

Splits mid-footprint processing into count, prefix, fill and draw stages, then runs the first pass's binning on a high-priority second stream while the huge-footprint gather kernels run on the main stream. Events join the streams before the mid draw. This is on by default, unless the older mid/huge overlap option is set. The aim is to hide binning latency, including its host sync for the totals, behind the huge kernels. The cost is extra events, stream-priority setup and a changed order of accumulation, which could change rounding or cause contention.

After: 20.94 billion, median of 6. About the same (+0.9%).

```diff
diff --git a/include/topsy_splat.h b/include/topsy_splat.h
--- a/include/topsy_splat.h
+++ b/include/topsy_splat.h
@@ -70,6 +70,7 @@
 int tsp_render_undo(tsp_context *ctx);
 
 int tsp_read_image(tsp_context *ctx, float *out);
+int tsp_read_accumulator(tsp_context *ctx, double *out);
 int tsp_write_image(tsp_context *ctx, const float *in);
 
 int tsp_colormap_scalar(tsp_context *ctx, const float *lut_rgba, int n_lut, float vmin, float vmax,
@@ -224,6 +225,7 @@
     int64_t n_mega;
     int64_t n_fragments_stream, n_fragments_mid, n_fragments_huge, n_fragments_mega;
     int64_t n_chunk_culled;
+    double ms_mid_bin;
 } tsp_stats;
 int tsp_get_stats(tsp_context *ctx, tsp_stats *out);
 int tsp_set_option(tsp_context *ctx, const char *name, int64_t value);
diff --git a/topsy_amd/_native.py b/topsy_amd/_native.py
--- a/topsy_amd/_native.py
+++ b/topsy_amd/_native.py
@@ -88,7 +88,8 @@
                 ("ms_stream", ctypes.c_double), ("ms_mid", ctypes.c_double), ("ms_huge", ctypes.c_double),
                 ("ms_total", ctypes.c_double), ("ms_mega", ctypes.c_double), ("n_mega", ctypes.c_int64),
                 ("n_fragments_stream", ctypes.c_int64), ("n_fragments_mid", ctypes.c_int64),
-                ("n_fragments_huge", ctypes.c_int64), ("n_fragments_mega", ctypes.c_int64), ("n_chunk_culled", ctypes.c_int64)]
+                ("n_fragments_huge", ctypes.c_int64), ("n_fragments_mega", ctypes.c_int64), ("n_chunk_culled", ctypes.c_int64),
+                ("ms_mid_bin", ctypes.c_double)]
 
     def as_dict(self):
         return {k: getattr(self, k) for k, _ in self._fields_}
@@ -127,6 +128,7 @@
                                   ctypes.c_int, ctypes.POINTER(ctypes.c_double)]),
     "tsp_render_undo": (ctypes.c_int, [_ctx]),
     "tsp_read_image": (ctypes.c_int, [_ctx, _fp]),
+    "tsp_read_accumulator": (ctypes.c_int, [_ctx, ctypes.POINTER(ctypes.c_double)]),
     "tsp_write_image": (ctypes.c_int, [_ctx, _fp]),
     "tsp_colormap_scalar": (ctypes.c_int, [_ctx, _fp, ctypes.c_int, ctypes.c_float, ctypes.c_float, ctypes.c_int,
                                            ctypes.c_int, _u8p]),
@@ -402,6 +404,11 @@
         _check(self._lib.tsp_read_image(self._h, _ptr(out)))
         return out
 
+    def read_accumulator(self):
+        out = np.empty((self.resolution, self.resolution, self.active_channels), dtype=np.float64)
+        _check(self._lib.tsp_read_accumulator(self._h, out.ctypes.data_as(ctypes.POINTER(ctypes.c_double))))
+        return out
+
     def write_image(self, img):
         img = np.ascontiguousarray(img, dtype=np.float32)
         if img.shape[:2] != (self.resolution, self.resolution) or img.shape[2] not in (2, 4) or img.shape[2] > self.n_channels:
diff --git a/topsy_amd/csrc/tsp_api.hip b/topsy_amd/csrc/tsp_api.hip
--- a/topsy_amd/csrc/tsp_api.hip
+++ b/topsy_amd/csrc/tsp_api.hip
@@ -212,7 +212,7 @@
 extern "C" {
 
 const char *tsp_last_error(void) { return g_err; }
-int tsp_version(void) { return 119; }
+int tsp_version(void) { return 120; }
 int tsp_stats_size(void) { return (int)sizeof(tsp_stats); }
 
 int tsp_device_count(void) {
@@ -228,8 +228,10 @@
     hipDeviceProp_t prop;
     TSP_HIP(hipGetDeviceProperties(&prop, device_id));
     ctx->cu_count = prop.multiProcessorCount > 0 ? prop.multiProcessorCount : 256;
-    TSP_HIP(hipStreamCreateWithFlags(&ctx->stream, hipStreamNonBlocking));
-    TSP_HIP(hipStreamCreateWithFlags(&ctx->stream2, hipStreamNonBlocking));
+    int prio_low = 0, prio_high = 0;
+    TSP_HIP(hipDeviceGetStreamPriorityRange(&prio_low, &prio_high));
+    TSP_HIP(hipStreamCreateWithPriority(&ctx->stream, hipStreamNonBlocking, prio_low));
+    TSP_HIP(hipStreamCreateWithPriority(&ctx->stream2, hipStreamNonBlocking, prio_high));
     for (auto &e : ctx->ev) TSP_HIP(hipEventCreate(&e));
     const size_t npx = (size_t)resolution * resolution;
     TSP_HIP(hipMalloc((void **)&ctx->image, npx * n_channels * sizeof(float)));
@@ -283,6 +285,7 @@
         if (p) (void)hipFree(p);
     for (auto &e : ctx->ev)
         if (e) (void)hipEventDestroy(e);
+    for (auto &e : ctx->pass_ev) (void)hipEventDestroy(e);
     if (ctx->stream2) (void)hipStreamDestroy(ctx->stream2);
     if (ctx->stream) (void)hipStreamDestroy(ctx->stream);
     delete ctx;
@@ -688,6 +691,14 @@
     return TSP_OK;
 }
 
+int tsp_read_accumulator(tsp_context *ctx, double *out) {
+    TSP_REQUIRE(ctx && out, TSP_EINVAL, "NULL argument");
+    TSP_REQUIRE(!ctx->surface_keys, TSP_ESTATE, "the accumulator holds the keys of tsp_render_surface");
+    TSP_HIP(hipSetDevice(ctx->device));
+    TSP_HIP(hipMemcpy(out, ctx->image64, (size_t)ctx->R * ctx->R * ctx->C * sizeof(double), hipMemcpyDeviceToHost));
+    return TSP_OK;
+}
+
 int tsp_write_image(tsp_context *ctx, const float *in) {
     TSP_REQUIRE(ctx && in, TSP_EINVAL, "NULL argument");
     TSP_HIP(hipSetDevice(ctx->device));
@@ -1166,7 +1177,7 @@
         return TSP_OK;
     }
     if (!strcmp(name, "debug_fail_stage")) {
-        TSP_REQUIRE(value >= 0 && value <= 2, TSP_EINVAL, "%s out of range", name);
+        TSP_REQUIRE(value >= 0 && value <= 3, TSP_EINVAL, "%s out of range", name);
         ctx->debug_fail_stage = (int)value;
         return TSP_OK;
     }
@@ -1224,6 +1235,10 @@
         ctx->overlap_mid_huge = value != 0;
         return TSP_OK;
     }
+    if (!strcmp(name, "overlap_binning")) {
+        ctx->overlap_binning = value != 0;
+        return TSP_OK;
+    }
     if (!strcmp(name, "use_quantity")) {
         ctx->use_quantity = value != 0;
         return TSP_OK;
diff --git a/topsy_amd/csrc/tsp_group.hip b/topsy_amd/csrc/tsp_group.hip
--- a/topsy_amd/csrc/tsp_group.hip
+++ b/topsy_amd/csrc/tsp_group.hip
@@ -268,7 +268,7 @@
         t.n_fragments_huge += s.n_fragments_huge; t.n_fragments_mega += s.n_fragments_mega; t.n_chunk_culled += s.n_chunk_culled;
         t.ms_stream = std::max(t.ms_stream, s.ms_stream); t.ms_mid = std::max(t.ms_mid, s.ms_mid);
         t.ms_huge = std::max(t.ms_huge, s.ms_huge); t.ms_mega = std::max(t.ms_mega, s.ms_mega);
-        t.ms_total = std::max(t.ms_total, s.ms_total);
+        t.ms_total = std::max(t.ms_total, s.ms_total); t.ms_mid_bin = std::max(t.ms_mid_bin, s.ms_mid_bin);
     }
     *out = t;
     return TSP_OK;
diff --git a/topsy_amd/csrc/tsp_internal.h b/topsy_amd/csrc/tsp_internal.h
--- a/topsy_amd/csrc/tsp_internal.h
+++ b/topsy_amd/csrc/tsp_internal.h
@@ -109,6 +109,7 @@
     bool use_quantity = true;
     hipStream_t stream = nullptr;
     hipStream_t stream2 = nullptr;
+    std::vector<hipEvent_t> pass_ev;
     hipEvent_t ev[tsp::EV_COUNT] = {};
     float *image = nullptr;
     double *image64 = nullptr;
@@ -157,6 +158,7 @@
     bool chunk_cull = true;
     int64_t chunk_culled_particles = 0;
     bool overlap_mid_huge = false;
+    bool overlap_binning = true;
     int64_t slice_records = 0;
     int debug_fail_stage = 0;
     int64_t debug_fail_alloc = 0;
diff --git a/topsy_amd/csrc/tsp_mid.hip b/topsy_amd/csrc/tsp_mid.hip
--- a/topsy_amd/csrc/tsp_mid.hip
+++ b/topsy_amd/csrc/tsp_mid.hip
@@ -519,44 +519,90 @@
     }
 }
 
-template <int NW>
-static int bin_mid_records(tsp_context *ctx, TileArgs &ta, const float4 *mid_geom, const float *mid_w, long long n_mid, int tw, int th, float pmin,
-                           float pmax, bool exact, int *n_items_out, hipStream_t st) {
+static int strip_rows(int mode, bool second_channel) { return (mode == TSP_MODE_RGB || second_channel) ? 16 : TSP_G_HR1; }
+
+struct BinShape {
+    BinArgs ba;
+    int n_tiles, n_win, win_tiles;
+    unsigned grid;
+    bool lds;
+};
+static BinShape bin_shape(const tsp_context *ctx, const MidPass &p) {
+    BinShape s;
+    const int tw = p.narrow ? NSW : 64, th = strip_rows(p.mode, p.second_channel);
+    const int tiles_x = (ctx->R + tw - 1) / tw, tiles_y = (ctx->R + th - 1) / th;
+    BinArgs &ba = s.ba;
+    ba.R = ctx->R; ba.tw = tw; ba.th = th; ba.tiles_x = tiles_x; ba.tiles_y = tiles_y; ba.pmin = p.pmin; ba.pmax = p.pmax;
+    ba.disc_k2 = p.ta.disc_k2; ba.exact = p.narrow ? 1 : 0; ba.narrow = p.narrow ? 1 : 0;
+    ba.win_rows = std::max(1, G_WIN_TILES / tiles_x);
+    s.n_tiles = tiles_x * tiles_y;
+    s.n_win = (tiles_y + ba.win_rows - 1) / ba.win_rows;
+    s.win_tiles = std::min(tiles_y, ba.win_rows) * tiles_x;
+    s.grid = (unsigned)((p.n + 256 * TSP_BIN_PER - 1) / (256 * TSP_BIN_PER));
+    s.lds = s.win_tiles <= G_LDS_TILES;
+    return s;
+}
+
+int mid_passes(tsp_context *ctx, const TileArgs &ta, int mode, bool second_channel, const float4 *mid_geom, const float *mid_w, long long n_mid,
+               MidPass out[2], int *n_out) {
+    *n_out = 0;
+    TSP_REQUIRE(mode == TSP_MODE_WEIGHTED || mode == TSP_MODE_DEPTH || mode == TSP_MODE_RGB, TSP_EINVAL, "bad mode %d", mode);
+    TSP_REQUIRE(n_mid < (1ll << 28), TSP_EINVAL, "%lld mid footprints in one launch (kernel G indexes its work items with 32 bits; run_pipeline slices the list)", n_mid);
+    MidPass p;
+    p.mode = mode; p.second_channel = mode != TSP_MODE_WEIGHTED || second_channel;
+    p.geom = mid_geom; p.w = mid_w; p.n = n_mid; p.ta = ta; p.ta.n_records = n_mid;
+    p.item_records = 0; p.n_items = 0;
+    const float split = ctx->mid_narrow_px;
+    if (split > 0.0f) {
+        p.narrow = true; p.pmin = 0.0f; p.pmax = split;
+        out[(*n_out)++] = p;
+        if (split >= P_BILINEAR) return TSP_OK;
+    }
+    p.narrow = false; p.pmin = split; p.pmax = __builtin_inff();
+    out[(*n_out)++] = p;
+    return TSP_OK;
+}
+
+int mid_bin_count(tsp_context *ctx, MidPass &p, hipStream_t st) {
     Workspace &ws = ctx->ws;
-    const int tiles_x = (ctx->R + tw - 1) / tw, tiles_y = (ctx->R + th - 1) / th, n_tiles = tiles_x * tiles_y;
-    BinArgs ba;
-    ba.R = ctx->R; ba.tw = tw; ba.th = th; ba.tiles_x = tiles_x; ba.tiles_y = tiles_y; ba.pmin = pmin; ba.pmax = pmax;
-    ba.disc_k2 = ta.disc_k2; ba.exact = exact ? 1 : 0; ba.narrow = exact ? 1 : 0;
-    ba.win_rows = std::max(1, G_WIN_TILES / tiles_x);
-    const int n_win = (tiles_y + ba.win_rows - 1) / ba.win_rows, win_tiles = std::min(tiles_y, ba.win_rows) * tiles_x;
+    const BinShape s = bin_shape(ctx, p);
+    const int NW = (p.mode == TSP_MODE_RGB) ? 2 : 1;
     int rc;
-    if (ws.mtile_capacity < n_tiles) {
-        if ((rc = alloc_group(ctx, {{"mband_count", (void **)&ws.mband_count, 2 * (size_t)n_tiles * sizeof(int)},
-                                    {"mband_base", (void **)&ws.mband_base, ((size_t)n_tiles + 1) * sizeof(long long)},
-                                    {"mitem_base", (void **)&ws.mitem_base, ((size_t)n_tiles + 1) * sizeof(int)}},
-                              {{&ws.mtile_capacity, n_tiles}})))
+    if (ws.mtile_capacity < s.n_tiles) {
+        if ((rc = alloc_group(ctx, {{"mband_count", (void **)&ws.mband_count, 2 * (size_t)s.n_tiles * sizeof(int)},
+                                    {"mband_base", (void **)&ws.mband_base, ((size_t)s.n_tiles + 1) * sizeof(long long)},
+                                    {"mitem_base", (void **)&ws.mitem_base, ((size_t)s.n_tiles + 1) * sizeof(int)}},
+                              {{&ws.mtile_capacity, s.n_tiles}})))
             return rc;
     }
     if ((rc = check_workspace(ctx))) return rc;
     int item_records = ctx->mid_item_records;
     if (item_records <= 0) {
-        const double want = ctx->mid_item_scale * std::sqrt((double)n_mid);
+        const double want = ctx->mid_item_scale * std::sqrt((double)p.n);
         item_records = 64;
         while (item_records < GCHUNK_MAX && (double)item_records * 1.41 < want) item_records *= 2;
     }
+    p.item_records = item_records;
     TSP_HIP(hipMemsetAsync(ws.mband_count, 0, 2 * (size_t)ws.mtile_capacity * sizeof(int), st));
-    const bool lds = win_tiles <= G_LDS_TILES;
     if (!(ctx->kernel_attr_done & attr_bit_bins(NW))) {
         TSP_HIP(hipFuncSetAttribute((const void *)tile_count_kernel, hipFuncAttributeMaxDynamicSharedMemorySize, G_LDS_TILES * (int)sizeof(int)));
-        TSP_HIP(hipFuncSetAttribute((const void *)tile_fill_kernel<NW>, hipFuncAttributeMaxDynamicSharedMemorySize, 2 * G_LDS_TILES * (int)sizeof(int)));
+        if (NW == 2) TSP_HIP(hipFuncSetAttribute((const void *)tile_fill_kernel<2>, hipFuncAttributeMaxDynamicSharedMemorySize, 2 * G_LDS_TILES * (int)sizeof(int)));
+        else TSP_HIP(hipFuncSetAttribute((const void *)tile_fill_kernel<1>, hipFuncAttributeMaxDynamicSharedMemorySize, 2 * G_LDS_TILES * (int)sizeof(int)));
         ctx->kernel_attr_done |= attr_bit_bins(NW);
     }
-    const unsigned grid = (unsigned)((n_mid + 256 * TSP_BIN_PER - 1) / (256 * TSP_BIN_PER));
-    hipLaunchKernelGGL(tile_count_kernel, dim3(grid, n_win), dim3(256), lds ? win_tiles * sizeof(int) : 0, st, mid_geom, n_mid, ba, ws.mband_count);
-    hipLaunchKernelGGL(tile_prefix_kernel, dim3(1), dim3(1024), 0, st, (const int *)ws.mband_count, n_tiles, ws.mband_base, ws.mitem_base, (int *)nullptr, 0, item_records);
+    hipLaunchKernelGGL(tile_count_kernel, dim3(s.grid, s.n_win), dim3(256), s.lds ? s.win_tiles * sizeof(int) : 0, st, p.geom, p.n, s.ba, ws.mband_count);
+    hipLaunchKernelGGL(tile_prefix_kernel, dim3(1), dim3(1024), 0, st, (const int *)ws.mband_count, s.n_tiles, ws.mband_base, ws.mitem_base, (int *)nullptr, 0, item_records);
+    TSP_HIP(hipGetLastError());
+    return TSP_OK;
+}
+
+int mid_bin_prefix(tsp_context *ctx, MidPass &p, hipStream_t st) {
+    Workspace &ws = ctx->ws;
+    const BinShape s = bin_shape(ctx, p);
+    int rc;
     long long total_records = 0; int total_items = 0;
-    TSP_HIP(hipMemcpyAsync(&total_records, ws.mband_base + n_tiles, sizeof(long long), hipMemcpyDeviceToHost, st));
-    TSP_HIP(hipMemcpyAsync(&total_items, ws.mitem_base + n_tiles, sizeof(int), hipMemcpyDeviceToHost, st));
+    TSP_HIP(hipMemcpyAsync(&total_records, ws.mband_base + s.n_tiles, sizeof(long long), hipMemcpyDeviceToHost, st));
+    TSP_HIP(hipMemcpyAsync(&total_items, ws.mitem_base + s.n_tiles, sizeof(int), hipMemcpyDeviceToHost, st));
     TSP_HIP(hipStreamSynchronize(st));
     if (ws.mband_capacity < total_records || ws.mitem_capacity < total_items) {
         const int64_t rec_cap = std::max<int64_t>(ws.mband_capacity, total_records + total_records / 4 + 1024);
@@ -568,40 +614,46 @@
             return rc;
     }
     if ((rc = check_workspace(ctx))) return rc;
-    hipLaunchKernelGGL(tile_prefix_kernel, dim3(1), dim3(1024), 0, st, (const int *)ws.mband_count, n_tiles, ws.mband_base, ws.mitem_base, ws.mitem_tile, total_items, item_records);
-    hipLaunchKernelGGL((tile_fill_kernel<NW>), dim3(grid, n_win), dim3(256), lds ? 2 * win_tiles * sizeof(int) : 0, st, mid_geom, mid_w, n_mid, ba,
-                       (float4 *)ws.mband_geom, (float *)ws.mband_w, (const long long *)ws.mband_base, ws.mband_count + ws.mtile_capacity,
-                       &ctx->counters->mid_odd_weights);
+    hipLaunchKernelGGL(tile_prefix_kernel, dim3(1), dim3(1024), 0, st, (const int *)ws.mband_count, s.n_tiles, ws.mband_base, ws.mitem_base, ws.mitem_tile, total_items, p.item_records);
     TSP_HIP(hipGetLastError());
+    TileArgs &ta = p.ta;
     ta.geom = (const float4 *)ws.mband_geom; ta.w = (const float *)ws.mband_w;
     ta.bin_count = ws.mband_count; ta.band_stride = 0; ta.bin_base = ws.mband_base;
-    ta.item_tile = ws.mitem_tile; ta.item_base = ws.mitem_base; ta.n_tiles = n_tiles; ta.item_records = item_records;
-    ta.tiles_x = tiles_x;
-    *n_items_out = total_items;
+    ta.item_tile = ws.mitem_tile; ta.item_base = ws.mitem_base; ta.n_tiles = s.n_tiles; ta.item_records = p.item_records;
+    ta.tiles_x = s.ba.tiles_x;
+    p.n_items = total_items;
     return TSP_OK;
 }
 
+int mid_bin_fill(tsp_context *ctx, MidPass &p, hipStream_t st) {
+    Workspace &ws = ctx->ws;
+    const BinShape s = bin_shape(ctx, p);
+    const size_t smem = s.lds ? 2 * s.win_tiles * sizeof(int) : 0;
+    const dim3 grid(s.grid, s.n_win);
+    with_bool(p.mode == TSP_MODE_RGB, [&](auto RGB) {
+        hipLaunchKernelGGL((tile_fill_kernel<decltype(RGB)::value ? 2 : 1>), grid, dim3(256), smem, st, p.geom, p.w, p.n, s.ba,
+                           (float4 *)ws.mband_geom, (float *)ws.mband_w, (const long long *)ws.mband_base, ws.mband_count + ws.mtile_capacity,
+                           &ctx->counters->mid_odd_weights);
+        return 0;
+    });
+    TSP_HIP(hipGetLastError());
+    return TSP_OK;
+}
+
 struct KernelG {
-    static constexpr int STRIP_W = 64;
-    static constexpr bool EXACT_BINS = false;
     static size_t lds_bytes(bool quad, int ) { return (size_t)(quad ? MIPQ_TOTAL : MIP_TOTAL) * sizeof(float) + (H2T / 64) * 64 * sizeof(int); }
     template <int MODE, int NACC, int HR, int OCC, bool QUAD, bool CNT> static constexpr auto kernel() { return splat_mid_gather_kernel<MODE, NACC, HR, OCC, QUAD, CNT>; }
 };
 struct KernelN {
-    static constexpr int STRIP_W = NSW;
-    static constexpr bool EXACT_BINS = true;
     static size_t lds_bytes(bool quad, int HR) { return (size_t)(quad ? NQ_LINES * 32 : MIP_TOTAL + 64) * sizeof(float) + (H2T / 64) * 4 * HR * sizeof(int); }
     template <int MODE, int NACC, int HR, int OCC, bool QUAD, bool CNT> static constexpr auto kernel() { return splat_narrow_gather_kernel<MODE, NACC, HR, OCC, QUAD, CNT>; }
 };
 
 template <class K, int MODE, int NACC, int HR, int OCC>
-static int launch_strip_kernel(tsp_context *ctx, TileArgs ta, const float4 *mid_geom, const float *mid_w, long long n_mid, float pmin, float pmax, hipStream_t st) {
+static int launch_draw(tsp_context *ctx, const MidPass &p, hipStream_t st) {
     const bool quad = ctx->lut_mirror_symmetric && !ctx->debug_gather_full_lut;
-    int rc, n_items = 0;
-    ta.n_records = n_mid;
-    if ((rc = bin_mid_records<(MODE == TSP_MODE_RGB) ? 2 : 1>(ctx, ta, mid_geom, mid_w, n_mid, K::STRIP_W, HR, pmin, pmax, K::EXACT_BINS, &n_items, st))) return rc;
-    if (n_items == 0) return TSP_OK;
-    const dim3 grid((n_items + H2T / 64 - 1) / (H2T / 64));
+    const TileArgs ta = p.ta;
+    const dim3 grid((p.n_items + H2T / 64 - 1) / (H2T / 64));
     with_bool(quad, [&](auto Q) { with_bool(ta.count_frag != 0, [&](auto CNT) {
         hipLaunchKernelGGL((K::template kernel<MODE, NACC, HR, OCC, decltype(Q)::value, decltype(CNT)::value>()), grid, dim3(H2T), K::lds_bytes(quad, HR), st, ta);
     }); });
@@ -609,29 +661,32 @@
     return TSP_OK;
 }
 template <class K, int MODE>
-static int launch_strip_kernel_mode(tsp_context *ctx, TileArgs ta, bool second_channel, const float4 *mid_geom, const float *mid_w, long long n_mid, float pmin, float pmax, hipStream_t st) {
-    if (MODE == TSP_MODE_RGB) return launch_strip_kernel<K, MODE, 3, 16, TSP_G_OCC3>(ctx, ta, mid_geom, mid_w, n_mid, pmin, pmax, st);
-    if (second_channel) return launch_strip_kernel<K, MODE, 2, 16, TSP_G_OCC2>(ctx, ta, mid_geom, mid_w, n_mid, pmin, pmax, st);
-    return launch_strip_kernel<K, MODE, 1, TSP_G_HR1, TSP_G_OCC1>(ctx, ta, mid_geom, mid_w, n_mid, pmin, pmax, st);
-}
-
-template <int MODE>
-static int launch_mid_gather_mode(tsp_context *ctx, TileArgs ta, bool second_channel, const float4 *mid_geom, const float *mid_w, long long n_mid, hipStream_t st) {
-    TSP_REQUIRE(n_mid < (1ll << 28), TSP_EINVAL, "%lld mid footprints in one launch (kernel G indexes its work items with 32 bits; run_pipeline slices the list)", n_mid);
-    const float split = ctx->mid_narrow_px;
-    if (split > 0.0f) {
-        if (int rc = launch_strip_kernel_mode<KernelN, MODE>(ctx, ta, second_channel, mid_geom, mid_w, n_mid, 0.0f, split, st)) return rc;
-        if (split >= P_BILINEAR) return TSP_OK;
-    }
-    return launch_strip_kernel_mode<KernelG, MODE>(ctx, ta, second_channel, mid_geom, mid_w, n_mid, split, __builtin_inff(), st);
+static int launch_draw_mode(tsp_context *ctx, const MidPass &p, hipStream_t st) {
+    if (MODE == TSP_MODE_RGB) return launch_draw<K, MODE, 3, 16, TSP_G_OCC3>(ctx, p, st);
+    if (p.second_channel) return launch_draw<K, MODE, 2, 16, TSP_G_OCC2>(ctx, p, st);
+    return launch_draw<K, MODE, 1, TSP_G_HR1, TSP_G_OCC1>(ctx, p, st);
+}
+
+int mid_draw(tsp_context *ctx, const MidPass &p, hipStream_t st) {
+    if (p.n_items == 0) return TSP_OK;
+    return with_mode(p.mode, [&](auto M) {
+        constexpr int MODE = decltype(M)::value;
+        return p.narrow ? launch_draw_mode<KernelN, MODE>(ctx, p, st) : launch_draw_mode<KernelG, MODE>(ctx, p, st);
+    });
 }
 
 int launch_mid_gather(tsp_context *ctx, TileArgs ta, int mode, bool second_channel, const float4 *mid_geom, const float *mid_w,
                       long long n_mid, hipStream_t st) {
-    return with_mode(mode, [&](auto M) {
-        constexpr int MODE = decltype(M)::value;
-        return launch_mid_gather_mode<MODE>(ctx, ta, MODE != TSP_MODE_WEIGHTED || second_channel, mid_geom, mid_w, n_mid, st);
-    });
-}
-
-}
+    MidPass pass[2];
+    int n_pass = 0, rc;
+    if ((rc = mid_passes(ctx, ta, mode, second_channel, mid_geom, mid_w, n_mid, pass, &n_pass))) return rc;
+    for (int i = 0; i < n_pass; ++i) {
+        if ((rc = mid_bin_count(ctx, pass[i], st))) return rc;
+        if ((rc = mid_bin_prefix(ctx, pass[i], st))) return rc;
+        if ((rc = mid_bin_fill(ctx, pass[i], st))) return rc;
+        if ((rc = mid_draw(ctx, pass[i], st))) return rc;
+    }
+    return TSP_OK;
+}
+
+}
diff --git a/topsy_amd/csrc/tsp_pipeline.h b/topsy_amd/csrc/tsp_pipeline.h
--- a/topsy_amd/csrc/tsp_pipeline.h
+++ b/topsy_amd/csrc/tsp_pipeline.h
@@ -115,4 +115,19 @@
 int launch_mid_gather(tsp_context *ctx, TileArgs ta, int mode, bool second_channel, const float4 *mid_geom, const float *mid_w,
                       long long n_mid, hipStream_t st);
 
+struct MidPass {
+    bool narrow;
+    int mode; bool second_channel;
+    const float4 *geom; const float *w; long long n;
+    float pmin, pmax;
+    TileArgs ta;
+    int item_records, n_items;
+};
+int mid_passes(tsp_context *ctx, const TileArgs &ta, int mode, bool second_channel, const float4 *mid_geom, const float *mid_w, long long n_mid,
+               MidPass out[2], int *n_out);
+int mid_bin_count(tsp_context *ctx, MidPass &pass, hipStream_t st);
+int mid_bin_prefix(tsp_context *ctx, MidPass &pass, hipStream_t st);
+int mid_bin_fill(tsp_context *ctx, MidPass &pass, hipStream_t st);
+int mid_draw(tsp_context *ctx, const MidPass &pass, hipStream_t st);
+
 }
diff --git a/topsy_amd/csrc/tsp_pipeline.hip b/topsy_amd/csrc/tsp_pipeline.hip
--- a/topsy_amd/csrc/tsp_pipeline.hip
+++ b/topsy_amd/csrc/tsp_pipeline.hip
@@ -660,6 +660,99 @@
 }
 
 template <int MODE>
+static int run_block_overlapped(tsp_context *ctx, const TileArgs &ta, bool second_channel, const Counters &hc, bool cull) {
+    Workspace &ws = ctx->ws;
+    hipStream_t st = ctx->stream, sb = ctx->stream2;
+    int rc;
+    if ((rc = check_workspace(ctx))) return rc;
+    if (ctx->debug_fail_stage == 1) { ctx->debug_fail_stage = 0; TSP_REQUIRE(false, TSP_ENOMEM, "injected failure after kernel S (debug_fail_stage)"); }
+    constexpr int NWr = (MODE == TSP_MODE_RGB) ? 2 : 1;
+    const long long n_mid = (long long)hc.n_mid, n_huge = (long long)hc.n_huge;
+    const long long mid_slice = ctx->slice_records > 0 ? ctx->slice_records : (1ll << 27);
+    const long long huge_slice = ctx->slice_records > 0 ? ctx->slice_records : (1ll << 30);
+    const float4 *mid_geom = (const float4 *)ws.mid_geom, *huge_geom = (const float4 *)ws.huge_geom;
+    const float *mid_w = (const float *)ws.mid_w, *huge_w = (const float *)ws.huge_w;
+
+    std::vector<MidPass> passes;
+    for (long long o = 0; o < n_mid; o += mid_slice) {
+        MidPass two[2];
+        int k = 0;
+        if ((rc = mid_passes(ctx, ta, MODE, second_channel, mid_geom + o, mid_w + o * NWr, std::min(mid_slice, n_mid - o), two, &k))) return rc;
+        passes.insert(passes.end(), two, two + k);
+    }
+    enum { COUNT0, COUNT1, FILL0, FILL1, DRAW0, DRAW1, PER_PASS };
+    while (ctx->pass_ev.size() < passes.size() * PER_PASS) {
+        hipEvent_t e;
+        TSP_HIP(hipEventCreate(&e));
+        ctx->pass_ev.push_back(e);
+    }
+    auto ev = [&](size_t pass, int which) { return ctx->pass_ev[pass * PER_PASS + which]; };
+    auto bin_count = [&](size_t i, hipStream_t s) -> int {
+        TSP_HIP(hipEventRecord(ev(i, COUNT0), s));
+        if (int e = mid_bin_count(ctx, passes[i], s)) return e;
+        TSP_HIP(hipEventRecord(ev(i, COUNT1), s));
+        return TSP_OK;
+    };
+    auto bin_fill = [&](size_t i, hipStream_t s) -> int {
+        if (int e = mid_bin_prefix(ctx, passes[i], s)) return e;
+        TSP_HIP(hipEventRecord(ev(i, FILL0), s));
+        if (int e = mid_bin_fill(ctx, passes[i], s)) return e;
+        TSP_HIP(hipEventRecord(ev(i, FILL1), s));
+        return TSP_OK;
+    };
+    auto draw = [&](size_t i) -> int {
+        TSP_HIP(hipEventRecord(ev(i, DRAW0), st));
+        if (int e = mid_draw(ctx, passes[i], st)) return e;
+        TSP_HIP(hipEventRecord(ev(i, DRAW1), st));
+        return TSP_OK;
+    };
+
+    if (!passes.empty()) {
+        TSP_HIP(hipEventRecord(ctx->ev[EV_S_DONE], st));
+        TSP_HIP(hipStreamWaitEvent(sb, ctx->ev[EV_S_DONE], 0));
+        if ((rc = bin_count(0, sb))) return rc;
+    }
+    TSP_HIP(hipEventRecord(ctx->ev[EV_HUGE_BEGIN], st));
+    TSP_HIP(hipEventRecord(ctx->ev[EV_HUGE_END], st));
+    for (long long o = 0; o < n_huge; o += huge_slice)
+        if ((rc = launch_gather_kernels(ctx, ta, MODE, second_channel, huge_geom + o, huge_w + o * NWr, std::min(huge_slice, n_huge - o)))) return rc;
+    if (!passes.empty() && (rc = bin_fill(0, sb))) return rc;
+    if (ctx->debug_fail_stage == 3) { ctx->debug_fail_stage = 0; TSP_REQUIRE(false, TSP_ENOMEM, "injected failure between the bins and kernel N (debug_fail_stage)"); }
+    if (!passes.empty()) {
+        TSP_HIP(hipStreamWaitEvent(st, ev(0, FILL1), 0));
+        if ((rc = draw(0))) return rc;
+        for (size_t i = 1; i < passes.size(); ++i)
+            if ((rc = bin_count(i, st)) || (rc = bin_fill(i, st)) || (rc = draw(i))) return rc;
+    }
+    if (ctx->debug_fail_stage == 2) { ctx->debug_fail_stage = 0; TSP_REQUIRE(false, TSP_ENOMEM, "injected failure after kernel G (debug_fail_stage)"); }
+    if (MODE == TSP_MODE_RGB && (n_mid > 0 || n_huge > 0)) {
+        if (n_mid <= mid_slice && n_huge <= huge_slice) {
+            if ((rc = add_rect_counts(ctx, mid_geom, n_mid, huge_geom, n_huge))) return rc;
+        } else {
+            for (long long o = 0; o < n_mid; o += mid_slice)
+                if ((rc = add_rect_counts(ctx, mid_geom + o, std::min(mid_slice, n_mid - o), nullptr, 0))) return rc;
+            for (long long o = 0; o < n_huge; o += huge_slice)
+                if ((rc = add_rect_counts(ctx, nullptr, 0, huge_geom + o, std::min(huge_slice, n_huge - o)))) return rc;
+        }
+    }
+    TSP_HIP(hipEventRecord(ctx->ev[EV_BLOCK_END], st));
+    TSP_HIP(hipStreamSynchronize(st));
+    float ms = 0.f;
+    TSP_HIP(hipEventElapsedTime(&ms, ctx->ev[cull ? EV_CULL_BEGIN : EV_S_BEGIN], ctx->ev[EV_S_END])); ctx->stats.ms_stream = ms;
+    TSP_HIP(hipEventElapsedTime(&ms, ctx->ev[EV_HUGE_BEGIN], ctx->ev[EV_HUGE_END])); ctx->stats.ms_huge = ms;
+    double ms_bin = 0.0, ms_draw = 0.0;
+    for (size_t i = 0; i < passes.size(); ++i) {
+        TSP_HIP(hipEventElapsedTime(&ms, ev(i, COUNT0), ev(i, COUNT1))); ms_bin += ms;
+        TSP_HIP(hipEventElapsedTime(&ms, ev(i, FILL0), ev(i, FILL1))); ms_bin += ms;
+        TSP_HIP(hipEventElapsedTime(&ms, ev(i, DRAW0), ev(i, DRAW1))); ms_draw += ms;
+    }
+    ctx->stats.ms_mid_bin = ms_bin;
+    ctx->stats.ms_mid = ms_bin + ms_draw;
+    ctx->stats.ms_mega = 0.0;
+    return TSP_OK;
+}
+
+template <int MODE>
 static int run_pipeline(tsp_context *ctx, const Camera &cam, const int64_t *h_starts, const int64_t *h_lens, int n_ranges,
                         int64_t total) {
     constexpr int C = (MODE == TSP_MODE_RGB) ? 4 : 2;
@@ -789,6 +882,7 @@
     ta.count_frag = ctx->count_fragments ? 1 : 0;
     ta.bin_count = nullptr; ta.band_stride = 0; ta.bin_base = nullptr; ta.n_tiles = 0; ta.item_tile = nullptr; ta.item_base = nullptr;
     ta.disc_k2 = (ctx->lut_zero_outside_disc && !ctx->count_fragments) ? 0.5235f * 0.5235f : 0.0f;
+    if (ctx->overlap_binning && !ctx->overlap_mid_huge) return run_block_overlapped<MODE>(ctx, ta, second_channel, hc, cull);
     hipStream_t st_mid = ctx->overlap_mid_huge ? ctx->stream2 : st;
     if (ctx->overlap_mid_huge) {
         TSP_HIP(hipEventRecord(ctx->ev[EV_S_DONE], st));
@@ -806,7 +900,7 @@
     for (long long o = 0; o < n_mid; o += mid_slice)
         if ((rc = launch_mid_gather(ctx, ta, MODE, second_channel, mid_geom + o, mid_w + o * NWr, std::min(mid_slice, n_mid - o), st_mid))) return rc;
     TSP_HIP(hipEventRecord(ctx->ev[EV_MID_END], st_mid));
-    if (ctx->debug_fail_stage == 2) { ctx->debug_fail_stage = 0; TSP_REQUIRE(false, TSP_ENOMEM, "injected failure after kernel G (debug_fail_stage)"); }
+    if (ctx->debug_fail_stage >= 2) { ctx->debug_fail_stage = 0; TSP_REQUIRE(false, TSP_ENOMEM, "injected failure after kernel G (debug_fail_stage)"); }
     TSP_HIP(hipEventRecord(ctx->ev[EV_HUGE_BEGIN], st));
     TSP_HIP(hipEventRecord(ctx->ev[EV_HUGE_END], st));
     for (long long o = 0; o < n_huge; o += huge_slice)
```
